# JoelTankard/web-rwkv-gguf

Measured on AMD Instinct MI355X. Metric: tokens/sec RWKV-7 1.5B Q4_K_M decode @1 GPU; achieved HBM GB/s vs roofline, higher is better.
Workload: dtype f16; 1 GPU; RWKV-7 World 1.5B Q4_K_M (Q4_K matrices, Q6_K head, F16 LoRA) batch=1 greedy decode, fused kernels under hipGraph; decode_engine=on, streams_per_gpu=1, pipelines_per_gpu=1, streams=1, parallelism=single

## Files before the change

include/wrk_hip.h:

```cpp
#ifndef WRK_HIP_H
#define WRK_HIP_H

#include <stddef.h>
#include <stdint.h>

#ifdef __cplusplus
extern "C" {
#endif

#define WRK_ABI_VERSION 1

typedef struct wrk_ctx wrk_ctx;
typedef struct wrk_buf wrk_buf;
typedef struct wrk_matrix wrk_matrix;
typedef struct wrk_program wrk_program;
typedef struct wrk_v7_model wrk_v7_model;
typedef struct wrk_v7_state wrk_v7_state;

enum {
    WRK_OK = 0,
    WRK_E_ARG = 1,
    WRK_E_OOM = 2,
    WRK_E_HIP = 3,
    WRK_E_UNSUPPORTED = 4
// ... 56 lines not shown
int32_t wrk_buf_read(wrk_ctx* ctx, const wrk_buf* buf, size_t offset, void* dst, size_t bytes);
int32_t wrk_buf_copy(wrk_ctx* ctx, const wrk_buf* src, size_t src_off, wrk_buf* dst, size_t dst_off, size_t bytes);

int32_t wrk_capture_begin(wrk_ctx* ctx);
int32_t wrk_capture_end(wrk_ctx* ctx, wrk_program** out);
int32_t wrk_program_launch(wrk_ctx* ctx, wrk_program* prog);
int32_t wrk_program_destroy(wrk_program* prog);

int32_t wrk_matrix_create(wrk_ctx* ctx, uint32_t kind, uint32_t k, uint32_t m,
                          const void* data, size_t bytes, uint32_t flags, wrk_matrix** out);
int32_t wrk_matrix_quantize(wrk_ctx* ctx, uint32_t kind, uint32_t k, uint32_t m,
                            const wrk_buf* f16_data, const float* levels, wrk_matrix** out);
int32_t wrk_matrix_export(wrk_matrix* mat, void* dst, size_t capacity, size_t* bytes);
int32_t wrk_matrix_set_scale(wrk_matrix* mat, float scale);
int32_t wrk_matrix_release(wrk_matrix* mat);
size_t wrk_matrix_stream_bytes(const wrk_matrix* mat);


int32_t wrk_op_matmul(wrk_ctx* ctx, const wrk_matrix* mat, const wrk_tensor* input, const wrk_tensor* output,
                      uint32_t act, int32_t turbo, int32_t sparse);
int32_t wrk_op_layer_norm(wrk_ctx* ctx, const wrk_buf* w, const wrk_buf* b, const wrk_tensor* x, float eps);
int32_t wrk_op_group_norm(wrk_ctx* ctx, const wrk_buf* w, const wrk_buf* b, const wrk_tensor* x, float eps);
int32_t wrk_op_l2_norm(wrk_ctx* ctx, const wrk_tensor* x, float eps);
int32_t wrk_op_token_shift(wrk_ctx* ctx, const wrk_buf* cursors, const wrk_tensor* time_mix, const wrk_tensor* state,
                           const wrk_tensor* input, const wrk_tensor* output, int32_t reversed);
int32_t wrk_op_transpose(wrk_ctx* ctx, const wrk_tensor* input, const wrk_tensor* output);
int32_t wrk_op_time_mix_v6(wrk_ctx* ctx, const wrk_buf* cursors, const wrk_tensor* time_decay, const wrk_buf* time_first,
                           const wrk_tensor* state, const wrk_tensor* k, const wrk_tensor* v, const wrk_tensor* r, const wrk_tensor* x);
int32_t wrk_op_channel_mix(wrk_ctx* ctx, const wrk_buf* cursors, const wrk_tensor* state, const wrk_tensor* r, const wrk_tensor* v, const wrk_tensor* x);
int32_t wrk_op_add(wrk_ctx* ctx, const wrk_tensor* input, const wrk_tensor* output, uint32_t act_x, uint32_t act_y, uint32_t act_o);
int32_t wrk_op_mul(wrk_ctx* ctx, const wrk_tensor* input, const wrk_tensor* output, uint32_t act_x, uint32_t act_y, uint32_t act_o);
int32_t wrk_op_lerp(wrk_ctx* ctx, const wrk_tensor* x, const wrk_tensor* y, const wrk_tensor* f, int32_t reversed);
int32_t wrk_op_blit(wrk_ctx* ctx, const wrk_tensor* input, const wrk_tensor* output);
int32_t wrk_op_affine(wrk_ctx* ctx, const wrk_tensor* x, float scale, float bias);
int32_t wrk_op_activate(wrk_ctx* ctx, const wrk_tensor* x, uint32_t act);
int32_t wrk_op_control_k_v7(wrk_ctx* ctx, const wrk_buf* p, const wrk_tensor* a, const wrk_tensor* k);
int32_t wrk_op_time_mix_v7(wrk_ctx* ctx, const wrk_buf* cursors, const wrk_tensor* state, const wrk_tensor* r,
                           const wrk_tensor* w, const wrk_tensor* n, const wrk_tensor* x);
int32_t wrk_op_time_first_v7(wrk_ctx* ctx, const wrk_buf* u, const wrk_tensor* r, const wrk_tensor* n, const wrk_tensor* x);
int32_t wrk_op_channel_mix_v7(wrk_ctx* ctx, const wrk_buf* cursors, const wrk_tensor* state, const wrk_tensor* v, const wrk_tensor* x);
int32_t wrk_op_softmax(wrk_ctx* ctx, const wrk_tensor* x);


typedef struct wrk_v7_layer_desc {
    const wrk_buf *ln1_w, *ln1_b, *ln2_w, *ln2_b;
    const wrk_buf *x_r, *x_w, *x_k, *x_v, *x_a, *x_g;
    const wrk_buf *w0, *a0, *v0;
    const wrk_matrix *w1, *w2, *a1, *a2, *g1, *g2, *v1, *v2;
    const wrk_buf *r_k, *k_k, *k_a;
    const wrk_matrix *w_k, *w_v, *w_r, *w_o;
    const wrk_buf *gn_w, *gn_b;
    const wrk_buf* ffn_x_k;
    const wrk_matrix *ffn_w_k, *ffn_w_v;
} wrk_v7_layer_desc;

typedef struct wrk_v7_model_desc {
    uint32_t num_layer, num_emb, num_hidden, num_vocab, num_head;
    uint32_t lora_w, lora_a, lora_g, lora_v;
    uint32_t rescale;
    const wrk_buf *ln0_w, *ln0_b, *ln_out_w, *ln_out_b;
    const wrk_buf* emb_f16;
    const wrk_matrix* head;
    const wrk_v7_layer_desc* layers;
} wrk_v7_model_desc;

int32_t wrk_v7_model_create(wrk_ctx* ctx, const wrk_v7_model_desc* desc, wrk_v7_model** out);
int32_t wrk_v7_model_destroy(wrk_v7_model* model);
size_t wrk_v7_model_token_bytes(const wrk_v7_model* model, uint32_t num_batch);

int32_t wrk_v7_state_create(wrk_ctx* ctx, const wrk_v7_model* model, uint32_t num_batch, wrk_v7_state** out);
int32_t wrk_v7_state_destroy(wrk_v7_state* state);
int32_t wrk_v7_state_load(wrk_ctx* ctx, wrk_v7_state* state, uint32_t batch, const float* src);
int32_t wrk_v7_state_back(wrk_ctx* ctx, const wrk_v7_state* state, uint32_t batch, float* dst);
int32_t wrk_v7_state_read(wrk_ctx* ctx, const wrk_v7_state* state, uint32_t batch, wrk_buf* buf);
int32_t wrk_v7_state_write(wrk_ctx* ctx, wrk_v7_state* state, uint32_t batch, const wrk_buf* buf);

int32_t wrk_v7_infer(wrk_ctx* ctx, wrk_v7_model* model, wrk_v7_state* state,
                     const uint32_t* tokens, const uint16_t* emb_rows, const uint32_t* cursors, uint32_t num_token,
                     const uint32_t* headers, uint32_t num_header, float* logits, uint32_t* argmax, uint32_t mode);

int32_t wrk_v7_model_set_frame_dtype(wrk_ctx* ctx, wrk_v7_model* model, uint32_t dtype);

int32_t wrk_v7_model_engine_status(wrk_ctx* ctx, wrk_v7_model* model, char* why, size_t capacity);

int32_t wrk_v7_infer_layer(wrk_ctx* ctx, wrk_v7_model* model, wrk_v7_state* state, uint32_t layer, const void* x, const void* v_first,
                           const uint32_t* cursors, uint32_t num_token, uint32_t mode);
int32_t wrk_v7_frame_read(wrk_ctx* ctx, wrk_v7_model* model, const char* name, uint32_t num_token, void* dst, size_t capacity, size_t* bytes);

int32_t wrk_v7_generate_greedy(wrk_ctx* ctx, wrk_v7_model* model, wrk_v7_state* state,
                               const uint32_t* first_tokens, uint32_t num_batch, uint32_t steps,
                               uint32_t* out_tokens, float* last_logits_or_null, float* elapsed_ms_or_null, uint32_t mode);

int32_t wrk_sample_logits(wrk_ctx* ctx, const wrk_buf* logits, uint32_t num_vocab, uint32_t row_stride, uint32_t num_rows,
                          const float* temperature, const float* top_p, const uint32_t* seed, uint32_t step, uint32_t* out_tokens);
int32_t wrk_v7_generate_sample(wrk_ctx* ctx, wrk_v7_model* model, wrk_v7_state* state, const uint32_t* first_tokens, uint32_t num_batch,
                               uint32_t steps, const float* temperature, const float* top_p, const uint32_t* seed,
                               uint32_t* out_tokens, float* last_logits_or_null, float* elapsed_ms_or_null, uint32_t mode);

int32_t wrk_score_logits(wrk_ctx* ctx, const wrk_buf* logits, uint32_t num_vocab, uint32_t row_stride, uint32_t num_rows,
                         const uint32_t* targets, float* logprob, uint32_t* rank);
int32_t wrk_v7_score(wrk_ctx* ctx, wrk_v7_model* model, wrk_v7_state* state,
                     const uint32_t* tokens, const uint16_t* emb_rows, const uint32_t* cursors, uint32_t num_token,
                     const uint32_t* headers, uint32_t num_header, const uint32_t* targets, float* logprob, uint32_t* rank, uint32_t mode);

typedef struct wrk_occurrence wrk_occurrence;
int32_t wrk_occurrence_create(wrk_ctx* ctx, uint32_t num_batch, uint32_t num_vocab, wrk_occurrence** out);
int32_t wrk_occurrence_destroy(wrk_occurrence* occ);
int32_t wrk_occurrence_set_weights(wrk_ctx* ctx, wrk_occurrence* occ, const float* weights);
int32_t wrk_occurrence_ban(wrk_ctx* ctx, wrk_occurrence* occ, uint32_t batch, const uint32_t* tokens, uint32_t n, int32_t banned);
int32_t wrk_occurrence_add(wrk_ctx* ctx, wrk_occurrence* occ, uint32_t batch, const uint32_t* tokens, uint32_t n, float decay);
int32_t wrk_occurrence_back(wrk_ctx* ctx, const wrk_occurrence* occ, uint32_t batch, float* counts, uint32_t* flags);
int32_t wrk_occurrence_load(wrk_ctx* ctx, wrk_occurrence* occ, uint32_t batch, const float* counts, const uint32_t* flags);
int32_t wrk_penalize_logits(wrk_ctx* ctx, wrk_buf* logits, uint32_t num_vocab, uint32_t row_stride, uint32_t num_rows,
                            const wrk_occurrence* occ, uint32_t first_batch, const float* presence, const float* frequency);
int32_t wrk_v7_generate_penalized(wrk_ctx* ctx, wrk_v7_model* model, wrk_v7_state* state, const uint32_t* first_tokens, uint32_t num_batch,
                                  uint32_t steps, const float* temperature, const float* top_p, const uint32_t* seed, const float* presence,
                                  const float* frequency, const float* decay, wrk_occurrence* occ, uint32_t* out_tokens,
                                  float* last_logits_or_null, float* elapsed_ms_or_null, uint32_t mode);

#define WRK_MAX_STOP_TOKENS 16
typedef struct wrk_generate_options {
    const float *temperature, *top_p;
    const uint32_t *seed;
    const float *presence, *frequency, *decay;
    wrk_occurrence *occ;
    const uint32_t *stop_tokens, *stop_offsets;
    uint32_t poll_steps;
} wrk_generate_options;
int32_t wrk_v7_generate_stop(wrk_ctx* ctx, wrk_v7_model* model, wrk_v7_state* state, const uint32_t* first_tokens, uint32_t num_batch,
                             uint32_t steps, const wrk_generate_options* opt, uint32_t* out_tokens, uint32_t* out_lengths,
                             float* last_logits_or_null, uint32_t* steps_run, float* elapsed_ms_or_null, uint32_t mode);

typedef struct wrk_v6_model wrk_v6_model;

typedef struct wrk_v6_layer_desc {
    const wrk_buf *ln1_w, *ln1_b, *ln2_w, *ln2_b;
    const wrk_buf *time_decay;
    const wrk_buf *time_first;
    const wrk_buf *time_mix_x;
    const wrk_buf *time_mix;
    const wrk_matrix *time_decay_w1, *time_decay_w2, *time_mix_w1;
    const wrk_matrix *time_mix_w2[5];
    const wrk_matrix *w_k, *w_v, *w_r, *w_g, *w_o;
    const wrk_buf *gn_w, *gn_b;
    const wrk_buf *ffn_mix_k, *ffn_mix_r;
    const wrk_matrix *ffn_w_k, *ffn_w_v, *ffn_w_r;
} wrk_v6_layer_desc;

typedef struct wrk_v6_model_desc {
    uint32_t num_layer, num_emb, num_hidden, num_vocab, num_head;
    uint32_t time_mix, time_decay;
    uint32_t rescale;
    const wrk_buf *ln0_w, *ln0_b, *ln_out_w, *ln_out_b, *emb_f16;
    const wrk_matrix* head;
    const wrk_v6_layer_desc* layers;
} wrk_v6_model_desc;

int32_t wrk_v6_model_create(wrk_ctx* ctx, const wrk_v6_model_desc* desc, wrk_v6_model** out);
int32_t wrk_v6_model_destroy(wrk_v6_model* model);
size_t wrk_v6_model_token_bytes(const wrk_v6_model* model, uint32_t num_batch);
int32_t wrk_v6_state_create(wrk_ctx* ctx, const wrk_v6_model* model, uint32_t num_batch, wrk_v7_state** out);
int32_t wrk_v6_infer(wrk_ctx* ctx, wrk_v6_model* model, wrk_v7_state* state,
                     const uint32_t* tokens, const uint16_t* emb_rows, const uint32_t* cursors, uint32_t num_token,
                     const uint32_t* headers, uint32_t num_header, float* logits, uint32_t* argmax, uint32_t mode);
int32_t wrk_v6_generate_greedy(wrk_ctx* ctx, wrk_v6_model* model, wrk_v7_state* state,
                               const uint32_t* first_tokens, uint32_t num_batch, uint32_t steps,
// ... 22 lines not shown
```

web-rwkv-gguf_amd/csrc/wrk_runner.h:

```cpp
#pragma once
#include <atomic>
#include <functional>
#include <map>
#include <tuple>
#include <vector>

#include "wrk_internal.h"
#include "wrk_device.h"

struct wrk_v7_state {
    const void* uid = next_uid();
    static const void* next_uid() { static std::atomic<uintptr_t> n{1}; return (const void*)(n.fetch_add(1) << 4); }
    wrk_ctx* ctx = nullptr;
    uint32_t num_layer = 0, num_emb = 0, head_size = 0, num_batch = 0;
    float* data = nullptr;
    size_t layer_elems() const { return (size_t)num_batch * (head_size + 2) * num_emb; }
    float* layer_ptr(uint32_t l) const { return data + layer_elems() * l; }
};

namespace wrk {
struct FrameIo {
    float* head_o;
    uint32_t *cursors, *tokens, *headers, *argmax, *counter;
};

MatJob mat_job(const wrk_matrix* m, DTensor in, DTensor out, uint32_t act);

void advance_tokens(hipStream_t s, const uint32_t* argmax, uint32_t* tokens, uint32_t* history, uint32_t* counter, uint32_t b);
void argmax_finish(hipStream_t s, const float* pv, const uint32_t* pi, uint32_t nwg, uint32_t ntok, uint32_t* argmax, uint32_t* tokens,
                   uint32_t* history, uint32_t* counter);

struct LnMixParams {
    const f16* src;
    const uint32_t* ids;
    const f16 *ln_w, *ln_b;
    float eps;
    uint32_t d, nmix;
    const f16* mix[6];
    f16* out[6];
    f16* ln_out;
    float* state_row;
    size_t state_stride;
    const uint32_t* cursors;
    uint32_t batch1;
    uint32_t no_carry;
};
int ln_mix(hipStream_t s, const LnMixParams& P, uint32_t T);
}

int32_t wrk_buf_write_raw(wrk_ctx* ctx, void* dst, const void* src, size_t bytes);

int32_t wrk_mm(wrk_ctx* ctx, const wrk_matrix* m, DTensor in, DTensor out, uint32_t act);
int32_t wrk_mm_group(wrk_ctx* ctx, wrk::MatJob* jobs, int n);

struct wrk_job_args {
    const uint32_t* tokens; const uint16_t* emb_rows;
    const uint32_t* cursors; uint32_t T;
    const uint32_t* headers; uint32_t NH;
    float* logits; uint32_t* argmax;
    bool score; const uint32_t* targets; float* logprob; uint32_t* rank;
};
struct wrk_job_shape { uint32_t nseq; bool one_token_each, contiguous, identity; };
int32_t wrk_job_check(wrk_ctx* ctx, const wrk_v7_state* st, const uint32_t* cursors, uint32_t T, const uint32_t* tokens_or_null, uint32_t V,
                      const uint32_t* headers, uint32_t NH, wrk_job_shape* shape);
int32_t wrk_score_check(wrk_ctx* ctx, const wrk_job_args& a, uint32_t V, const char* who);

struct wrk_frame_common {
    wrk_ctx* ctx = nullptr;
    void* scratch = nullptr;
    uint32_t scratch_tokens = 0, scratch_headers = 0;
    uint32_t* history = nullptr;
    size_t history_cap = 0;
    wrk::SampleParam* sample_par = nullptr;
    uint32_t sample_par_cap = 0;
    wrk::PenaltyParam* pen_par = nullptr;
    float* pen_o = nullptr;
    uint32_t pen_cap = 0;
    wrk_score_scratch score;
    wrk::StopParam* stop_par = nullptr;
    uint32_t* stop_flags = nullptr;
    float *stop_snap_state = nullptr, *stop_snap_logits = nullptr;
    uint32_t stop_cap = 0;
    size_t stop_slot_cap = 0;
    uint32_t stop_vocab_cap = 0;
    uint32_t* stop_just_ended() const { return stop_flags; }
    uint32_t* stop_live() const { return stop_flags + stop_cap; }
    uint32_t* stop_lengths() const { return stop_flags + stop_cap + 1; }
    uint32_t* live_host = nullptr;
    uint32_t live_host_cap = 0;
    std::vector<hipEvent_t> poll_events;
    uint32_t wkv_nseq = 0;

    struct GraphKey {
        const void* state; uint32_t b, mode, nh = 0;
        bool operator<(const GraphKey& o) const { return std::tie(state, b, mode, nh) < std::tie(o.state, o.b, o.mode, o.nh); }
    };
    std::map<GraphKey, wrk_program*> graphs;

    void drop_graphs();
    int32_t ensure_history(size_t n);
    int32_t ensure_sample_params(uint32_t n);
    int32_t ensure_penalty(uint32_t n, uint32_t num_vocab);
    int32_t ensure_stop(uint32_t n, uint32_t L, uint32_t S, uint32_t D, uint32_t V);
    int32_t ensure_poll(uint32_t lanes);
    void release_common();
};

int32_t wrk_cached_program(wrk_ctx* ctx, std::map<wrk_frame_common::GraphKey, wrk_program*>& graphs, const wrk_frame_common::GraphKey& key,
                           const std::function<int32_t()>& enqueue, wrk_program** prog);

int32_t wrk_job_upload(wrk_frame_common& f, wrk::FrameIo& io, void* input, const wrk_buf* emb, uint32_t D, const wrk_job_args& a, bool gather);
int32_t wrk_job_read_back(wrk_frame_common& f, const wrk::FrameIo& io, uint32_t V, const wrk_job_args& a);

struct wrk_pick_args {
    const float *temperature, *top_p; const uint32_t* seed;
    bool penalized = false;
    const float *presence = nullptr, *frequency = nullptr, *decay = nullptr; wrk_occurrence* occ = nullptr;
};
struct wrk_pick_params {
    std::vector<wrk::SampleParam> par_rows; std::vector<wrk::PenaltyParam> pen_rows;
    const wrk::SampleParam* par = nullptr; const wrk::PenaltyParam* pen = nullptr;
};
int32_t wrk_pick_pack(wrk_ctx* ctx, const wrk_pick_args* pick, uint32_t B, uint32_t V, wrk_pick_params& out);
int32_t wrk_generate_check(wrk_ctx* ctx, const wrk_v7_state* st, bool has_emb, uint32_t num_emb, uint32_t num_layer, uint32_t V,
                           const uint32_t* first_tokens, uint32_t B);
int32_t wrk_decode_prepare(wrk_frame_common& f, wrk::FrameIo& io, uint32_t V, const uint32_t* first_tokens, uint32_t b0, uint32_t B, uint32_t steps,
                           const wrk::SampleParam* par, const wrk::PenaltyParam* pen);
struct wrk_stop_step { const wrk_v7_state* st; uint32_t b0; };
// ... 15 lines not shown
```

web-rwkv-gguf_amd/csrc/wrk_v7.hip:

```cpp
#include "wrk_internal.h"
#include "wrk_v7.h"
#include "wrk_v7_engine.h"

#define LOCK(ctx) std::lock_guard<std::recursive_mutex> _lk((ctx)->mu)

static constexpr float LN_EPS = 1.0e-5f;
static constexpr float GN_EPS = 64.0e-5f;
static constexpr float L2_EPS = 1.0e-12f;

static inline size_t up256(size_t x) { return (x + 255) & ~(size_t)255; }
using wrk::mat_job;

int32_t wrk_v7_model::ensure_scratch(uint32_t T, uint32_t NH) {
    if (T <= scratch_tokens && NH <= scratch_headers && scratch) return WRK_OK;
    if (ctx->capturing_here()) return wrk_fail(ctx, WRK_E_ARG, "scratch must be sized before capture");
    const uint32_t nt = T > scratch_tokens ? T : scratch_tokens;
    const uint32_t nh = NH > scratch_headers ? NH : scratch_headers;
    WRK_HIP(ctx, hipStreamSynchronize(ctx->stream));
    drop_graphs();
    if (scratch) hipFree(scratch);
    scratch = nullptr;
    const size_t D = d.num_emb, F = d.num_hidden, V = d.num_vocab;
    size_t off = 0;
    auto take = [&](size_t bytes) { size_t o = off; off += up256(bytes); return o; };
// ... 400 lines not shown
    wrk_job_shape sh;
    int32_t rc = wrk_job_check(ctx, st, a.cursors, T, a.tokens, V, a.headers, NH, &sh);
    if (rc == WRK_OK) rc = wrk_score_check(ctx, a, V, "wrk_v7_score");
    if (rc == WRK_OK) rc = m->ensure_scratch(T, NH ? NH : 1);
    if (rc == WRK_OK && T == 1 && mode == 1) rc = m->ensure_engine();
    if (rc != WRK_OK) return rc;
    const bool fused = (mode == 1 && sh.one_token_each && sh.nseq == T && m->act_dtype == WRK_F16), want_argmax = NH && a.argmax;
    const uint32_t batch0 = a.cursors[0] & 0xffu;
    rc = wrk_job_upload(*m, m->s, m->s.input, m->emb, m->d.num_emb, a, !fused);
    if (rc != WRK_OK) return rc;
    m->wkv_nseq = sh.nseq;
    auto enqueue_job = [&]() -> int32_t {
        int32_t r;
        if (fused) r = m->enqueue_fused_decode(st, T, NH, sh.identity, a.tokens != nullptr, want_argmax, false, batch0, sh.contiguous);
        else {
            r = m->enqueue_ops(st, T, NH, sh.identity, mode == 1);
            if (r == WRK_OK && want_argmax) wrk::argmax_rows(ctx->op_stream(), m->s.head_o, V, V, NH, m->s.argmax);
        }
        if (r == WRK_OK && a.score && NH &&
            wrk::score_rows(ctx->op_stream(), m->s.head_o, V, V, NH, m->score.targets, m->score.part, m->score.logprob, m->score.rank,
                            ctx->num_cu) != 0)
            r = wrk_fail(ctx, WRK_E_UNSUPPORTED, "score: vocabulary of %u tokens", V);
        return r;
    };
    static const bool no_graph = [] { const char* e = getenv("WRK_NO_GRAPH"); return e && e[0] == '1'; }();
    if (no_graph || ctx->capturing_here()) rc = enqueue_job();
    else {
        const uint32_t flags = 16u | (m->act_dtype == WRK_F32 ? 64u : 0u) | (fused ? 1u : 0u) | (sh.identity ? 2u : 0u) | (a.tokens ? 4u : 0u) | (want_argmax ? 8u : 0u) |
                               ((!fused && mode == 1) ? 32u : 0u) | (fused ? batch0 << 8 : 0u) | ((fused && sh.contiguous) ? 1u << 16 : 0u) |
                               ((fused && T == 1 && m->engine_on()) ? 1u << 17 : 0u) | (split_head_env_on() ? 0u : 1u << 18) |
                               ((!fused && (size_t)sh.nseq * m->d.num_head >= 768) ? 1u << 19 : 0u) | (a.score ? 1u << 20 : 0u);
        const wrk_v7_model::GraphKey key{st->uid, T, flags, NH};
        if (!m->graphs.count(key) && m->graphs.size() > 64) { WRK_HIP(ctx, hipStreamSynchronize(ctx->stream)); m->drop_graphs(); }
        wrk_program* prog = nullptr;
        rc = wrk_cached_program(ctx, m->graphs, key, enqueue_job, &prog);
        if (rc != WRK_OK) return rc;
        WRK_HIP(ctx, hipGraphLaunch(prog->exec, ctx->stream));
    }
    if (rc == WRK_OK) rc = wrk_job_read_back(*m, m->s, V, a);
    if (rc != WRK_OK || ctx->capturing_here()) return rc;
    return wrk_v7_engine_check(m->engine);
}

int32_t wrk_v7_infer(wrk_ctx* ctx, wrk_v7_model* m, wrk_v7_state* st, const uint32_t* tokens, const uint16_t* emb_rows,
                     const uint32_t* cursors, uint32_t T, const uint32_t* headers, uint32_t NH, float* logits, uint32_t* argmax,
                     uint32_t mode) {
    return v7_job(ctx, m, st, {tokens, emb_rows, cursors, T, headers, NH, logits, argmax, false, nullptr, nullptr, nullptr}, mode);
}

int32_t wrk_v7_score(wrk_ctx* ctx, wrk_v7_model* m, wrk_v7_state* st, const uint32_t* tokens, const uint16_t* emb_rows,
                     const uint32_t* cursors, uint32_t T, const uint32_t* headers, uint32_t NH, const uint32_t* targets, float* logprob,
                     uint32_t* rank, uint32_t mode) {
    return v7_job(ctx, m, st, {tokens, emb_rows, cursors, T, headers, NH, nullptr, nullptr, true, targets, logprob, rank}, mode);
}

int32_t wrk_v7_model_set_frame_dtype(wrk_ctx* ctx, wrk_v7_model* m, uint32_t dtype) {
    if (!ctx || !m) return WRK_E_ARG;
    LOCK(ctx);
    WRK_ARG(ctx, dtype == WRK_F16 || dtype == WRK_F32, "frame dtype must be WRK_F16 or WRK_F32");
    WRK_ARG(ctx, !ctx->capturing_here(), "cannot change the frame inside a capture");
    if (dtype == m->act_dtype) return WRK_OK;
    WRK_HIP(ctx, hipSetDevice(ctx->device));
    WRK_HIP(ctx, hipStreamSynchronize(ctx->stream));
    m->drop_graphs();
    if (m->scratch) hipFree(m->scratch);
    m->scratch = nullptr;
    m->scratch_tokens = m->scratch_headers = 0;
    m->act_dtype = dtype;
    for (hipStream_t ls : m->lane_streams) WRK_HIP(ctx, hipStreamSynchronize(ls));
    std::vector<wrk_v7_model*> old_lanes;
    old_lanes.swap(m->lanes);
    for (wrk_v7_model* lane : old_lanes) wrk_v7_model_destroy(lane);
    return WRK_OK;
}

int32_t wrk_v7_model_engine_status(wrk_ctx* ctx, wrk_v7_model* m, char* why, size_t capacity) {
    if (!ctx || !m) return WRK_E_ARG;
    LOCK(ctx);
    WRK_HIP(ctx, hipSetDevice(ctx->device));
    WRK_ARG(ctx, !ctx->capturing_here(), "not inside a capture");
    const int32_t rc = m->ensure_engine();
    if (rc != WRK_OK) return rc;
    if (why && capacity) {
        const std::string& w = m->engine ? std::string() : (m->engine_tried ? m->engine_why : std::string("disabled (WRK_ENGINE=0 or f32 frames)"));
        snprintf(why, capacity, "%s", w.c_str());
    }
    return m->engine ? 1 : 0;
}

int32_t wrk_v7_infer_layer(wrk_ctx* ctx, wrk_v7_model* m, wrk_v7_state* st, uint32_t layer, const void* x, const void* v_first,
                           const uint32_t* cursors, uint32_t T, uint32_t mode) {
    if (!ctx || !m || !st || !x || !cursors) return WRK_E_ARG;
    LOCK(ctx);
    WRK_HIP(ctx, hipSetDevice(ctx->device));
    WRK_ARG(ctx, !ctx->capturing_here(), "wrk_v7_infer_layer cannot be captured");
    WRK_ARG(ctx, layer < m->d.num_layer, "layer %u out of range", layer);
    WRK_ARG(ctx, T >= 1, "no tokens");
    WRK_ARG(ctx, layer == 0 || v_first, "layers above 0 read the layer-0 value (att_v0)");
    WRK_ARG(ctx, st->num_emb == m->d.num_emb && st->num_layer == m->d.num_layer, "state does not belong to this model");
    wrk_job_shape sh;
    int32_t rc = wrk_job_check(ctx, st, cursors, T, nullptr, 0, nullptr, 0, &sh);
    if (rc == WRK_OK) rc = m->ensure_scratch(T, 1);
    if (rc == WRK_OK && T == 1 && mode == 1) rc = m->ensure_engine();
    if (rc != WRK_OK) return rc;
    const size_t esz = m->act_dtype == WRK_F32 ? 4 : 2;
    rc = wrk_buf_write_raw(ctx, m->s.cursors, cursors, (size_t)T * 4);
    if (rc == WRK_OK) rc = wrk_buf_write_raw(ctx, m->s.x, x, (size_t)T * m->d.num_emb * esz);
    if (rc == WRK_OK && v_first) rc = wrk_buf_write_raw(ctx, m->s.att_v0, v_first, (size_t)T * m->d.num_emb * esz);
    if (rc != WRK_OK) return rc;
    m->layer_begin = layer; m->layer_end = layer + 1; m->skip_embed = true;
    m->wkv_nseq = sh.nseq;
    { const char* ei = getenv("WRK_ENGINE_INSPECT"); m->engine_skip_once = !(ei && ei[0] == '1'); }
    if (mode == 1 && sh.one_token_each && sh.nseq == T && m->act_dtype == WRK_F16) rc = m->enqueue_fused_decode(st, T, 0, true, false, false, false, cursors[0] & 0xff, sh.contiguous);
    else rc = m->enqueue_ops(st, T, 0, true, mode == 1);
    m->layer_begin = 0; m->layer_end = 0xffffffffu; m->skip_embed = false; m->engine_skip_once = false;
    if (rc != WRK_OK) return rc;
    WRK_LAUNCH_CHECK(ctx);
    WRK_HIP(ctx, hipStreamSynchronize(ctx->stream));
    return wrk_v7_engine_check(m->engine);
}

int32_t wrk_v7_frame_read(wrk_ctx* ctx, wrk_v7_model* m, const char* name, uint32_t T, void* dst, size_t capacity, size_t* bytes) {
    if (!ctx || !m || !name || !bytes) return WRK_E_ARG;
    LOCK(ctx);
    WRK_ARG(ctx, m->scratch && T >= 1 && T <= m->scratch_tokens, "no frame of %u tokens has been run", T);
    const uint32_t D = m->d.num_emb, F = m->d.num_hidden;
    const V7Scratch& s = m->s;
    struct { const char* n; const void* p; uint32_t c; } tab[] = {
        {"x", s.x, D}, {"att_x", s.att_x, D}, {"att_v0", s.att_v0, D}, {"att_rx", s.rx, D}, {"att_wx", s.wx, D}, {"att_kx", s.kx, D},
        {"att_vx", s.vx, D}, {"att_ax", s.ax, D}, {"att_gx", s.gx, D}, {"att_r", s.r, D}, {"att_w", s.w, D}, {"att_k", s.k, D}, {"att_v", s.v, D},
        {"att_a", s.a, D}, {"att_g", s.g, D}, {"att_o", s.o, D}, {"att_kk", s.kk, D}, {"att_vv", s.vv, D}, {"att_n", s.n, 4 * D},
        {"aux_w", s.aux_w, m->d.lora_w}, {"aux_a", s.aux_a, m->d.lora_a}, {"aux_g", s.aux_g, m->d.lora_g}, {"aux_v", s.aux_v, m->d.lora_v},
        {"ffn_x", s.ffn_x, D}, {"ffn_kx", s.ffn_kx, D}, {"ffn_k", s.ffn_k, F}, {"ffn_v", s.ffn_v, D}, {"att_x_ln", s.ln_tmp, D}};
    const size_t esz = m->act_dtype == WRK_F32 ? 4 : 2;
    for (auto& e : tab)
        if (strcmp(e.n, name) == 0) {
            const size_t n = (size_t)e.c * T * esz;
            *bytes = n;
            if (!dst) return WRK_OK;
            WRK_ARG(ctx, capacity >= n, "frame buffer %s needs %zu bytes, capacity %zu", name, n, capacity);
            WRK_HIP(ctx, hipSetDevice(ctx->device));
            WRK_HIP(ctx, hipMemcpyAsync(dst, e.p, n, hipMemcpyDeviceToHost, ctx->stream));
            WRK_HIP(ctx, hipStreamSynchronize(ctx->stream));
            return WRK_OK;
        }
    return wrk_fail(ctx, WRK_E_ARG, "no frame buffer named %s", name);
}

static int32_t enqueue_decode_step(wrk_ctx* ctx, wrk_v7_model* m, wrk_v7_state* st, uint32_t b0, uint32_t B, uint32_t mode, bool sampled,
                                   bool penalized, bool stop = false) {
    int32_t rc;
    const wrk_stop_step ss{st, b0};
    if (mode == 1 && m->act_dtype == WRK_F16) {
        rc = m->enqueue_fused_decode(st, B, B, true, true, !sampled, !sampled && !stop, b0, true);
        if (!sampled && (!stop || rc != WRK_OK)) return rc;
        if (!sampled) return wrk_enqueue_stop_tail(*m, m->s, m->d.num_vocab, B, false, ss);
    } else {
        wrk::gather_rows_f16(ctx->op_stream(), m->emb->ptr, m->s.tokens, m->s.input, m->d.num_emb, B);
        rc = m->enqueue_ops(st, B, B, true);
    }
    if (rc != WRK_OK) return rc;
    return wrk_enqueue_pick(*m, m->s, m->d.num_vocab, B, sampled, penalized, stop ? &ss : nullptr);
}

static int32_t decode_prepare(wrk_ctx* ctx, wrk_v7_model* m, wrk_v7_state* st, const uint32_t* first_tokens, uint32_t b0, uint32_t B,
                              uint32_t steps, uint32_t mode, bool eager, const wrk::SampleParam* par, const wrk::PenaltyParam* pen,
                              const wrk::StopParam* stop, wrk_program** prog_out) {
    int32_t rc = m->ensure_scratch(B, B);
    if (rc == WRK_OK && B == 1 && mode == 1) rc = m->ensure_engine();
    if (rc == WRK_OK) rc = wrk_decode_prepare(*m, m->s, m->d.num_vocab, first_tokens, b0, B, steps, par, pen);
// ... 134 lines not shown
```

web-rwkv-gguf_amd/csrc/wrk_v7_engine.h:

```cpp
#pragma once
#include <stdint.h>

#include "wrk_internal.h"

namespace wrk {

constexpr int ENG_K1_JOBS = 7;
constexpr uint32_t ENG_NO_HEAD = 0xffffffffu;

struct EngJob {
    uint32_t rows, row_bytes, f16;
    uint32_t act, mix;
    uint32_t wg0, nwg, rows_per_wg;
    uint32_t gbase;
    uint32_t headed;
};

struct EngShape {
    uint32_t D, F, H, nwg;
    uint32_t rw, ra, rg, rv;
    uint32_t rb_d, rb_f;
    uint32_t rb_w2, rb_a2, rb_g2, rb_v2;
    EngJob k1[ENG_K1_JOBS];
    uint32_t k3_rpw, k5_rpw, k6_rpw;
    uint32_t lds_slot1, lds_slot5, lds_slot6, lds_slot3, lds_xraw0, lds_xraw1, lds_xs, lds_ln, lds_misc, lds_total;
    uint32_t g_x, g_k1, g_o, g_x1, g_k, g_total, g_aux;
    float ln_eps, gn_eps, l2_eps;
    uint32_t layer_begin, layer_end, rescale;
    uint32_t batch, state_rows;
    uint32_t x_from_granules;
};

struct EngLayer {
    const uint8_t *w_r, *w_k, *w_v, *w1, *a1, *g1, *v1;
    const uint8_t *w2, *a2, *g2, *v2;
    const uint8_t *w_o, *ffn_k, *ffn_v;
};
enum { ENG_V_LN1W, ENG_V_LN1B, ENG_V_LN2W, ENG_V_LN2B, ENG_V_MIX0, ENG_V_W0 = ENG_V_MIX0 + 6, ENG_V_A0, ENG_V_V0, ENG_V_RK, ENG_V_KK, ENG_V_KA,
       ENG_V_GNW, ENG_V_GNB, ENG_V_FFNXK, ENG_NV };
enum { ENG_S_O = ENG_K1_JOBS, ENG_S_FK, ENG_S_FV, ENG_NS = 16 };

struct EngArgs {
    EngShape S;
    const EngLayer* layers;
    const void* vecs;
    const float* scal;
    unsigned long long* gran;
    const void* x_in;
    const uint32_t* x_row;
    void* x_out;
    void* v_first;
    float* state;
    uint32_t num_batch;
    uint32_t* fail;
    unsigned long long* stamps;
    uint32_t stamp_layer;
};
constexpr int ENG_STAMPS = 32;

}

struct wrk_v7_model;
struct wrk_v7_state;
struct wrk_v7_engine;
int32_t wrk_v7_engine_create(wrk_v7_model* m, wrk_v7_engine** out);
void wrk_v7_engine_destroy(wrk_v7_engine* e);
int32_t wrk_v7_engine_enqueue(wrk_v7_engine* e, hipStream_t q, wrk_v7_state* st, uint32_t batch, uint32_t l0, uint32_t l1, const void* x_in,
                              void* x_out, void* v_first, const uint32_t* token = nullptr);
bool wrk_v7_engine_has_table(const wrk_v7_engine* e);
int32_t wrk_v7_engine_check(wrk_v7_engine* e);
void wrk_v7_engine_report(wrk_v7_engine* e);
```

web-rwkv-gguf_amd/csrc/wrk_v7_engine.hip:

```cpp
#include "wrk_device.h"
#include "wrk_v7.h"
#include "wrk_dmv_body.h"
#include "wrk_v7_engine.h"
#include "wrk_lora_dev.h"

#include <algorithm>
#include <string>

namespace wrk {

#define ENG_LDS __attribute__((address_space(3)))
typedef ENG_LDS unsigned char lds_u8;

#define ENG_BAR() asm volatile("s_waitcnt lgkmcnt(0)\n\ts_barrier" ::: "memory")

constexpr uint32_t ENG_SPIN_MAX = 1u << 21;

__device__ __forceinline__ uint32_t eng_tag(uint32_t layer, uint32_t stage) { return layer * 8u + stage + 1u; }

__device__ __forceinline__ void eng_store_granule(unsigned long long* g, uint32_t tag, uint32_t payload) {
    __hip_atomic_store(g, ((unsigned long long)tag << 32) | payload, __ATOMIC_RELAXED, __HIP_MEMORY_SCOPE_AGENT);
}
__device__ __forceinline__ uint32_t pack_h2(float a, float b) {
    const f16x2 h = {(f16)a, (f16)b};
    return __builtin_bit_cast(uint32_t, h);
}

__device__ __forceinline__ bool eng_gather(const unsigned long long* g, uint32_t n16, uint32_t tag, ENG_LDS uint32_t* dst, uint32_t lane) {
    for (uint32_t base = 0; base < n16; base += 512) {
        const u32x4* p[8];
#pragma unroll
        for (int i = 0; i < 8; ++i) p[i] = (const u32x4*)g + min(base + lane + 64u * i, n16 - 1);
        u32x4 v[8];
        bool good = false;
        for (uint32_t spins = 0; spins < ENG_SPIN_MAX; ++spins) {
            asm volatile(
                "global_load_dwordx4 %0, %8, off sc1\n\tglobal_load_dwordx4 %1, %9, off sc1\n\tglobal_load_dwordx4 %2, %10, off sc1\n\t"
                "global_load_dwordx4 %3, %11, off sc1\n\tglobal_load_dwordx4 %4, %12, off sc1\n\tglobal_load_dwordx4 %5, %13, off sc1\n\t"
                "global_load_dwordx4 %6, %14, off sc1\n\tglobal_load_dwordx4 %7, %15, off sc1\n\ts_waitcnt vmcnt(0)"
                : "=&v"(v[0]), "=&v"(v[1]), "=&v"(v[2]), "=&v"(v[3]), "=&v"(v[4]), "=&v"(v[5]), "=&v"(v[6]), "=&v"(v[7])
                : "v"(p[0]), "v"(p[1]), "v"(p[2]), "v"(p[3]), "v"(p[4]), "v"(p[5]), "v"(p[6]), "v"(p[7])
                : "memory");
            bool ok = true;
#pragma unroll
            for (int i = 0; i < 8; ++i) ok &= (v[i].y == tag) & (v[i].w == tag);
            if (__all(ok)) { good = true; break; }
            __builtin_amdgcn_s_sleep(1);
        }
        if (!good) return false;
#pragma unroll
        for (int i = 0; i < 8; ++i) {
            const uint32_t q = base + lane + 64u * i;
            if (q < n16) { dst[2 * q] = v[i].x; dst[2 * q + 1] = v[i].z; }
        }
    }
    return true;
}

__device__ __forceinline__ void eng_copy_in(const void* src, uint32_t n16, ENG_LDS u32x4* dst, uint32_t lane) {
    for (uint32_t q = lane; q < n16; q += 64) dst[q] = ((const u32x4*)src)[q];
}

template <int KIND>
__device__ __forceinline__ bool eng_sweep_x(const unsigned long long* g, uint32_t c, uint32_t tag, XRegs& x) {
    uint32_t lo, hi;
    chunk_xoff<KIND>(c, lo, hi);
    const u32x4* pl = (const u32x4*)g + (lo >> 2);
    const u32x4* ph = (const u32x4*)g + (hi >> 2);
    u32x4 v[8];
    for (uint32_t spins = 0; spins < ENG_SPIN_MAX; ++spins) {
        asm volatile(
            "global_load_dwordx4 %0, %8, off sc1\n\tglobal_load_dwordx4 %1, %8, off offset:16 sc1\n\tglobal_load_dwordx4 %2, %8, off offset:32 sc1\n\t"
            "global_load_dwordx4 %3, %8, off offset:48 sc1\n\tglobal_load_dwordx4 %4, %9, off sc1\n\tglobal_load_dwordx4 %5, %9, off offset:16 sc1\n\t"
            "global_load_dwordx4 %6, %9, off offset:32 sc1\n\tglobal_load_dwordx4 %7, %9, off offset:48 sc1\n\ts_waitcnt vmcnt(0)"
            : "=&v"(v[0]), "=&v"(v[1]), "=&v"(v[2]), "=&v"(v[3]), "=&v"(v[4]), "=&v"(v[5]), "=&v"(v[6]), "=&v"(v[7])
            : "v"(pl), "v"(ph)
            : "memory");
        bool ok = true;
#pragma unroll
        for (int i = 0; i < 8; ++i) ok &= (v[i].y == tag) & (v[i].w == tag);
        if (__all(ok)) {
#pragma unroll
            for (int h = 0; h < 4; ++h) {
                const u32x4 q = {v[2 * h].x, v[2 * h].z, v[2 * h + 1].x, v[2 * h + 1].z};
                x.v[h] = __builtin_bit_cast(f16x8, q);
            }
            return true;
        }
        __builtin_amdgcn_s_sleep(1);
    }
    return false;
}

__device__ __forceinline__ uint32_t eng_fill(const uint8_t* src, uint32_t bytes, lds_u8* smem, uint32_t lds_off, uint32_t lane) {
    if (bytes == 0) return 0;
    const uint32_t np = (bytes + 1023u) >> 10;
    for (uint32_t p = 0; p < np; ++p) {
        const uint32_t off = min(p * 1024u + lane * 16u, bytes - 16u);
        __builtin_amdgcn_global_load_lds((const __attribute__((address_space(1))) void*)(src + off), (ENG_LDS void*)(smem + lds_off + p * 1024u), 16, 0, 2);
    }
    return np;
// ... 9 lines not shown
    else asm volatile("s_waitcnt vmcnt(0)" ::: "memory");
}

template <int KIND>
__device__ __forceinline__ Raw lds_raw(const lds_u8* row, uint32_t k, uint32_t c) {
    Raw r;
    r.w = *(const ENG_LDS u32x4*)(row + c * 16u);
    r.a = (u32x4){0, 0, 0, 0};
    r.b = (u32x2){0, 0};
    const uint32_t nb = k >> 8, b = c >> 3;
    if (KIND == WRK_MAT_Q4_K) {
        r.a.x = *(const ENG_LDS uint32_t*)(row + (nb * 128u + b * 4u));
        r.a.y = *(const ENG_LDS uint32_t*)(row + (nb * 132u + b * 16u + ((c & 7u) >> 1) * 4u));
    }
    return r;
}

template <int KIND>
__device__ __forceinline__ XRegs lds_x(const ENG_LDS f16* x, uint32_t c) {
    XRegs r;
    const f16x8 z = {0, 0, 0, 0, 0, 0, 0, 0};
    r.v[0] = r.v[1] = r.v[2] = r.v[3] = z;
    r.s[0] = r.s[1] = 0.0f;
    uint32_t lo, hi;
    chunk_xoff<KIND>(c, lo, hi);
    r.v[0] = *(const ENG_LDS f16x8*)(x + lo);
    if (KIND != WRK_MAT_F16) {
        r.v[1] = *(const ENG_LDS f16x8*)(x + lo + 8);
        r.v[2] = *(const ENG_LDS f16x8*)(x + hi);
        r.v[3] = *(const ENG_LDS f16x8*)(x + hi + 8);
    }
    return r;
}

template <int MAXCH>
__device__ __forceinline__ float eng_lora_dot(const f16x8 (&w)[MAXCH], const ENG_LDS f16* aux, uint32_t rank, uint32_t part) {
    float acc = 0.0f;
#pragma unroll
    for (int n = 0; n < MAXCH; ++n) {
        const uint32_t c = part * 8 + 32 * n;
        if (c < rank) {
            const f16x8 x = *(const ENG_LDS f16x8*)(aux + c);
            acc = __builtin_amdgcn_fdot2(__builtin_shufflevector(w[n], w[n], 0, 1), __builtin_shufflevector(x, x, 0, 1), acc, false);
            acc = __builtin_amdgcn_fdot2(__builtin_shufflevector(w[n], w[n], 2, 3), __builtin_shufflevector(x, x, 2, 3), acc, false);
            acc = __builtin_amdgcn_fdot2(__builtin_shufflevector(w[n], w[n], 4, 5), __builtin_shufflevector(x, x, 4, 5), acc, false);
            acc = __builtin_amdgcn_fdot2(__builtin_shufflevector(w[n], w[n], 6, 7), __builtin_shufflevector(x, x, 6, 7), acc, false);
        }
    }
    acc += dpp_f32<0xB1>(acc);
    acc += dpp_f32<0x4E>(acc);
    return acc;
}

struct EngFin {
    uint32_t act;
    float scale;
    const ENG_LDS f16* res;
    float post;
};
__device__ __forceinline__ float eng_finish(const EngFin& f, uint32_t row, float v) {
    float o = act_apply(f.act, v * f.scale);
    if (f.res) o = r16(o) + (float)f.res[row];
    return o;
}

template <int KIND, bool R16, int XI, int RB, class GIDX>
__device__ __forceinline__ void eng_rows(const lds_u8* slot, uint32_t row_bytes, uint32_t K, const ENG_LDS f16* xs, uint32_t row0, uint32_t r_begin,
                                         uint32_t r_end, const EngFin& fin, ENG_LDS uint32_t* pub, unsigned long long* gran, uint32_t tag, GIDX gidx,
                                         uint32_t lane) {
    if (r_begin >= r_end) return;
    const uint32_t kpad = (K + 15u) & ~15u;
    const uint32_t nch = num_chunks<KIND>(K, kpad);
    XRegs x[1][XI];
#pragma unroll
    for (int ci = 0; ci < XI; ++ci) {
        const uint32_t c = lane + 64u * ci;
        x[0][ci] = lds_x<KIND>(xs, min(c, nch - 1));
        if (c >= nch) {
            const f16x8 z = {0, 0, 0, 0, 0, 0, 0, 0};
            x[0][ci].v[0] = x[0][ci].v[1] = x[0][ci].v[2] = x[0][ci].v[3] = z;
        }
        x_sums<KIND>(x[0][ci]);
    }
    static_assert(RB == 2 || RB == 4, "rows per batch");
    for (uint32_t ri = r_begin; ri < r_end; ri += RB) {
        Raw raw[RB][XI];
#pragma unroll
        for (int rb = 0; rb < RB; ++rb) {
            const lds_u8* rowp = slot + (size_t)min(ri + rb, r_end - 1) * row_bytes;
#pragma unroll
            for (int ci = 0; ci < XI; ++ci) raw[rb][ci] = lds_raw<KIND>(rowp, K, min(lane + 64u * ci, nch - 1));
        }
        float v[4] = {0.0f, 0.0f, 0.0f, 0.0f};
#pragma unroll
        for (int rb = 0; rb < RB; ++rb) {
            float acc[1] = {0.0f};
#pragma unroll
            for (int ci = 0; ci < XI; ++ci) dot_raw_tokens<KIND, R16, 1, XI>(raw[rb][ci], min(lane + 64u * ci, nch - 1), x, ci, acc);
            v[rb] = wave_sum(acc[0]);
        }
        if (lane < RB / 2) {
            const uint32_t ra = ri + 2 * lane;
            if (ra < r_end) {
                const float o0 = eng_finish(fin, row0 + ra, lane ? v[2] : v[0]) * fin.post;
                const float o1 = eng_finish(fin, row0 + ra + 1, lane ? v[3] : v[1]) * fin.post;
                if (pub) pub[ra >> 1] = pack_h2(o0, o1);
                else eng_store_granule(gran + gidx(row0 + ra), tag, pack_h2(o0, o1));
            }
        }
    }
}

template <class GIDX>
__device__ __forceinline__ void eng_publish(const ENG_LDS uint32_t* pub, uint32_t nrows, uint32_t row0, unsigned long long* gran, uint32_t tag, GIDX gidx,
                                            uint32_t lane) {
    for (uint32_t i = lane; 2 * i < nrows; i += 64) eng_store_granule(gran + gidx(row0 + 2 * i), tag, pub[i]);
}

template <int VPT>
__device__ __forceinline__ void eng_ln_mix(bool active, const ENG_LDS f16* xraw, ENG_LDS f16* xs, ENG_LDS f16* ln_out, ENG_LDS float* red, uint32_t K, float eps,
                                           const f16x8 (&wv)[VPT], const f16x8 (&bv)[VPT], const f16x8 (&mv)[VPT], const f32x4 (&pv)[VPT][2],
                                           uint32_t tid, uint32_t lane, uint32_t wave) {
    const uint32_t nvec = K >> 3;
    f16x8 xv[VPT];
    float c0 = 0.0f;
    if (active) {
#pragma unroll
        for (int v = 0; v < VPT; ++v) xv[v] = *(const ENG_LDS f16x8*)(xraw + min(tid + 256u * v, nvec - 1) * 8);
        c0 = (float)xraw[0];
        float s1 = 0.0f, s2 = 0.0f;
#pragma unroll
        for (int v = 0; v < VPT; ++v)
            if (tid + 256u * v < nvec)
#pragma unroll
                for (int e = 0; e < 8; ++e) { const float dl = (float)xv[v][e] - c0; s1 += dl; s2 = __builtin_fmaf(dl, dl, s2); }
        s1 = wave_sum(s1);
        s2 = wave_sum(s2);
        if (lane == 0) { red[wave] = s1; red[4 + wave] = s2; }
    }
    ENG_BAR();
    if (active) {
        const float a1 = (red[0] + red[1]) + (red[2] + red[3]);
        const float a2 = (red[4] + red[5]) + (red[6] + red[7]);
        const float md = a1 / (float)K;
        const float mean = c0 + md;
        const float dev = 1.0f / sqrtf(fmaxf(a2 / (float)K - md * md, 0.0f) + eps);
#pragma unroll
        for (int v = 0; v < VPT; ++v) {
            const uint32_t i = tid + 256u * v;
            if (i >= nvec) continue;
            f16x8 yv, o;
#pragma unroll
            for (int e = 0; e < 8; ++e) {
                yv[e] = (f16)__builtin_fmaf(((float)xv[v][e] - mean) * dev, (float)wv[v][e], (float)bv[v][e]);
                o[e] = (f16)wgsl_mix((float)yv[e], pv[v][e >> 2][e & 3], (float)mv[v][e]);
            }
            *(ENG_LDS f16x8*)(xs + i * 8) = o;
            *(ENG_LDS f16x8*)(ln_out + i * 8) = yv;
        }
    }
    ENG_BAR();
}

constexpr int ENG_K2_BARRIERS = 6;
template <int XD, bool R16, int QK, int NCW>
__global__ void __launch_bounds__((NCW + 2) * 64) v7_engine_kernel(const EngArgs A, const uint32_t* __restrict__ wg_head) {
    extern __shared__ __attribute__((aligned(16))) unsigned char eng_smem_generic[];
    lds_u8* smem = (lds_u8*)eng_smem_generic;
    const EngShape& S = A.S;
    const uint32_t tid_all = threadIdx.x;
    const uint32_t wave = (uint32_t)__builtin_amdgcn_readfirstlane((int)(tid_all >> 6));
    const uint32_t wg = blockIdx.x;
    const uint32_t D = S.D, F = S.F;
    const uint32_t head = wg_head[2 * wg], k1r = wg_head[2 * wg + 1];
    const bool is_head = head != ENG_NO_HEAD;
    ENG_LDS uint32_t* abort_flag = (ENG_LDS uint32_t*)(smem + S.lds_misc + 1008);
    ENG_LDS float* red = (ENG_LDS float*)(smem + S.lds_misc);
    ENG_LDS float* part = (ENG_LDS float*)(smem + S.lds_misc + 64);
    ENG_LDS uint32_t* pub = (ENG_LDS uint32_t*)(smem + S.lds_misc + 64);
    ENG_LDS f16* xraw0 = (ENG_LDS f16*)(smem + S.lds_xraw0);
    ENG_LDS f16* xraw1 = (ENG_LDS f16*)(smem + S.lds_xraw1);
    ENG_LDS f16* xs = (ENG_LDS f16*)(smem + S.lds_xs);
    ENG_LDS f16* lnbuf = (ENG_LDS f16*)(smem + S.lds_ln);
    ENG_LDS f16* auxbuf = (ENG_LDS f16*)(smem + S.lds_xs + D * 2u);
    const uint32_t naux = S.rw + S.ra + S.rg + S.rv;
    ENG_LDS float* k2f = (ENG_LDS float*)(smem + S.lds_xs + D * 2u + ((naux + 192u) * 2u + 15u & ~15u));

    uint32_t j1 = ENG_K1_JOBS;
#pragma unroll
    for (int j = 0; j < ENG_K1_JOBS; ++j)
        if (k1r >= S.k1[j].wg0 && k1r < S.k1[j].wg0 + S.k1[j].nwg) j1 = j;
    const uint32_t k1_row0 = j1 < ENG_K1_JOBS ? (k1r - S.k1[j1].wg0) * S.k1[j1].rows_per_wg : 0u;
    const uint32_t k1_rows = j1 < ENG_K1_JOBS ? min(S.k1[j1].rows_per_wg, S.k1[j1].rows - k1_row0) : 0u;
    const uint32_t k1_rb = j1 < ENG_K1_JOBS ? S.k1[j1].row_bytes : 0u;
    const uint32_t k3_row0 = wg * S.k3_rpw, k3_rows = k3_row0 < D ? min(S.k3_rpw, D - k3_row0) : 0u;
    const uint32_t k5_row0 = wg * S.k5_rpw, k5_rows = k5_row0 < F ? min(S.k5_rpw, F - k5_row0) : 0u;
    const uint32_t k6_row0 = wg * S.k6_rpw, k6_rows = k6_row0 < D ? min(S.k6_rpw, D - k6_row0) : 0u;
    const uint32_t srows = S.state_rows;
    auto layer_state = [&](uint32_t l) { return A.state + ((size_t)l * A.num_batch + S.batch) * srows * D; };
    auto k1_src = [&](const EngLayer& L) -> const uint8_t* {
        const uint8_t* base = j1 == 0 ? L.w_r : j1 == 1 ? L.w_k : j1 == 2 ? L.w_v : j1 == 3 ? L.w1 : j1 == 4 ? L.a1 : j1 == 5 ? L.g1 : L.v1;
        return base + (size_t)k1_row0 * k1_rb;
    };
    auto k1_active = [&](uint32_t l) { return j1 < ENG_K1_JOBS && !(j1 == 6 && l == 0) && k1_rows > 0; };
    ENG_LDS unsigned long long* lds_stamps = (ENG_LDS unsigned long long*)(smem + S.lds_misc + 1024);
#define ENG_STAMP(l, k)                                                                                                  \
    do {                                                                                                                 \
        if (A.stamps && (l) == A.stamp_layer && (tid_all & 63u) == 0) lds_stamps[wave * 24 + (k)] = __builtin_amdgcn_s_memrealtime(); \
    } while (0)
#define ENG_STAMP0(l, k) ENG_STAMP(l, k)
#define ENG_FLUSH(l)                                                                                                     \
    do {                                                                                                                 \
        if (A.stamps && (l) == A.stamp_layer && (tid_all & 63u) < 24u)                                                   \
            A.stamps[((size_t)wg * (NCW + 2) + wave) * 24 + (tid_all & 63u)] = lds_stamps[wave * 24 + (tid_all & 63u)];   \
    } while (0)

    if (A.stamps && tid_all < (NCW + 2) * 24) lds_stamps[tid_all] = 0;
    if (tid_all == 0) *abort_flag = 0;
    ENG_BAR();

    if (wave == NCW + 1) {
        const uint32_t lane = tid_all & 63u;
        uint32_t issued = 0, m1 = 0, m3 = 0, m5 = 0, m6 = 0;
        auto fill1 = [&](uint32_t l) { const EngLayer& L = A.layers[l]; issued += eng_fill(k1_src(L), k1_active(l) ? k1_rows * k1_rb : 0u, smem, S.lds_slot1, lane); m1 = issued; };
        auto fill3 = [&](uint32_t l) { const EngLayer& L = A.layers[l]; issued += eng_fill(L.w_o + (size_t)k3_row0 * S.rb_d, k3_rows * S.rb_d, smem, S.lds_slot3, lane); m3 = issued; };
        auto fill5 = [&](uint32_t l) { const EngLayer& L = A.layers[l]; issued += eng_fill(L.ffn_k + (size_t)k5_row0 * S.rb_d, k5_rows * S.rb_d, smem, S.lds_slot5, lane); m5 = issued; };
        auto fill6 = [&](uint32_t l) { const EngLayer& L = A.layers[l]; issued += eng_fill(L.ffn_v + (size_t)k6_row0 * S.rb_f, k6_rows * S.rb_f, smem, S.lds_slot6, lane); m6 = issued; };
        fill1(S.layer_begin); fill3(S.layer_begin); fill5(S.layer_begin); fill6(S.layer_begin);
        bool p6 = false;
        for (uint32_t l = S.layer_begin; l < S.layer_end; ++l) {
            const bool more = l + 1 < S.layer_end;
            eng_wait_vm(issued - m1);
            ENG_BAR();
            if (*abort_flag) break;
            if (p6) { fill6(l); p6 = false; }
            ENG_BAR(); ENG_BAR(); ENG_BAR();
            ENG_STAMP(l, 0);
            if (more) fill1(l + 1);
            if (is_head) {
                ENG_BAR();
                if (*abort_flag) break;
#pragma unroll
                for (int i = 1; i < ENG_K2_BARRIERS; ++i) ENG_BAR();
            }
            eng_wait_vm(issued - m3);
            ENG_BAR();
            if (*abort_flag) break;
            ENG_BAR();
            eng_wait_vm(issued - m5);
            ENG_BAR();
            if (*abort_flag) break;
            if (more) fill3(l + 1);
            ENG_BAR(); ENG_BAR(); ENG_BAR(); ENG_BAR();
            eng_wait_vm(issued - m6);
            ENG_BAR();
            if (*abort_flag) break;
            if (more) fill5(l + 1);
            ENG_BAR(); ENG_BAR();
            p6 = more;
            ENG_FLUSH(l);
        }
        asm volatile("s_waitcnt vmcnt(0)" ::: "memory");
        return;
    }

    if (wave == NCW) {
        const uint32_t lane = tid_all & 63u;
        for (uint32_t l = S.layer_begin; l < S.layer_end; ++l) {
            bool ok = true;
            if (l == S.layer_begin) eng_copy_in(A.x_row ? (const void*)((const f16*)A.x_in + (size_t)A.x_row[0] * D) : A.x_in, D >> 3, (ENG_LDS u32x4*)xraw0, lane);
            else ok = eng_gather(A.gran + S.g_x, D >> 2, eng_tag(l - 1, 4), (ENG_LDS uint32_t*)xraw0, lane);
            if (!ok && lane == 0) { *abort_flag = 1; atomicOr(A.fail, 1u); }
            ENG_STAMP(l, 0);
            ENG_BAR();
            if (*abort_flag) break;
            ENG_BAR(); ENG_BAR(); ENG_BAR();
            if (is_head) {
                ok = eng_gather(A.gran + S.g_k1, (l == 0 ? naux - S.rv : naux) >> 2, eng_tag(l, 0), (ENG_LDS uint32_t*)auxbuf, lane);
                if (ok) ok = eng_gather(A.gran + S.g_k1 + S.g_aux + head * 96u, 48u, eng_tag(l, 0), (ENG_LDS uint32_t*)(auxbuf + naux), lane);
                if (!ok && lane == 0) { *abort_flag = 1; atomicOr(A.fail, 2u); }
                ENG_STAMP(l, 1);
                ENG_BAR();
                if (*abort_flag) break;
#pragma unroll
                for (int i = 1; i < ENG_K2_BARRIERS; ++i) ENG_BAR();
            }
            ok = eng_gather(A.gran + S.g_o, D >> 2, eng_tag(l, 1), (ENG_LDS uint32_t*)xs, lane);
            if (!ok && lane == 0) { *abort_flag = 1; atomicOr(A.fail, 4u); }
            ENG_STAMP(l, 2);
            ENG_BAR();
            if (*abort_flag) break;
            ENG_BAR();
            ok = eng_gather(A.gran + S.g_x1, D >> 2, eng_tag(l, 2), (ENG_LDS uint32_t*)xraw1, lane);
            if (!ok && lane == 0) { *abort_flag = 1; atomicOr(A.fail, 8u); }
            ENG_STAMP(l, 3);
            ENG_BAR();
            if (*abort_flag) break;
            ENG_BAR(); ENG_BAR(); ENG_BAR(); ENG_BAR();
            ENG_BAR();
            if (*abort_flag) break;
            ENG_BAR(); ENG_BAR();
            ENG_FLUSH(l);
        }
        return;
    }

    constexpr int VPT = XD;
    constexpr int S64 = 64;
    constexpr int MAXU = (16 + NCW - 1) / NCW;
    const uint32_t nvec = D >> 3;
    const float eps = S.ln_eps;
    const bool ln_wave = wave < 4;
    auto wave_rows = [&](uint32_t nrows, uint32_t& b, uint32_t& e) {
        const uint32_t q = 2u * (((nrows + 1u) / 2u + NCW - 1u) / NCW);
        b = min(wave * q, nrows);
        e = min(b + q, nrows);
    };
    const uint32_t c0 = is_head ? head * S64 : 0u;
    float vfirst_keep = 0.0f;
    if (is_head && S.layer_begin > 0 && wave == 0) vfirst_keep = (float)((const f16*)A.v_first)[c0 + (tid_all & 63u)];

    unsigned long long clk0 = 0, rt0 = 0;
    if (A.stamps && wg == 0 && tid_all == 0) { clk0 = __builtin_amdgcn_s_memtime(); rt0 = __builtin_amdgcn_s_memrealtime(); }
    for (uint32_t l = S.layer_begin; l < S.layer_end; ++l) {
        uint32_t tid = tid_all;
        asm volatile("" : "+v"(tid));
        const uint32_t lane = tid & 63u;
        float* lst = layer_state(l);
        const bool layer0 = l == 0;
        const f16* lv_base = (const f16*)A.vecs + (size_t)l * ENG_NV * D;
        auto lvec = [&](uint32_t idx) { return lv_base + (size_t)idx * D; };
        const float* scl = A.scal + (size_t)l * ENG_NS;
        const float sc_k1 = scl[j1 < ENG_K1_JOBS ? j1 : 0u], sc_o = scl[ENG_S_O], sc_fk = scl[ENG_S_FK], sc_fv = scl[ENG_S_FV];

        f16x8 wv[VPT], bv[VPT], mv[VPT];
        f32x4 pv[VPT][2];
        if (ln_wave) {
            const f16* mixp = lvec(ENG_V_MIX0 + (j1 < ENG_K1_JOBS ? S.k1[j1].mix : 0u));
#pragma unroll
            for (int v = 0; v < VPT; ++v) {
                const uint32_t i = min(tid + 256u * v, nvec - 1);
                wv[v] = *(const f16x8*)(lvec(ENG_V_LN1W) + i * 8);
                bv[v] = *(const f16x8*)(lvec(ENG_V_LN1B) + i * 8);
                mv[v] = *(const f16x8*)(mixp + i * 8);
                pv[v][0] = *(const f32x4*)(lst + i * 8);
                pv[v][1] = *(const f32x4*)(lst + i * 8 + 4);
            }
        }

        auto request_k5 = [&]() {
            if (ln_wave) {
                float* rowf = lst + (size_t)(srows - 1) * D;
    #pragma unroll
                for (int v = 0; v < VPT; ++v) {
                    const uint32_t i = min(tid + 256u * v, nvec - 1);
                    wv[v] = *(const f16x8*)(lvec(ENG_V_LN2W) + i * 8);
                    bv[v] = *(const f16x8*)(lvec(ENG_V_LN2B) + i * 8);
                    mv[v] = *(const f16x8*)(lvec(ENG_V_FFNXK) + i * 8);
                    pv[v][0] = *(const f32x4*)(rowf + i * 8);
                    pv[v][1] = *(const f32x4*)(rowf + i * 8 + 4);
                }
            }
        };
        if (!is_head) {
            ENG_BAR();
            if (*abort_flag) break;
            ENG_STAMP0(l, 1);
            eng_ln_mix<VPT>(ln_wave, xraw0, xs, lnbuf, red, D, eps, wv, bv, mv, pv, tid, lane, wave);
            ENG_STAMP0(l, 2);
            if (k1_active(l)) {
                const EngJob& J = S.k1[j1];
                uint32_t rb, re;
                wave_rows(k1_rows, rb, re);
                const EngFin fin{J.act, sc_k1, nullptr, 1.0f};
                const lds_u8* slot = smem + S.lds_slot1;
                ENG_LDS uint32_t* nopub = nullptr;
                if (J.f16) {
                    const uint32_t gb = S.g_k1 + J.gbase;
                    eng_rows<WRK_MAT_F16, false, 4 * XD, 2>(slot, k1_rb, D, xs, k1_row0, rb, re, fin, nopub, A.gran, eng_tag(l, 0),
                                                            [&](uint32_t r) { return gb + (r >> 1); }, lane);
                } else {
                    const uint32_t gb = S.g_k1 + S.g_aux + J.gbase * 32u;
                    eng_rows<QK, R16, XD, 4>(slot, k1_rb, D, xs, k1_row0, rb, re, fin, nopub, A.gran, eng_tag(l, 0),
                                             [&](uint32_t r) { return gb + (r >> 6) * 96u + ((r & 63u) >> 1); }, lane);
                }
            }
            ENG_STAMP0(l, 3);
            ENG_BAR();
        } else {
            const EngLayer& Lp = A.layers[l];
            const uint8_t* p_m[4] = {Lp.w2, Lp.a2, Lp.g2, layer0 ? Lp.w2 : Lp.v2};
            const uint32_t rbm[4] = {S.rb_w2, S.rb_a2, S.rb_g2, layer0 ? S.rb_w2 : S.rb_v2};
            const uint32_t rkm[4] = {S.rw, S.ra, S.rg, layer0 ? S.rw : S.rv};
            f16x8 lu[MAXU][8];
#pragma unroll
            for (int i = 0; i < MAXU; ++i) {
                const uint32_t u = min(wave + (uint32_t)i * NCW, 15u), mi = u >> 2, bi = u & 3u;
                const f16* rowp = (const f16*)(p_m[mi] + (size_t)(c0 + 16u * bi + (lane >> 2)) * rbm[mi]);
#pragma unroll
                for (int n = 0; n < 8; ++n) lu[i][n] = *(const f16x8*)(rowp + min((lane & 3u) * 8 + 32 * n, rkm[mi] - 8));
            }
            float Sreg[16];
            const uint32_t ci64 = tid & 63u, g4 = tid >> 6;
            float* st = lst + (size_t)D + c0 + ci64;
            if (ln_wave) {
#pragma unroll
                for (int jj = 0; jj < 16; ++jj) Sreg[jj] = st[(size_t)(g4 * 16 + jj) * D];
            }
            f16 h_w0 = 0, h_a0 = 0, h_kk = 0, h_ka = 0, h_v0 = 0, h_gnw = 0, h_gnb = 0, h_rk = 0;
            if (wave == 0) {
                const uint32_t cc = c0 + lane;
                h_w0 = lvec(ENG_V_W0)[cc]; h_a0 = lvec(ENG_V_A0)[cc]; h_kk = lvec(ENG_V_KK)[cc]; h_ka = lvec(ENG_V_KA)[cc]; h_v0 = lvec(ENG_V_V0)[cc];
                h_gnw = lvec(ENG_V_GNW)[cc]; h_gnb = lvec(ENG_V_GNB)[cc]; h_rk = lvec(ENG_V_RK)[cc];
            }
            ENG_BAR();
            if (*abort_flag) break;
            ENG_STAMP0(l, 1);
            eng_ln_mix<VPT>(ln_wave, xraw0, xs, lnbuf, red, D, eps, wv, bv, mv, pv, tid, lane, wave);
            ENG_STAMP0(l, 3);
            ENG_BAR();

            ENG_LDS float* sh_r = k2f; ENG_LDS float* sh_w = k2f + 64; ENG_LDS float* sh_k = k2f + 128; ENG_LDS float* sh_v = k2f + 192;
            ENG_LDS float* sh_a = k2f + 256; ENG_LDS float* sh_b = k2f + 320; ENG_LDS float* sh_g = k2f + 384; ENG_LDS float* sh_kk = k2f + 448;
            ENG_LDS float* sh_red = k2f + 512;
            ENG_LDS float* sh_red2 = k2f + 768;
            ENG_LDS float* sh_d = k2f + 1024;
            ENG_BAR();
            if (*abort_flag) break;
            ENG_STAMP0(l, 4);
            {
                const ENG_LDS f16* auxm[4] = {auxbuf, auxbuf + S.rw, auxbuf + S.rw + S.ra, layer0 ? auxbuf : auxbuf + S.rw + S.ra + S.rg};
#pragma unroll
                for (int i = 0; i < MAXU; ++i) {
                    const uint32_t u = wave + (uint32_t)i * NCW;
                    if (u < 16u) {
                        const uint32_t mi = u >> 2, bi = u & 3u;
                        const float dd = eng_lora_dot<8>(lu[i], auxm[mi], rkm[mi], lane & 3u);
                        if ((lane & 3u) == 0) sh_d[mi * 64 + 16 * bi + (lane >> 2)] = dd;
                    }
                }
            }
            ENG_STAMP0(l, 16);
            ENG_BAR();
            const ENG_LDS f16* hr = auxbuf + naux, *hk = hr + 64, *hv = hr + 128;
            if (wave == 0) {
                const float w0 = (float)h_w0, a0 = (float)h_a0, kkw = (float)h_kk, kaw = (float)h_ka;
                const float kraw = (float)hk[lane], rraw = (float)hr[lane];
                float v = (float)hv[lane];
                const float v0w = layer0 ? 0.0f : (float)h_v0, vfirst = layer0 ? 0.0f : vfirst_keep;
                const float dw = sh_d[lane], da = sh_d[64 + lane], dg = sh_d[128 + lane], dv = layer0 ? 0.0f : sh_d[192 + lane];
                const float w = r16(w0 + r16(dw));
                const float a = r16(act_sigmoid(a0 + r16(da)));
                const float g = r16(dg);
                if (layer0) { vfirst_keep = v; ((f16*)A.v_first)[c0 + lane] = (f16)v; }
                else {
                    const float vv = r16(act_sigmoid(v0w + r16(dv)));
                    v = r16(wgsl_mix(v, vfirst, vv));
                }
                sh_w[lane] = __expf(-0.606531f * act_sigmoid(w));
                sh_g[lane] = g;
                sh_v[lane] = v;
                sh_r[lane] = rraw;
                const float kkv = r16(kkw * kraw);
                sh_k[lane] = r16(kraw * (1.0f + (a - 1.0f) * kaw));
                const float nrm = 1.0f / sqrtf(wave_sum(kkv * kkv) + S.l2_eps);
                const float kkn = r16(kkv * nrm);
                sh_a[lane] = -kkn;
                sh_b[lane] = kkn * a;
                sh_kk[lane] = kkv;
            }
            if (wave == 1) lst[c0 + lane] = (float)lnbuf[c0 + lane];
            ENG_STAMP0(l, 17);
            ENG_BAR();
            if (ln_wave) {
                float sa = 0.0f;
                f32x4 av[4];
#pragma unroll
                for (int q = 0; q < 4; ++q) av[q] = *(const ENG_LDS f32x4*)(sh_a + g4 * 16 + 4 * q);
#pragma unroll
                for (int jj = 0; jj < 16; ++jj) sa = __builtin_fmaf(Sreg[jj], av[jj >> 2][jj & 3], sa);
                sh_red[g4 * 64 + ci64] = sa;
            }
            ENG_BAR();
            if (ln_wave) {
                const float sa = (sh_red[ci64] + sh_red[64 + ci64]) + (sh_red[128 + ci64] + sh_red[192 + ci64]);
                const float vv = sh_v[ci64];
                float y = 0.0f;
#pragma unroll
                for (int q = 0; q < 4; ++q) {
                    const f32x4 wq = *(const ENG_LDS f32x4*)(sh_w + g4 * 16 + 4 * q), kq4 = *(const ENG_LDS f32x4*)(sh_k + g4 * 16 + 4 * q);
                    const f32x4 bq = *(const ENG_LDS f32x4*)(sh_b + g4 * 16 + 4 * q), rq4 = *(const ENG_LDS f32x4*)(sh_r + g4 * 16 + 4 * q);
#pragma unroll
                    for (int e = 0; e < 4; ++e) {
                        const int jj = 4 * q + e, j = g4 * 16 + jj;
                        const float sn = Sreg[jj] * wq[e] + kq4[e] * vv + sa * bq[e];
                        st[(size_t)j * D] = sn;
                        y = __builtin_fmaf(rq4[e], sn, y);
                    }
                }
                sh_red2[g4 * 64 + ci64] = y;
            }
            ENG_STAMP0(l, 18);
            ENG_BAR();
            if (wave == 0) {
                float y = r16((sh_red2[lane] + sh_red2[64 + lane]) + (sh_red2[128 + lane] + sh_red2[192 + lane]));
                const float mean = wave_sum(y) * (1.0f / S64);
                const float dl = y - mean;
                const float var = wave_sum(dl * dl) * (1.0f / S64) + S.gn_eps;
                float o = r16(__builtin_fmaf(dl * (1.0f / sqrtf(var)), (float)h_gnw, (float)h_gnb));
                const float xx = wave_sum((float)h_rk * sh_k[lane] * sh_r[lane]);
                o = r16(o + xx * sh_v[lane]);
                o = sh_g[lane] * o;
                const float o_next = __shfl_down(o, 1, WAVE);
                if ((lane & 1u) == 0) eng_store_granule(A.gran + S.g_o + ((c0 + lane) >> 1), eng_tag(l, 1), pack_h2(o, o_next));
            }
            ENG_STAMP0(l, 5);
            ENG_BAR();
        }

        request_k5();
        ENG_BAR();
        if (*abort_flag) break;
        ENG_STAMP0(l, 6);
        {
            uint32_t rb, re;
            wave_rows(k3_rows, rb, re);
            const EngFin fin{WRK_ACT_NONE, sc_o, xraw0, 1.0f};
            const uint32_t gb = S.g_x1;
            ENG_LDS uint32_t* nopub = nullptr;
            eng_rows<QK, R16, XD, 2>(smem + S.lds_slot3, S.rb_d, D, xs, k3_row0, rb, re, fin, nopub, A.gran, eng_tag(l, 2),
                                     [&](uint32_t r) { return gb + (r >> 1); }, lane);
        }
        ENG_STAMP0(l, 7);
        ENG_BAR();

        ENG_BAR();
        if (*abort_flag) break;
        ENG_STAMP0(l, 8);
        eng_ln_mix<VPT>(ln_wave, xraw1, xs, lnbuf, red, D, eps, wv, bv, mv, pv, tid, lane, wave);
        ENG_STAMP0(l, 14);
        {
            uint32_t rb, re;
            wave_rows(k5_rows, rb, re);
            const EngFin fin{WRK_ACT_SQUARED_RELU, sc_fk, nullptr, 1.0f};
            const uint32_t gb = S.g_k;
            eng_rows<QK, R16, XD, 4>(smem + S.lds_slot5, S.rb_d, D, xs, k5_row0, rb, re, fin, pub, A.gran, eng_tag(l, 3), [&](uint32_t r) { return gb + (r >> 1); }, lane);
            ENG_BAR();
            if (wave == 0) eng_publish(pub, k5_rows, k5_row0, A.gran, eng_tag(l, 3), [&](uint32_t r) { return gb + (r >> 1); }, lane);
        }
        ENG_STAMP0(l, 9);
        ENG_BAR();

        {
            constexpr uint32_t NG = NCW / 4;
            const uint32_t kq = wave & 3u, grp = wave >> 2;
            const bool k6_wave = grp < NG;
            const uint32_t rq = (k6_rows + NG - 1) / NG;
            const uint32_t g_b = min(grp * rq, k6_rows), g_e = min(g_b + rq, k6_rows);
            const uint32_t kpad = (F + 15u) & ~15u;
            const uint32_t nch = num_chunks<QK>(F, kpad);
            const uint32_t cbase = lane + 64u * kq;
            XRegs x[1][XD];
            bool swept = true;
#pragma unroll
            for (int ci = 0; ci < XD; ++ci) {
                const uint32_t c = cbase + 256u * ci;
                x[0][ci].s[0] = x[0][ci].s[1] = 0.0f;
                const f16x8 z = {0, 0, 0, 0, 0, 0, 0, 0};
                x[0][ci].v[0] = x[0][ci].v[1] = x[0][ci].v[2] = x[0][ci].v[3] = z;
                if (k6_wave && g_b < g_e && swept) swept = eng_sweep_x<QK>(A.gran + S.g_k, min(c, nch - 1), eng_tag(l, 3), x[0][ci]);
                if (c >= nch) x[0][ci].v[0] = x[0][ci].v[1] = x[0][ci].v[2] = x[0][ci].v[3] = z;
                x_sums<QK>(x[0][ci]);
            }
            if (!swept && lane == 0) { *abort_flag = 1; atomicOr(A.fail, 16u); }
            ENG_STAMP0(l, 10);
            ENG_BAR();
            if (*abort_flag) break;
            ENG_STAMP0(l, 11);
            const lds_u8* slot = smem + S.lds_slot6;
            if (k6_wave)
                for (uint32_t ri = g_b; ri < g_e; ri += 4) {
                    Raw raw[4][XD];
#pragma unroll
                    for (int rb = 0; rb < 4; ++rb) {
                        const lds_u8* rowp = slot + (size_t)min(ri + rb, g_e - 1) * S.rb_f;
#pragma unroll
                        for (int ci = 0; ci < XD; ++ci) raw[rb][ci] = lds_raw<QK>(rowp, F, min(cbase + 256u * ci, nch - 1));
                    }
#pragma unroll
                    for (int rb = 0; rb < 4; ++rb) {
                        float acc[1] = {0.0f};
#pragma unroll
                        for (int ci = 0; ci < XD; ++ci) dot_raw_tokens<QK, R16, 1, XD>(raw[rb][ci], min(cbase + 256u * ci, nch - 1), x, ci, acc);
                        const float pvs = wave_sum(acc[0]);
                        if (lane == 0 && ri + rb < g_e) part[(ri + rb) * 4 + kq] = pvs;
                    }
                }
        }
        ENG_STAMP0(l, 12);
        ENG_BAR();
        if (wave == 0) {
            const bool valid = lane < k6_rows;
            const uint32_t r = k6_row0 + min(lane, k6_rows ? k6_rows - 1 : 0u);
            float o = 0.0f;
            if (k6_rows) {
                const uint32_t p = min(lane, k6_rows - 1);
                o = ((part[p * 4] + part[p * 4 + 1]) + (part[p * 4 + 2] + part[p * 4 + 3])) * sc_fv;
                o = r16(o) + (float)xraw1[r];
                if ((l + 1) % S.rescale == 0) o = r16(o) * 0.5f;
            }
            const float o_next = __shfl_down(o, 1, WAVE);
            if (valid) {
                lst[(size_t)(srows - 1) * D + r] = (float)lnbuf[r];
                if ((lane & 1u) == 0) eng_store_granule(A.gran + S.g_x + (r >> 1), eng_tag(l, 4), pack_h2(o, o_next));
                if (l + 1 == S.layer_end) ((f16*)A.x_out)[r] = (f16)o;
            }
        }
        ENG_STAMP0(l, 13);
        ENG_BAR();
        ENG_FLUSH(l);
    }
    if (A.stamps && wg == 0 && tid_all == 0) {
        unsigned long long* tail = A.stamps + (size_t)S.nwg * 16 * 24;
        tail[0] = __builtin_amdgcn_s_memtime() - clk0;
        tail[1] = __builtin_amdgcn_s_memrealtime() - rt0;
    }
#undef ENG_STAMP
#undef ENG_STAMP0
#undef ENG_FLUSH
}

}

struct wrk_v7_engine {
    wrk_v7_model* m = nullptr;
    wrk::EngShape S{};
    wrk::EngLayer* layers = nullptr;
    void* vecs = nullptr;
    float* scal = nullptr;
    uint32_t* wg_head = nullptr;
    unsigned long long* gran = nullptr;
    uint32_t* fail = nullptr;
    unsigned long long* stamps = nullptr;
    void* emb_ln = nullptr;
    bool r16 = false;
    int xd = 1, ncw = 8;
    uint32_t quant = 0;
};

static uint32_t up(uint32_t v, uint32_t a) { return (v + a - 1) / a * a; }

typedef void (*eng_fn)(const wrk::EngArgs, const uint32_t*);
static eng_fn eng_kernel(int xd, bool r16, int ncw) {
    using namespace wrk;
#define ENG_PICK(XD_, R_) (ncw == 14 ? (eng_fn)v7_engine_kernel<XD_, R_, WRK_MAT_Q4_K, 14> : (eng_fn)v7_engine_kernel<XD_, R_, WRK_MAT_Q4_K, 8>)
    if (xd == 1) return r16 ? ENG_PICK(1, true) : ENG_PICK(1, false);
    return r16 ? ENG_PICK(2, true) : ENG_PICK(2, false);
#undef ENG_PICK
}
static const void* eng_kernel_fn(int xd, bool r16, int ncw) { return (const void*)eng_kernel(xd, r16, ncw); }

int32_t wrk_v7_engine_create(wrk_v7_model* m, wrk_v7_engine** out) {
    using namespace wrk;
    wrk_ctx* ctx = m->ctx;
    *out = nullptr;
    const auto& d = m->d;
    const uint32_t D = d.num_emb, F = d.num_hidden, H = d.num_head, NWG = (uint32_t)ctx->num_cu;
    auto no = [&](const char* why) { return wrk_fail(ctx, WRK_E_UNSUPPORTED, "decode engine: %s", why); };
    if (m->act_dtype != WRK_F16) return no("f32 frames");
    if (H == 0 || D != H * 64 || D % 256 || D > 4096 || F % 1024 || F != 4 * D) return no("shape");
    if (d.lora_w % 8 || d.lora_a % 8 || d.lora_g % 8 || d.lora_v % 8 || d.lora_w < 8 || d.lora_a < 8 || d.lora_g < 8 || d.lora_v < 8 ||
        d.lora_w > 128 || d.lora_a > 128 || d.lora_v > 128 || d.lora_g > 256 || ((d.lora_w + d.lora_a + d.lora_g + d.lora_v) % 16))
        return no("LoRA ranks");
    if (NWG < 2 * H || NWG < 64) return no("too few compute units");
    uint32_t quant = 0xffffffffu, flags = 0xffffffffu;
    for (size_t li = 0; li < m->layers.size(); ++li) {
        const auto& L = m->layers[li];
        const wrk_matrix* big[] = {L.w_r, L.w_k, L.w_v, L.w_o, L.ffn_w_k, L.ffn_w_v};
        for (const wrk_matrix* q : big) {
            if (quant == 0xffffffffu) { quant = q->kind; flags = q->flags; }
            if (q->kind != quant || q->flags != flags) return no("mixed matrix kinds");
        }
        const wrk_matrix* lo[] = {L.w1, L.a1, L.g1, li ? L.v1 : L.a1, L.w2, L.a2, L.g2, li ? L.v2 : L.a2};
        for (const wrk_matrix* q : lo)
            if (!q || q->kind != WRK_MAT_F16) return no("LoRA matrices must be F16");
        if (L.w_r->k != D || L.w_r->m != D || L.ffn_w_k->m != F || L.ffn_w_v->k != F || L.w1->m != d.lora_w || L.a1->m != d.lora_a ||
            L.g1->m != d.lora_g || (li && L.v1->m != d.lora_v))
            return no("matrix shapes");
    }
    if (quant != WRK_MAT_Q4_K) return no("only Q4_K matrices so far");
    if (m->layers.empty()) return no("no layers");

    wrk_v7_engine* e = new wrk_v7_engine();
    e->m = m;
    e->quant = quant;
    e->r16 = (flags & WRK_MATRIX_ROUND_F16) != 0;
    e->xd = D <= 2048 ? 1 : 2;
    EngShape& S = e->S;
    S.D = D; S.F = F; S.H = H; S.nwg = NWG;
    S.rw = d.lora_w; S.ra = d.lora_a; S.rg = d.lora_g; S.rv = d.lora_v;
    const auto& L0 = m->layers[0];
    const auto& L1 = m->layers[m->layers.size() > 1 ? 1 : 0];
    S.rb_d = (uint32_t)L0.w_r->row_bytes; S.rb_f = (uint32_t)L0.ffn_w_v->row_bytes;
    S.rb_w2 = (uint32_t)L0.w2->row_bytes; S.rb_a2 = (uint32_t)L0.a2->row_bytes; S.rb_g2 = (uint32_t)L0.g2->row_bytes;
    S.rb_v2 = (uint32_t)(m->layers.size() > 1 ? L1.v2->row_bytes : L0.a2->row_bytes);
    for (const auto& L : m->layers) {
        if (L.w_r->row_bytes != S.rb_d || L.w_k->row_bytes != S.rb_d || L.w_v->row_bytes != S.rb_d || L.w_o->row_bytes != S.rb_d ||
            L.ffn_w_k->row_bytes != S.rb_d || L.ffn_w_v->row_bytes != S.rb_f || L.w2->row_bytes != S.rb_w2 || L.a2->row_bytes != S.rb_a2 ||
            L.g2->row_bytes != S.rb_g2) { delete e; return no("row strides differ between layers"); }
    }
    const uint32_t rb_l = (uint32_t)L0.w1->row_bytes;
    struct { uint32_t rows, rb, f16, act, mix, headed, gbase; } jd[ENG_K1_JOBS] = {
        {D, S.rb_d, 0, WRK_ACT_NONE, 0, 1, 0}, {D, S.rb_d, 0, WRK_ACT_NONE, 2, 1, 1}, {D, S.rb_d, 0, WRK_ACT_NONE, 3, 1, 2},
        {S.rw, rb_l, 1, WRK_ACT_TANH, 1, 0, 0}, {S.ra, rb_l, 1, WRK_ACT_NONE, 4, 0, S.rw / 2}, {S.rg, rb_l, 1, WRK_ACT_SIGMOID, 5, 0, (S.rw + S.ra) / 2},
        {S.rv, rb_l, 1, WRK_ACT_NONE, 3, 0, (S.rw + S.ra + S.rg) / 2}};
    double total = 0;
    for (auto& j : jd) total += (double)j.rows * j.rb;
    uint32_t slot1 = 0;
    bool placed = false;
    const uint32_t NK1 = NWG - H;
    for (double target = total / NK1; target < total; target *= 1.03) {
        uint32_t used = 0, worst = 0;
        uint32_t rpw[ENG_K1_JOBS], nw[ENG_K1_JOBS];
        for (int j = 0; j < ENG_K1_JOBS; ++j) {
            uint32_t r = (uint32_t)(target / jd[j].rb);
            r = std::max(2u, r / 2 * 2);
            rpw[j] = r;
            nw[j] = (jd[j].rows + r - 1) / r;
            used += nw[j];
            worst = std::max(worst, std::min(r, jd[j].rows) * jd[j].rb);
        }
        if (used > NK1) continue;
        uint32_t w0 = 0;
        for (int j = 0; j < ENG_K1_JOBS; ++j) {
            S.k1[j] = EngJob{jd[j].rows, jd[j].rb, jd[j].f16, jd[j].act, jd[j].mix, w0, nw[j], rpw[j], jd[j].gbase, jd[j].headed};
            w0 += nw[j];
        }
        slot1 = worst;
        placed = true;
        break;
    }
    if (!placed) { delete e; return no("K1 partition"); }
    S.k3_rpw = std::max(8u, up((D + NWG - 1) / NWG, 8));
    S.k5_rpw = std::max(8u, up((F + NWG - 1) / NWG, 8));
    S.k6_rpw = std::max(2u, up((D + NWG - 1) / NWG, 2));
    if (S.k6_rpw > 32) { delete e; return no("ffn value rows per workgroup"); }
    uint32_t off = 0;
    auto take = [&](uint32_t bytes) { const uint32_t o = off; off += up(bytes, 1024); return o; };
    S.lds_slot1 = take(slot1);
    S.lds_slot5 = take(S.k5_rpw * S.rb_d);
    S.lds_slot6 = take(S.k6_rpw * S.rb_f);
    S.lds_slot3 = take(S.k3_rpw * S.rb_d);
    S.lds_xraw0 = take(D * 2);
    S.lds_xraw1 = take(D * 2);
    const uint32_t naux = S.rw + S.ra + S.rg + S.rv;
    S.lds_xs = take(D * 2 + up((naux + 192) * 2, 16) + 1280 * 4);
    S.lds_ln = take(D * 2);
    S.lds_misc = take(4096);
    S.lds_total = off;
    int lds_max = 0;
    hipDeviceGetAttribute(&lds_max, hipDeviceAttributeMaxSharedMemoryPerBlock, ctx->device);
    if (lds_max < 160 * 1024) lds_max = 160 * 1024;
    if (S.lds_total > (uint32_t)lds_max) { delete e; return no("weights of a layer do not fit the LDS"); }
    S.g_aux = naux / 2;
    uint32_t g = 0;
    auto gtake = [&](uint32_t n) { const uint32_t o = g; g += up(n, 128); return o; };
    S.g_x = gtake(D / 2);
    S.g_k1 = gtake(S.g_aux + H * 96);
    S.g_o = gtake(D / 2);
    S.g_x1 = gtake(D / 2);
    S.g_k = gtake(F / 2);
    S.g_total = g;
    S.ln_eps = 1.0e-5f; S.gn_eps = 64.0e-5f; S.l2_eps = 1.0e-12f;
    S.rescale = d.rescale ? d.rescale : 0xffffffffu;
    S.state_rows = 64 + 2;

    std::vector<float> hs(m->layers.size() * ENG_NS, 1.0f);
    auto fail_alloc = [&](hipError_t er) { wrk_v7_engine_destroy(e); return wrk_fail(ctx, WRK_E_OOM, "decode engine: %s", hipGetErrorString(er)); };
    hipError_t er;
    std::vector<EngLayer> hl(m->layers.size());
    for (size_t li = 0; li < m->layers.size(); ++li) {
        const auto& L = m->layers[li];
        EngLayer& o = hl[li];
        o.w_r = L.w_r->data; o.w_k = L.w_k->data; o.w_v = L.w_v->data; o.w1 = L.w1->data; o.a1 = L.a1->data; o.g1 = L.g1->data;
        o.v1 = li ? L.v1->data : L.a1->data;
        o.w2 = L.w2->data; o.a2 = L.a2->data; o.g2 = L.g2->data; o.v2 = li ? L.v2->data : L.a2->data;
        o.w_o = L.w_o->data; o.ffn_k = L.ffn_w_k->data; o.ffn_v = L.ffn_w_v->data;
        const wrk_matrix* k1m[ENG_K1_JOBS] = {L.w_r, L.w_k, L.w_v, L.w1, L.a1, L.g1, li ? L.v1 : L.a1};
        float* sc = hs.data() + li * ENG_NS;
        for (int j = 0; j < ENG_K1_JOBS; ++j) sc[j] = k1m[j]->out_scale;
        sc[ENG_S_O] = L.w_o->out_scale; sc[ENG_S_FK] = L.ffn_w_k->out_scale; sc[ENG_S_FV] = L.ffn_w_v->out_scale;
    }
    if ((er = hipMalloc((void**)&e->vecs, hl.size() * ENG_NV * D * 2)) != hipSuccess) return fail_alloc(er);
    for (size_t li = 0; li < m->layers.size(); ++li) {
        const auto& L = m->layers[li];
        const wrk_buf* src[ENG_NV] = {L.ln1_w, L.ln1_b, L.ln2_w, L.ln2_b, L.x_r, L.x_w, L.x_k, L.x_v, L.x_a, L.x_g, L.w0, L.a0, li ? L.v0 : L.w0,
                                      L.r_k, L.k_k, L.k_a, L.gn_w, L.gn_b, L.ffn_x_k};
        for (int i = 0; i < ENG_NV; ++i) {
            if (!src[i] || src[i]->bytes < (size_t)D * 2) { wrk_v7_engine_destroy(e); return no("a layer vector is missing"); }
            if ((er = hipMemcpy((char*)e->vecs + (li * ENG_NV + i) * (size_t)D * 2, src[i]->ptr, (size_t)D * 2, hipMemcpyDeviceToDevice)) != hipSuccess) return fail_alloc(er);
        }
    }
    if ((er = hipMalloc((void**)&e->scal, hs.size() * 4)) != hipSuccess) return fail_alloc(er);
    if ((er = hipMemcpy(e->scal, hs.data(), hs.size() * 4, hipMemcpyHostToDevice)) != hipSuccess) return fail_alloc(er);
    if ((er = hipMalloc((void**)&e->layers, hl.size() * sizeof(EngLayer))) != hipSuccess) return fail_alloc(er);
    if ((er = hipMemcpy(e->layers, hl.data(), hl.size() * sizeof(EngLayer), hipMemcpyHostToDevice)) != hipSuccess) return fail_alloc(er);
    std::vector<uint32_t> hh(2 * NWG, ENG_NO_HEAD);
    for (uint32_t h = 0; h < H; ++h) hh[2 * ((size_t)h * NWG / H)] = h;
    for (uint32_t w = 0, r = 0; w < NWG; ++w)
        if (hh[2 * w] == ENG_NO_HEAD) hh[2 * w + 1] = r++;
    if ((er = hipMalloc((void**)&e->wg_head, hh.size() * 4)) != hipSuccess) return fail_alloc(er);
    if ((er = hipMemcpy(e->wg_head, hh.data(), hh.size() * 4, hipMemcpyHostToDevice)) != hipSuccess) return fail_alloc(er);
    if ((er = hipMalloc((void**)&e->gran, (size_t)S.g_total * 8)) != hipSuccess) return fail_alloc(er);
    if ((er = hipMalloc((void**)&e->fail, 256)) != hipSuccess) return fail_alloc(er);
    if ((er = hipMemset(e->fail, 0, 256)) != hipSuccess) return fail_alloc(er);
    const char* tm = getenv("WRK_TIMING");
    if (tm && tm[0] == '1') {
        const size_t n = (size_t)NWG * 16 * 24 * 8 + 64;
        if ((er = hipMalloc((void**)&e->stamps, n)) != hipSuccess) return fail_alloc(er);
        hipMemset(e->stamps, 0, n);
    }
    { const char* ev = getenv("WRK_ENGINE_WAVES"); e->ncw = (ev && atoi(ev) == 14) ? 14 : 8; }
    const void* fn = eng_kernel_fn(e->xd, e->r16, e->ncw);
    if ((er = hipFuncSetAttribute(fn, hipFuncAttributeMaxDynamicSharedMemorySize, (int)S.lds_total)) != hipSuccess) {
        wrk_v7_engine_destroy(e);
        return wrk_fail(ctx, WRK_E_UNSUPPORTED, "decode engine: %u bytes of LDS refused (%s)", S.lds_total, hipGetErrorString(er));
    }
    {
        hipFuncAttributes fa{};
        const int waves = e->ncw + 2, per_simd = (waves + 3) / 4;
        if (hipFuncGetAttributes(&fa, fn) == hipSuccess && fa.numRegs > 0) {
            const int alloc = (fa.numRegs + 7) / 8 * 8;
            if (per_simd * alloc > 512 || fa.maxThreadsPerBlock < waves * 64 || (size_t)fa.sharedSizeBytes + S.lds_total > 160 * 1024) {
                const int regs = fa.numRegs;
                wrk_v7_engine_destroy(e);
                return wrk_fail(ctx, WRK_E_UNSUPPORTED, "decode engine: a workgroup of %d waves x %d registers + %u bytes of LDS does not fit a CU", waves, regs,
                                S.lds_total);
            }
        }
        (void)hipGetLastError();
    }
    {
        const char* te = getenv("WRK_ENGINE_TABLE");
        if (!(te && te[0] == '0') && m->emb && m->ln0_w && m->ln0_b) {
            const size_t bytes = (size_t)d.num_vocab * D * 2;
            if (hipMalloc(&e->emb_ln, bytes) == hipSuccess) {
                LnMixParams P{};
                P.src = (const f16*)m->emb->ptr; P.ln_w = (const f16*)m->ln0_w->ptr; P.ln_b = (const f16*)m->ln0_b->ptr; P.eps = 1.0e-5f;
                P.d = D; P.nmix = 0; P.ln_out = (f16*)e->emb_ln;
                if (ln_mix(ctx->stream, P, d.num_vocab) != 0 || hipStreamSynchronize(ctx->stream) != hipSuccess) { hipFree(e->emb_ln); e->emb_ln = nullptr; }
            } else e->emb_ln = nullptr;
            (void)hipGetLastError();
        }
    }
    *out = e;
    return WRK_OK;
}

bool wrk_v7_engine_has_table(const wrk_v7_engine* e) { return e && e->emb_ln; }

void wrk_v7_engine_destroy(wrk_v7_engine* e) {
    if (!e) return;
    if (e->emb_ln) hipFree(e->emb_ln);
    if (e->layers) hipFree(e->layers);
    if (e->vecs) hipFree(e->vecs);
    if (e->scal) hipFree(e->scal);
    if (e->wg_head) hipFree(e->wg_head);
    if (e->gran) hipFree(e->gran);
    if (e->fail) hipFree(e->fail);
    if (e->stamps) hipFree(e->stamps);
    delete e;
}

int32_t wrk_v7_engine_enqueue(wrk_v7_engine* e, hipStream_t q, wrk_v7_state* st, uint32_t batch, uint32_t l0, uint32_t l1, const void* x_in, void* x_out,
                              void* v_first, const uint32_t* token) {
    using namespace wrk;
    wrk_ctx* ctx = e->m->ctx;
    EngArgs A{};
    A.S = e->S;
    A.S.layer_begin = l0; A.S.layer_end = l1; A.S.batch = batch;
    A.layers = e->layers; A.vecs = e->vecs; A.scal = e->scal; A.gran = e->gran; A.x_in = x_in; A.x_out = x_out; A.v_first = v_first;
    if (token && e->emb_ln && l0 == 0) { A.x_in = e->emb_ln; A.x_row = token; }
    A.state = st->data; A.num_batch = st->num_batch; A.fail = e->fail; A.stamps = e->stamps; A.stamp_layer = std::min(5u, l1 - 1);
    WRK_HIP(ctx, hipMemsetAsync(e->gran, 0, (size_t)e->S.g_total * 8, q));
    const dim3 grid(e->S.nwg), block((e->ncw + 2) * 64);
    hipLaunchKernelGGL(eng_kernel(e->xd, e->r16, e->ncw), grid, block, e->S.lds_total, q, A, (const uint32_t*)e->wg_head);
    WRK_LAUNCH_CHECK(ctx);
    return WRK_OK;
}

int32_t wrk_v7_engine_check(wrk_v7_engine* e) {
    if (!e) return WRK_OK;
    wrk_ctx* ctx = e->m->ctx;
    uint32_t f = 0;
    WRK_HIP(ctx, hipMemcpy(&f, e->fail, 4, hipMemcpyDeviceToHost));
    if (f) {
        hipMemset(e->fail, 0, 4);
        return wrk_fail(ctx, WRK_E_HIP, "decode engine: a hand-off wait gave up (stage mask 0x%x): workgroups not co-resident or a producer died", f);
    }
    return WRK_OK;
}

void wrk_v7_engine_report(wrk_v7_engine* e) {
    using namespace wrk;
    if (!e || !e->stamps) return;
    const uint32_t NWG = e->S.nwg, NW = (uint32_t)e->ncw + 2;
    std::vector<unsigned long long> h((size_t)NWG * NW * 24);
    if (hipMemcpy(h.data(), e->stamps, h.size() * 8, hipMemcpyDeviceToHost) != hipSuccess) return;
    unsigned long long t0 = ~0ull;
    for (auto v : h) if (v && v < t0) t0 = v;
    auto col = [&](int wave, uint32_t k, const char* label) {
        std::vector<double> v;
        for (uint32_t w = 0; w < NWG; ++w) {
            unsigned long long x = 0;
            if (wave >= 0) x = h[((size_t)w * NW + wave) * 24 + k];
            else for (int cw = 0; cw < e->ncw; ++cw) x = std::max(x, h[((size_t)w * NW + cw) * 24 + k]);
            if (x) v.push_back((double)(x - t0) * 0.01);
        }
        if (v.empty()) return;
        std::sort(v.begin(), v.end());
        fprintf(stderr, "  %-62s %4zu WGs  first %7.2f  median %7.2f  last %7.2f us\n", label, v.size(), v.front(), v[v.size() / 2], v.back());
    };
    {
        unsigned long long tail[2] = {0, 0};
        if (hipMemcpy(tail, e->stamps + (size_t)NWG * 16 * 24, 16, hipMemcpyDeviceToHost) == hipSuccess && tail[1])
            fprintf(stderr, "[WRK_TIMING] decode engine: shader clock over the last launch %.0f MHz (%llu cycles in %.1f us)\n",
                    (double)tail[0] / ((double)tail[1] * 0.01), tail[0], (double)tail[1] * 0.01);
    }
    const int G = e->ncw, Ld = e->ncw + 1;
    fprintf(stderr, "[WRK_TIMING] decode engine (%d compute waves), one layer of the last token; us since the layer's first stamp\n", e->ncw);
    col(G, 0, "gather: layer input complete");
    col(0, 1, "K1 start (input + weights in LDS), wave 0");
    col(0, 2, "K1 LN + shift done, wave 0");
    col(0, 3, "K1 rows published, wave 0");
    col(-1, 3, "K1 rows published, slowest wave");
    col(G, 1, "gather (heads): K1 outputs complete");
    col(0, 4, "K2 start");
    col(-1, 16, "K2 LoRA dots done, slowest wave");
    col(0, 17, "K2 per-channel stage done");
    col(-1, 18, "K2 state updated, slowest wave");
    col(0, 5, "K2 published");
    col(G, 2, "gather: head outputs complete");
    col(0, 6, "K3 start");
    col(-1, 7, "K3 published, slowest wave");
    col(G, 3, "gather: x1 complete");
    col(0, 8, "K5 start");
    col(0, 14, "K5 LN + shift done, wave 0");
    col(0, 9, "K5 published, wave 0");
    col(-1, 9, "K5 published, slowest wave");
    col(0, 10, "K6 own quarter of the ffn vector swept, wave 0");
    col(-1, 10, "K6 swept, slowest wave");
    col(0, 11, "K6 start");
    col(-1, 12, "K6 partial sums done, slowest wave");
    col(0, 13, "K6 published");
    col(Ld, 0, "loader: K1 slot free, next layer's fill issued");
}
```

web-rwkv-gguf_amd/csrc/wrk_v7_fused.hip:

```cpp
#include "wrk_device.h"
#include "wrk_v7.h"
#include "wrk_v7_engine.h"
#include "wrk_lora_dev.h"

namespace wrk {

__global__ void advance_tokens_kernel(const uint32_t* __restrict__ argmax, uint32_t* __restrict__ tokens,
                                      uint32_t* __restrict__ history, uint32_t* __restrict__ counter, uint32_t b) {
    const uint32_t step = *counter;
    const uint32_t i = threadIdx.x;
    if (i < b) {
        const uint32_t t = argmax[i];
        tokens[i] = t;
        history[(size_t)step * b + i] = t;
    }
    __syncthreads();
    if (i == 0) *counter = step + 1;
}

void advance_tokens(hipStream_t s, const uint32_t* argmax, uint32_t* tokens, uint32_t* history, uint32_t* counter, uint32_t b) {
    advance_tokens_kernel<<<1, 256, 0, s>>>(argmax, tokens, history, counter, b);
}

template <int VPT, int NMIX>
__global__ void __launch_bounds__(256) ln_mix_kernel(const LnMixParams P) {
    __shared__ float red[4];
    const uint32_t t = blockIdx.x, D = P.d, nvec = D >> 3, tid = threadIdx.x;
    const size_t rowi = P.ids ? P.ids[t] : t;
    const uint32_t batch = P.batch1 ? P.batch1 - 1 + t : (P.cursors ? (P.cursors[t] & 0xffu) : t);
    const f16* row = P.src + rowi * D;
    const float* st = P.state_row ? P.state_row + (size_t)batch * P.state_stride : (const float*)P.ln_w;
    f16x8 xv[VPT], wv[VPT], bv[VPT], mv[NMIX > 0 ? NMIX : 1][VPT];
    f32x4 pv[VPT][2];
#pragma unroll
    for (int v = 0; v < VPT; ++v) {
        const uint32_t i = min(tid + 256u * v, nvec - 1);
        xv[v] = *(const f16x8*)(row + i * 8);
        wv[v] = *(const f16x8*)(P.ln_w + i * 8);
        bv[v] = *(const f16x8*)(P.ln_b + i * 8);
        if (NMIX > 0) {
            pv[v][0] = *(const f32x4*)(st + i * 8);
            pv[v][1] = *(const f32x4*)(st + i * 8 + 4);
#pragma unroll
            for (int m = 0; m < NMIX; ++m) mv[m][v] = *(const f16x8*)(P.mix[m] + i * 8);
        }
    }
    float s = 0.0f;
#pragma unroll
    for (int v = 0; v < VPT; ++v)
        if (tid + 256 * v < nvec)
#pragma unroll
            for (int e = 0; e < 8; ++e) s += (float)xv[v][e];
    const float mean = block_sum<4>(s, red) / (float)D;
    float q = 0.0f;
#pragma unroll
    for (int v = 0; v < VPT; ++v)
        if (tid + 256 * v < nvec)
#pragma unroll
            for (int e = 0; e < 8; ++e) { const float dl = (float)xv[v][e] - mean; q += dl * dl; }
    const float var = block_sum<4>(q, red) / (float)D + P.eps;
    const float dev = 1.0f / sqrtf(var);
#pragma unroll
    for (int v = 0; v < VPT; ++v) {
        const uint32_t i = tid + 256 * v;
        if (i >= nvec) continue;
        float y[8];
        f16x8 yv;
#pragma unroll
        for (int e = 0; e < 8; ++e) {
            const float value = ((float)xv[v][e] - mean) * dev;
            yv[e] = (f16)__builtin_fmaf(value, (float)wv[v][e], (float)bv[v][e]);
            y[e] = (float)yv[e];
        }
        if (P.ln_out) *(f16x8*)(P.ln_out + (size_t)t * D + i * 8) = yv;
        if (NMIX > 0) {
#pragma unroll
            for (int m = 0; m < NMIX; ++m) {
                f16x8 o;
#pragma unroll
                for (int e = 0; e < 8; ++e) o[e] = (f16)wgsl_mix(y[e], pv[v][e >> 2][e & 3], (float)mv[m][v][e]);
                *(f16x8*)(P.out[m] + (size_t)t * D + i * 8) = o;
            }
            if (!P.no_carry) {
                f32x4 n0 = {y[0], y[1], y[2], y[3]}, n1 = {y[4], y[5], y[6], y[7]};
                float* sw = P.state_row + (size_t)batch * P.state_stride;
                *(f32x4*)(sw + i * 8) = n0;
                *(f32x4*)(sw + i * 8 + 4) = n1;
            }
        }
    }
}

int ln_mix(hipStream_t s, const LnMixParams& P, uint32_t T) {
    const uint32_t nvec = P.d >> 3;
    const int vpt = nvec <= 256 ? 1 : (nvec <= 512 ? 2 : (nvec <= 1024 ? 4 : 0));
    if (vpt == 0 || (P.d & 7u)) return -1;
#define LN_LAUNCH(V, M) ln_mix_kernel<V, M><<<T, 256, 0, s>>>(P)
#define LN_SWITCH(M) do { if (vpt == 1) LN_LAUNCH(1, M); else if (vpt == 2) LN_LAUNCH(2, M); else LN_LAUNCH(4, M); } while (0)
    if (P.nmix == 0) LN_SWITCH(0);
    else if (P.nmix == 1) LN_SWITCH(1);
    else if (P.nmix == 2) LN_SWITCH(2);
    else if (P.nmix == 6) LN_SWITCH(6);
    else return -1;
#undef LN_SWITCH
#undef LN_LAUNCH
    return 0;
}

struct HeadParams {
    uint32_t d, layer0;
    uint32_t rw, ra, rg, rv;
    const f16 *w2, *a2, *g2, *v2;
    uint32_t w2_rb, a2_rb, g2_rb, v2_rb;
    const f16 *w0, *a0, *v0;
    const f16 *k_k, *k_a, *r_k, *gn_w, *gn_b;
    const f16 *aux_w, *aux_a, *aux_g, *aux_v;
    const f16 *r, *k, *v;
    f16* v_first;
    f16* out;
    float* state;
    const uint32_t* cursors;
    const f16* shift_src;
    float gn_eps, l2_eps;
    uint32_t batch1;
    unsigned long long* dbg;
};

template <int GCH>
__global__ void __launch_bounds__(256) head_kernel(const HeadParams P) {
    constexpr int S = 64;
    __shared__ float sh_r[S], sh_w[S], sh_k[S], sh_v[S], sh_a[S], sh_b[S], sh_g[S], sh_kk[S];
    __shared__ float sh_red[4][S];
    const uint32_t head = blockIdx.x, t = blockIdx.y, tid = threadIdx.x;
    const uint32_t D = P.d;
    const uint32_t c0 = head * S;
    const uint32_t i = tid & 63, g4 = tid >> 6;
    WRK_STAMP(P.dbg, 0);

    const uint32_t row = tid >> 2, part = tid & 3u, ch = c0 + row;
    LoraRegs<4> lw, la, lv;
    LoraRegs<GCH> lg;
    lora_load<4>(lw, (const f16*)((const uint8_t*)P.w2 + (size_t)ch * P.w2_rb), P.aux_w + (size_t)t * P.rw, P.rw, part);
    lora_load<4>(la, (const f16*)((const uint8_t*)P.a2 + (size_t)ch * P.a2_rb), P.aux_a + (size_t)t * P.ra, P.ra, part);
    lora_load<GCH>(lg, (const f16*)((const uint8_t*)P.g2 + (size_t)ch * P.g2_rb), P.aux_g + (size_t)t * P.rg, P.rg, part);
    if (!P.layer0) lora_load<4>(lv, (const f16*)((const uint8_t*)P.v2 + (size_t)ch * P.v2_rb), P.aux_v + (size_t)t * P.rv, P.rv, part);
    const float w0 = (float)P.w0[ch], a0 = (float)P.a0[ch], kkw = (float)P.k_k[ch], kaw = (float)P.k_a[ch];
    const float kraw = (float)P.k[(size_t)t * D + ch], rraw = (float)P.r[(size_t)t * D + ch];
    float v = (float)P.v[(size_t)t * D + ch];
    const f16 v0h = (P.layer0 ? P.w0 : P.v0)[ch], vfh = P.v_first[(size_t)t * D + ch];
    const float v0w = P.layer0 ? 0.0f : (float)v0h, vfirst = P.layer0 ? 0.0f : (float)vfh;
    const float gnw = (float)P.gn_w[c0 + i], gnb = (float)P.gn_b[c0 + i], rkw = (float)P.r_k[c0 + i];
    const float shift = (float)(P.shift_src ? P.shift_src + (size_t)t * D : P.w0)[c0 + i];

    const uint32_t batch = P.batch1 ? P.batch1 - 1 + t : (P.cursors[t] & 0xffu);
    float* st = P.state + ((size_t)batch * (S + 2) + 1) * D + c0 + i;
    float Sreg[16];
#pragma unroll
    for (int jj = 0; jj < 16; ++jj) Sreg[jj] = st[(size_t)(g4 * 16 + jj) * D];

    {
        const float dw = lora_dot<4>(lw, P.rw, part);
        const float da = lora_dot<4>(la, P.ra, part);
        const float dg = lora_dot<GCH>(lg, P.rg, part);
        float dv = 0.0f;
        if (!P.layer0) dv = lora_dot<4>(lv, P.rv, part);
        if (part == 0) {
            const float w = r16(w0 + r16(dw));
            const float a = r16(act_sigmoid(a0 + r16(da)));
            const float g = r16(dg);
            if (P.layer0) P.v_first[(size_t)t * D + ch] = (f16)v;
            else {
                const float vv = r16(act_sigmoid(v0w + r16(dv)));
                v = r16(wgsl_mix(v, vfirst, vv));
// ... 243 lines not shown
    return g_timing.dev + (g_timing.labels.size() - 1) * 16;
}
void wrk::timing_report(wrk_ctx* ctx) {
    if (!g_timing.enabled || !g_timing.dev || g_timing.labels.empty()) return;
    std::vector<unsigned long long> h(64 * 16);
    hipMemcpy(h.data(), g_timing.dev, h.size() * 8, hipMemcpyDeviceToHost);
    unsigned long long t0 = ~0ull;
    for (size_t i = 0; i < g_timing.labels.size() * 16; ++i) if (h[i] && h[i] < t0) t0 = h[i];
    fprintf(stderr, "[WRK_TIMING] layer %u of the last decode step; ns since the first stamp (100 MHz clock); first WG | last WG\n", TIMED_LAYER);
    for (size_t i = 0; i < g_timing.labels.size(); ++i) {
        fprintf(stderr, "  %-40s", g_timing.labels[i].c_str());
        for (int w = 0; w < 2; ++w) {
            for (int k = 0; k < 5; ++k) {
                const unsigned long long v = h[i * 16 + w * 8 + k];
                if (v) fprintf(stderr, " %6llu", (v - t0) * 10); else fprintf(stderr, "      -");
            }
            if (w == 0) fprintf(stderr, "  |");
        }
        fprintf(stderr, "\n");
    }
}

void wrk_v7_model::free_fused() {
    if (amax_val) hipFree(amax_val);
    if (amax_idx) hipFree(amax_idx);
    amax_val = nullptr; amax_idx = nullptr; amax_cap = 0;
}

int32_t wrk_v7_model::enqueue_fused_decode(wrk_v7_state* st, uint32_t T, uint32_t NH, bool identity_headers, bool from_tokens,
                                            bool want_argmax, bool advance, uint32_t cursor0_batch, bool contiguous) {
    using namespace wrk;
    hipStream_t q = ctx->op_stream();
    const uint32_t D = d.num_emb, F = d.num_hidden, H = d.num_head, S = D / H, V = d.num_vocab;
    bool ok = (D % 8 == 0) && D <= 8192 && d.lora_w % 8 == 0 && d.lora_a % 8 == 0 && d.lora_g % 8 == 0 && d.lora_v % 8 == 0 &&
              d.lora_w <= 128 && d.lora_a <= 128 && d.lora_v <= 128 && d.lora_g <= 512;
    for (auto& L : layers) {
        const wrk_matrix* ms[] = {L.w2, L.a2, L.g2, L.v2};
        for (const wrk_matrix* m : ms)
            if (m && m->kind != WRK_MAT_F16) ok = false;
    }
    if (!ok) {
        if (from_tokens) gather_rows_f16(q, emb->ptr, s.tokens, s.input, D, T);
        int32_t rc = enqueue_ops(st, T, NH, identity_headers);
        if (rc != WRK_OK) return rc;
        if (want_argmax && NH) {
            argmax_rows(q, s.head_o, V, V, NH, s.argmax);
            if (advance) advance_tokens(q, s.argmax, s.tokens, history, s.counter, NH);
        }
        return WRK_OK;
    }
    auto vec = [&](void* p, uint32_t c = 0) { return make_dense(p, WRK_F16, c ? c : D, T); };
    bool single = false;
    auto run_jobs = [&](MatJob* jobs, int n) -> int {
        if (!single && T >= gemm_min_tokens()) {
            jobs[0].ks_part = s.ks_part; jobs[0].ks_cnt = s.ks_cnt; jobs[0].ks_part_cap = s.ks_part_cap; jobs[0].ks_cnt_cap = s.ks_cnt_cap;
            jobs[0].xsum = ctx->gemm_scratch; jobs[0].xsum_cap = ctx->gemm_scratch_cap;
            if (matmul_mfma_multi(q, jobs, n, ctx->num_cu) == 0) return 0;
            for (int i = 0; i < n; ++i) {
                int rc = matmul_mfma(q, jobs[i], ctx->num_cu);
                if (rc == -2) rc = matvec(q, &jobs[i], 1, ctx->num_cu);
                if (rc != 0) return rc;
            }
            return 0;
        }
        return matvec_grouped(q, jobs, n, ctx->num_cu);
    };
#define LN(P, n)                                                                             \
    do {                                                                                     \
        if (ln_mix(q, P, n) != 0) return wrk_fail(ctx, WRK_E_UNSUPPORTED, "ln_mix shape");   \
    } while (0)

    if (T >= 2 && s.ks_cnt && s.ks_cnt_cap) WRK_HIP(ctx, hipMemsetAsync(s.ks_cnt, 0, (size_t)s.ks_cnt_cap * 4, q));
    const bool eng_embeds = T == 1 && from_tokens && !skip_embed && layer_begin == 0 && engine_on() && !engine_skip_once && wrk_v7_engine_has_table(engine) &&
                            d.num_layer > 0;
    if (!skip_embed && !eng_embeds) {
        LnMixParams P{};
        if (from_tokens) { P.src = (const f16*)emb->ptr; P.ids = s.tokens; }
        else P.src = (const f16*)s.input;
        P.ln_w = (const f16*)ln0_w->ptr; P.ln_b = (const f16*)ln0_b->ptr; P.eps = 1.0e-5f;
        P.d = D; P.nmix = 0; P.ln_out = (f16*)s.x;
        LN(P, T);
    }
    uint32_t first_launch_layer = layer_begin;
    if (T == 1 && engine_on() && !engine_skip_once) {
        const uint32_t l1 = std::min<uint32_t>(d.num_layer, layer_end);
        if (layer_begin < l1) {
            const int32_t rc = wrk_v7_engine_enqueue(engine, q, st, cursor0_batch, layer_begin, l1, s.x, s.x, s.att_v0, eng_embeds ? s.tokens : nullptr);
            if (rc != WRK_OK) return rc;
        }
        first_launch_layer = l1;
    }
    for (uint32_t li = first_launch_layer; li < d.num_layer && li < layer_end; ++li) {
        const wrk_v7_layer_desc& L = layers[li];
        float* lst = st->layer_ptr(li);
        static const bool fuse_ln = [] { const char* e = getenv("WRK_FUSE_LN"); return !(e && e[0] == '0'); }();
        static const uint32_t few_max = [] { const char* e = getenv("WRK_DMV_TOKENS"); const int v = e ? atoi(e) : 4; return (uint32_t)(v < 1 ? 1 : (v > 4 ? 4 : v)); }();
        single = fuse_ln && (T == 1 || (T <= few_max && contiguous)) && D <= 4096;
        if (single) {
            MatJob k1[7] = {mat_job(L.w_r, vec(s.x), vec(s.r), 0), mat_job(L.w_k, vec(s.x), vec(s.k), 0), mat_job(L.w_v, vec(s.x), vec(s.v), 0),
                            mat_job(L.w1, vec(s.x), vec(s.aux_w, d.lora_w), 0), mat_job(L.a1, vec(s.x), vec(s.aux_a, d.lora_a), 0),
                            mat_job(L.g1, vec(s.x), vec(s.aux_g, d.lora_g), 0), mat_job(li ? L.v1 : L.a1, vec(s.x), vec(s.aux_v, d.lora_v), 0)};
            for (MatJob& j : k1) j.pro = 1;
            MatJob k5 = mat_job(L.ffn_w_k, vec(s.x), vec(s.ffn_k, F), 0);
            k5.pro = 1;
            MatJob k6 = mat_job(L.ffn_w_v, vec(s.ffn_k, F), vec(s.x), 0);
            k6.has_res = 1; k6.res = vec(s.x);
            k6.carry_dst = (float*)s.x;
            single = matvec_grouped(q, k1, li ? 7 : 6, ctx->num_cu, true) == 0 && matvec(q, &k5, 1, ctx->num_cu, true) == 0 &&
                     matvec(q, &k6, 1, ctx->num_cu, true) == 0;
        }
        const bool want_split = split_head_env_on() && !(T == 1 && engine != nullptr && engine_env_on_public() && !engine_skip_once);
        const uint32_t state_stride = (S + 2) * D;
        bool split_head = want_split && single && d.lora_w >= 8 && d.lora_a >= 8 && d.lora_g >= 8 && d.lora_v >= 8 && d.lora_g <= 512;
        if (split_head) {
            MatJob k3 = mat_job(L.w_o, vec(s.att_x), vec(s.x), 0);
            k3.has_res = 1; k3.res = vec(s.x);
            k3.pro = 2; k3.ln_w = L.gn_w->ptr; k3.ln_b = L.gn_b->ptr; k3.mixw = s.g; k3.prev = (const float*)s.n;
            split_head = matvec(q, &k3, 1, ctx->num_cu, true) == 0;
        }
        uint32_t batch0 = 0;
        if (single) batch0 = cursor0_batch;
        float* row0 = lst + (size_t)batch0 * (S + 2) * D;
        if (!single) {
            LnMixParams P{};
            P.src = (const f16*)s.x; P.ln_w = (const f16*)L.ln1_w->ptr; P.ln_b = (const f16*)L.ln1_b->ptr; P.eps = 1.0e-5f;
            P.d = D; P.nmix = 6;
            const wrk_buf* mx[6] = {L.x_r, L.x_w, L.x_k, L.x_v, L.x_a, L.x_g};
            void* outs[6] = {s.rx, s.wx, s.kx, s.vx, s.ax, s.gx};
            for (int i = 0; i < 6; ++i) { P.mix[i] = (const f16*)mx[i]->ptr; P.out[i] = (f16*)outs[i]; }
            P.state_row = lst; P.state_stride = (size_t)(S + 2) * D; P.cursors = s.cursors; P.batch1 = contiguous ? cursor0_batch + 1 : 0;
            LN(P, T);
        }
        {
            MatJob jobs[7] = {mat_job(L.w_r, vec(s.rx), vec(s.r), WRK_ACT_NONE), mat_job(L.w_k, vec(s.kx), vec(s.k), WRK_ACT_NONE),
                              mat_job(L.w_v, vec(s.vx), vec(s.v), WRK_ACT_NONE),
                              mat_job(L.w1, vec(s.wx), vec(s.aux_w, d.lora_w), WRK_ACT_TANH),
                              mat_job(L.a1, vec(s.ax), vec(s.aux_a, d.lora_a), WRK_ACT_NONE),
                              mat_job(L.g1, vec(s.gx), vec(s.aux_g, d.lora_g), WRK_ACT_SIGMOID),
                              mat_job(li ? L.v1 : L.a1, vec(s.vx), vec(s.aux_v, d.lora_v), WRK_ACT_NONE)};
            if (single) {
                const wrk_buf* mx[7] = {L.x_r, L.x_k, L.x_v, L.x_w, L.x_a, L.x_g, L.x_v};
                for (int i = 0; i < 7; ++i) {
                    jobs[i].in = vec(s.x);
                    jobs[i].pro = 1; jobs[i].pro_eps = 1.0e-5f; jobs[i].ln_w = L.ln1_w->ptr; jobs[i].ln_b = L.ln1_b->ptr;
                    jobs[i].mixw = mx[i]->ptr; jobs[i].prev = row0; jobs[i].tok_prev_stride = state_stride;
                }
                jobs[0].ln_out = s.ln_tmp;
            }
            if (li == TIMED_LAYER) jobs[0].dbg = jobs[(li ? 7 : 6) - 1].dbg = wrk::timing_slot(ctx, "K1 r,k,v + LoRA-1 (LN1 prologue)");
            const int rc = run_jobs(jobs, li ? 7 : 6);
            if (rc != 0) return wrk_fail(ctx, WRK_E_ARG, "fused K1 rejected (%d)", rc);
        }
        {
            HeadParams P{};
            P.d = D; P.layer0 = li == 0;
            P.rw = d.lora_w; P.ra = d.lora_a; P.rg = d.lora_g; P.rv = d.lora_v;
            P.w2 = (const f16*)L.w2->data; P.a2 = (const f16*)L.a2->data; P.g2 = (const f16*)L.g2->data;
            P.w2_rb = (uint32_t)L.w2->row_bytes; P.a2_rb = (uint32_t)L.a2->row_bytes; P.g2_rb = (uint32_t)L.g2->row_bytes;
            if (li) { P.v2 = (const f16*)L.v2->data; P.v2_rb = (uint32_t)L.v2->row_bytes; P.v0 = (const f16*)L.v0->ptr; }
            P.w0 = (const f16*)L.w0->ptr; P.a0 = (const f16*)L.a0->ptr;
            P.k_k = (const f16*)L.k_k->ptr; P.k_a = (const f16*)L.k_a->ptr; P.r_k = (const f16*)L.r_k->ptr;
            P.gn_w = (const f16*)L.gn_w->ptr; P.gn_b = (const f16*)L.gn_b->ptr;
            P.aux_w = (const f16*)s.aux_w; P.aux_a = (const f16*)s.aux_a; P.aux_g = (const f16*)s.aux_g; P.aux_v = (const f16*)s.aux_v;
            P.r = (const f16*)s.r; P.k = (const f16*)s.k; P.v = (const f16*)s.v;
            P.v_first = (f16*)s.att_v0; P.out = (f16*)s.att_x;
            P.state = lst; P.cursors = s.cursors; P.gn_eps = 64.0e-5f; P.l2_eps = 1.0e-12f;
            P.shift_src = single ? (const f16*)s.ln_tmp : nullptr;
            P.batch1 = (single || contiguous) ? cursor0_batch + 1 : 0;
            P.dbg = li == TIMED_LAYER ? wrk::timing_slot(ctx, "K2 head: LoRA-2 + WKV7 + group norm") : nullptr;
            if (split_head) {
                if (d.lora_g <= 256) head_split_kernel<2><<<dim3(H * 4, T), 256, 0, q>>>(P, (float*)s.n, (f16*)s.g, H);
                else head_split_kernel<4><<<dim3(H * 4, T), 256, 0, q>>>(P, (float*)s.n, (f16*)s.g, H);
            }
            else if (d.lora_g <= 256) head_kernel<8><<<dim3(H, T), 256, 0, q>>>(P);
            else head_kernel<16><<<dim3(H, T), 256, 0, q>>>(P);
        }
        {
            MatJob j = mat_job(L.w_o, vec(s.att_x), vec(s.x), WRK_ACT_NONE);
            j.has_res = 1; j.res = vec(s.x);
            if (split_head) {
                j.pro = 2; j.pro_eps = 64.0e-5f; j.ln_w = L.gn_w->ptr; j.ln_b = L.gn_b->ptr; j.mixw = s.g; j.prev = (const float*)s.n;
                j.tok_mix_stride = D; j.tok_prev_stride = D;
            }
            if (li == TIMED_LAYER) j.dbg = wrk::timing_slot(ctx, "K3 w_o + residual");
            if (run_jobs(&j, 1) != 0) return wrk_fail(ctx, WRK_E_ARG, "fused K3 rejected");
        }
        float* rowf = lst + ((size_t)batch0 * (S + 2) + (S + 1)) * D;
        if (!single) {
            LnMixParams P{};
            P.src = (const f16*)s.x; P.ln_w = (const f16*)L.ln2_w->ptr; P.ln_b = (const f16*)L.ln2_b->ptr; P.eps = 1.0e-5f;
            P.d = D; P.nmix = 1; P.mix[0] = (const f16*)L.ffn_x_k->ptr; P.out[0] = (f16*)s.ffn_kx;
            P.state_row = lst + (size_t)(S + 1) * D; P.state_stride = (size_t)(S + 2) * D; P.cursors = s.cursors; P.batch1 = contiguous ? cursor0_batch + 1 : 0;
            LN(P, T);
        }
        {
            MatJob j = mat_job(L.ffn_w_k, vec(s.ffn_kx), vec(s.ffn_k, F), WRK_ACT_SQUARED_RELU);
            if (single) {
                j.in = vec(s.x);
                j.pro = 1; j.pro_eps = 1.0e-5f; j.ln_w = L.ln2_w->ptr; j.ln_b = L.ln2_b->ptr; j.mixw = L.ffn_x_k->ptr; j.prev = rowf;
                j.tok_prev_stride = state_stride;
                j.ln_out = s.ffn_x;
            }
            if (li == TIMED_LAYER) j.dbg = wrk::timing_slot(ctx, "K5 ffn key (LN2 prologue)");
            if (run_jobs(&j, 1) != 0) return wrk_fail(ctx, WRK_E_ARG, "fused K5 rejected");
        }
        {
            MatJob j = mat_job(L.ffn_w_v, vec(s.ffn_k, F), vec(s.x), WRK_ACT_NONE);
            j.has_res = 1; j.res = vec(s.x);
            if (single) { j.carry_src = s.ffn_x; j.carry_dst = rowf; j.tok_carry_src_stride = D; j.tok_carry_dst_stride = state_stride; }
            if (li == TIMED_LAYER) j.dbg = wrk::timing_slot(ctx, "K6 ffn value + residual");
            if (run_jobs(&j, 1) != 0) return wrk_fail(ctx, WRK_E_ARG, "fused K6 rejected");
        }
        if ((li + 1) % d.rescale == 0) wrk::affine(q, vec(s.x), 0.5f, 0.0f);
    }
    if (NH > 0) {
        LnMixParams P{};
        P.src = (const f16*)s.x; P.ids = identity_headers ? nullptr : s.headers;
        P.ln_w = (const f16*)ln_out_w->ptr; P.ln_b = (const f16*)ln_out_b->ptr; P.eps = 1.0e-5f;
        P.d = D; P.nmix = 0; P.ln_out = (f16*)s.head_x;
        LN(P, NH);
        MatJob j = mat_job(head, make_dense(s.head_x, WRK_F16, D, NH), make_dense(s.head_o, WRK_F32, V, NH), WRK_ACT_NONE);
        uint32_t nwg = 0;
        bool head_mv = NH < gemm_min_tokens();
        if (!head_mv && NH <= 4) {
            MatJob probe = j;
            if (want_argmax) { probe.amax_val = amax_val; probe.amax_idx = amax_idx; }
            head_mv = (size_t)matvec_num_wg(&j, 1, ctx->num_cu, nullptr) * NH <= amax_cap && matvec(q, &probe, 1, ctx->num_cu, true, false, true) == 0;
        }
        if (!head_mv && matmul_mfma(q, j, ctx->num_cu) == 0) {
            if (want_argmax) {
                wrk::argmax_rows(q, (const float*)s.head_o, V, V, NH, s.argmax);
                if (advance) wrk::advance_tokens(q, s.argmax, s.tokens, history, s.counter, NH);
            }
        } else {
            if (want_argmax) {
                nwg = matvec_num_wg(&j, 1, ctx->num_cu, nullptr);
                if ((size_t)nwg * NH > amax_cap) return wrk_fail(ctx, WRK_E_ARG, "arg-max scratch too small");
                j.amax_val = amax_val; j.amax_idx = amax_idx;
            }
            if (matvec(q, &j, 1, ctx->num_cu) != 0) return wrk_fail(ctx, WRK_E_ARG, "fused head rejected");
            if (want_argmax)
                argmax_finish(q, amax_val, amax_idx, nwg, NH, s.argmax, advance ? s.tokens : nullptr, history, advance ? s.counter : nullptr);
        }
    }
#undef LN
    WRK_LAUNCH_CHECK(ctx);
    return WRK_OK;
}
```

web-rwkv-gguf_amd/wrk/__init__.py:

```python
from __future__ import annotations

import ctypes as C
import os
from typing import Dict, List, Optional, Sequence

import numpy as np

_HERE = os.path.dirname(os.path.abspath(__file__))
_LIBDIR = os.environ.get("WRK_LIB_DIR") or os.path.join(os.path.dirname(_HERE), "lib")
LIB_HIP = os.path.join(_LIBDIR, "libwrk_hip.so")
LIB_RT = os.path.join(_LIBDIR, "libwrk_runtime.so")


class WrkError(RuntimeError):
    def __init__(self, code: int, msg: str):
        super().__init__(f"[{STATUS.get(code, code)}] {msg}")
        self.code = code


OK, E_ARG, E_OOM, E_HIP, E_UNSUPPORTED = 0, 1, 2, 3, 4
STATUS = {0: "WRK_OK", 1: "WRK_E_ARG", 2: "WRK_E_OOM", 3: "WRK_E_HIP", 4: "WRK_E_UNSUPPORTED"}
F16, F32, U8, U32 = 0, 1, 2, 3
ACT = {"none": 0, "squared_relu": 1, "tanh": 2, "stable_exp": 3, "opposite_exp": 4, "softplus": 5, "sigmoid": 6, "silu": 7}
MAT = {"F32": 0, "F16": 1, "Q8_0": 8, "Q4_K": 12, "Q5_K": 13, "Q6_K": 14, "INT8": 100, "NF4": 101}
# ... 18 lines not shown
class TensorDesc(C.Structure):
    _fields_ = [("buf", C.c_void_p), ("dtype", C.c_uint32), ("view", View)]


class ModelInfo(C.Structure):
    _fields_ = [(n, C.c_uint32) for n in ("version", "num_layer", "num_emb", "num_hidden", "num_vocab", "num_head",
                                           "lora_w", "lora_a", "lora_g", "lora_v")]

    def as_dict(self):
        return {n: getattr(self, n) for n, _ in self._fields_}


class BuildOptions(C.Structure):
    _fields_ = [("rescale", C.c_uint32), ("weights", C.c_uint32), ("quant", C.POINTER(C.c_uint8)), ("num_quant", C.c_uint32)]


_P = C.c_void_p
_u32p = C.POINTER(C.c_uint32)
_i32p = C.POINTER(C.c_int32)
_f32p = C.POINTER(C.c_float)


class GenerateOptions(C.Structure):
    _fields_ = [("temperature", _f32p), ("top_p", _f32p), ("seed", _u32p), ("presence", _f32p), ("frequency", _f32p), ("decay", _f32p),
                ("occ", _P), ("stop_tokens", _u32p), ("stop_offsets", _u32p), ("poll_steps", C.c_uint32)]


MAX_STOP_TOKENS = 16
_TP = C.POINTER(TensorDesc)

HIP_SYMBOLS = {
    "wrk_abi_version": (C.c_int32, []),
    "wrk_ctx_create": (C.c_int32, [C.c_int32, C.POINTER(_P)]),
    "wrk_ctx_destroy": (C.c_int32, [_P]),
    "wrk_last_error": (C.c_char_p, [_P]),
    "wrk_ctx_sync": (C.c_int32, [_P]),
    "wrk_ctx_stream": (_P, [_P]),
    "wrk_buf_create": (C.c_int32, [_P, C.c_size_t, _P, C.POINTER(_P)]),
    "wrk_buf_retain": (C.c_int32, [_P]),
    "wrk_buf_release": (C.c_int32, [_P]),
    "wrk_buf_size": (C.c_size_t, [_P]),
    "wrk_buf_device_ptr": (_P, [_P]),
    "wrk_buf_write": (C.c_int32, [_P, _P, C.c_size_t, _P, C.c_size_t]),
    "wrk_buf_read": (C.c_int32, [_P, _P, C.c_size_t, _P, C.c_size_t]),
    "wrk_buf_copy": (C.c_int32, [_P, _P, C.c_size_t, _P, C.c_size_t, C.c_size_t]),
    "wrk_capture_begin": (C.c_int32, [_P]),
    "wrk_capture_end": (C.c_int32, [_P, C.POINTER(_P)]),
    "wrk_program_launch": (C.c_int32, [_P, _P]),
    "wrk_program_destroy": (C.c_int32, [_P]),
    "wrk_matrix_create": (C.c_int32, [_P, C.c_uint32, C.c_uint32, C.c_uint32, _P, C.c_size_t, C.c_uint32, C.POINTER(_P)]),
    "wrk_matrix_quantize": (C.c_int32, [_P, C.c_uint32, C.c_uint32, C.c_uint32, _P, C.POINTER(C.c_float), C.POINTER(_P)]),
    "wrk_matrix_export": (C.c_int32, [_P, _P, C.c_size_t, C.POINTER(C.c_size_t)]),
    "wrk_matrix_set_scale": (C.c_int32, [_P, C.c_float]),
    "wrk_matrix_release": (C.c_int32, [_P]),
    "wrk_matrix_stream_bytes": (C.c_size_t, [_P]),
    "wrk_op_matmul": (C.c_int32, [_P, _P, _TP, _TP, C.c_uint32, C.c_int32, C.c_int32]),
    "wrk_op_layer_norm": (C.c_int32, [_P, _P, _P, _TP, C.c_float]),
    "wrk_op_group_norm": (C.c_int32, [_P, _P, _P, _TP, C.c_float]),
    "wrk_op_l2_norm": (C.c_int32, [_P, _TP, C.c_float]),
    "wrk_op_token_shift": (C.c_int32, [_P, _P, _TP, _TP, _TP, _TP, C.c_int32]),
    "wrk_op_add": (C.c_int32, [_P, _TP, _TP, C.c_uint32, C.c_uint32, C.c_uint32]),
    "wrk_op_mul": (C.c_int32, [_P, _TP, _TP, C.c_uint32, C.c_uint32, C.c_uint32]),
    "wrk_op_lerp": (C.c_int32, [_P, _TP, _TP, _TP, C.c_int32]),
    "wrk_op_blit": (C.c_int32, [_P, _TP, _TP]),
    "wrk_op_affine": (C.c_int32, [_P, _TP, C.c_float, C.c_float]),
    "wrk_op_activate": (C.c_int32, [_P, _TP, C.c_uint32]),
    "wrk_op_control_k_v7": (C.c_int32, [_P, _P, _TP, _TP]),
    "wrk_op_time_mix_v7": (C.c_int32, [_P, _P, _TP, _TP, _TP, _TP, _TP]),
    "wrk_op_time_first_v7": (C.c_int32, [_P, _P, _TP, _TP, _TP]),
    "wrk_op_channel_mix_v7": (C.c_int32, [_P, _P, _TP, _TP, _TP]),
    "wrk_op_softmax": (C.c_int32, [_P, _TP]),
    "wrk_v7_model_create": (C.c_int32, [_P, _P, C.POINTER(_P)]),
    "wrk_v7_model_destroy": (C.c_int32, [_P]),
    "wrk_v7_model_token_bytes": (C.c_size_t, [_P, C.c_uint32]),
    "wrk_v7_state_create": (C.c_int32, [_P, _P, C.c_uint32, C.POINTER(_P)]),
    "wrk_v7_state_destroy": (C.c_int32, [_P]),
    "wrk_v7_state_load": (C.c_int32, [_P, _P, C.c_uint32, _f32p]),
    "wrk_v7_state_read": (C.c_int32, [_P, _P, C.c_uint32, _P]),
    "wrk_v7_state_write": (C.c_int32, [_P, _P, C.c_uint32, _P]),
    "wrk_v7_state_back": (C.c_int32, [_P, _P, C.c_uint32, _f32p]),
    "wrk_v7_infer": (C.c_int32, [_P, _P, _P, _u32p, C.POINTER(C.c_uint16), _u32p, C.c_uint32, _u32p, C.c_uint32, _f32p, _u32p, C.c_uint32]),
    "wrk_v7_model_set_frame_dtype": (C.c_int32, [_P, _P, C.c_uint32]),
    "wrk_v7_model_engine_status": (C.c_int32, [_P, _P, C.c_char_p, C.c_size_t]),
    "wrk_v7_infer_layer": (C.c_int32, [_P, _P, _P, C.c_uint32, _P, _P, _u32p, C.c_uint32, C.c_uint32]),
    "wrk_v7_frame_read": (C.c_int32, [_P, _P, C.c_char_p, C.c_uint32, _P, C.c_size_t, C.POINTER(C.c_size_t)]),
    "wrk_v7_generate_greedy": (C.c_int32, [_P, _P, _P, _u32p, C.c_uint32, C.c_uint32, _u32p, _f32p, _f32p, C.c_uint32]),
    "wrk_op_transpose": (C.c_int32, [_P, _TP, _TP]),
    "wrk_op_time_mix_v6": (C.c_int32, [_P, _P, _TP, _P, _TP, _TP, _TP, _TP, _TP]),
    "wrk_op_channel_mix": (C.c_int32, [_P, _P, _TP, _TP, _TP, _TP]),
    "wrk_v6_model_create": (C.c_int32, [_P, _P, C.POINTER(_P)]),
    "wrk_v6_model_destroy": (C.c_int32, [_P]),
    "wrk_v6_model_token_bytes": (C.c_size_t, [_P, C.c_uint32]),
    "wrk_v6_state_create": (C.c_int32, [_P, _P, C.c_uint32, C.POINTER(_P)]),
    "wrk_v6_infer": (C.c_int32, [_P, _P, _P, _u32p, C.POINTER(C.c_uint16), _u32p, C.c_uint32, _u32p, C.c_uint32, _f32p, _u32p, C.c_uint32]),
    "wrk_v6_generate_greedy": (C.c_int32, [_P, _P, _P, _u32p, C.c_uint32, C.c_uint32, _u32p, _f32p, _f32p, C.c_uint32]),
    "wrk_sample_logits": (C.c_int32, [_P, _P, C.c_uint32, C.c_uint32, C.c_uint32, _f32p, _f32p, _u32p, C.c_uint32, _u32p]),
    "wrk_v7_generate_sample": (C.c_int32, [_P, _P, _P, _u32p, C.c_uint32, C.c_uint32, _f32p, _f32p, _u32p, _u32p, _f32p, _f32p,
                                           C.c_uint32]),
    "wrk_v6_generate_sample": (C.c_int32, [_P, _P, _P, _u32p, C.c_uint32, C.c_uint32, _f32p, _f32p, _u32p, _u32p, _f32p, _f32p,
                                           C.c_uint32]),
    "wrk_score_logits": (C.c_int32, [_P, _P, C.c_uint32, C.c_uint32, C.c_uint32, _u32p, _f32p, _u32p]),
    "wrk_v7_score": (C.c_int32, [_P, _P, _P, _u32p, C.POINTER(C.c_uint16), _u32p, C.c_uint32, _u32p, C.c_uint32, _u32p, _f32p, _u32p,
                                 C.c_uint32]),
    "wrk_v6_score": (C.c_int32, [_P, _P, _P, _u32p, C.POINTER(C.c_uint16), _u32p, C.c_uint32, _u32p, C.c_uint32, _u32p, _f32p, _u32p,
                                 C.c_uint32]),
    "wrk_occurrence_create": (C.c_int32, [_P, C.c_uint32, C.c_uint32, C.POINTER(_P)]),
    "wrk_occurrence_destroy": (C.c_int32, [_P]),
    "wrk_occurrence_set_weights": (C.c_int32, [_P, _P, _f32p]),
    "wrk_occurrence_ban": (C.c_int32, [_P, _P, C.c_uint32, _u32p, C.c_uint32, C.c_int32]),
    "wrk_occurrence_add": (C.c_int32, [_P, _P, C.c_uint32, _u32p, C.c_uint32, C.c_float]),
    "wrk_occurrence_back": (C.c_int32, [_P, _P, C.c_uint32, _f32p, _u32p]),
    "wrk_occurrence_load": (C.c_int32, [_P, _P, C.c_uint32, _f32p, _u32p]),
    "wrk_penalize_logits": (C.c_int32, [_P, _P, C.c_uint32, C.c_uint32, C.c_uint32, _P, C.c_uint32, _f32p, _f32p]),
    "wrk_v7_generate_penalized": (C.c_int32, [_P, _P, _P, _u32p, C.c_uint32, C.c_uint32, _f32p, _f32p, _u32p, _f32p, _f32p, _f32p, _P,
                                              _u32p, _f32p, _f32p, C.c_uint32]),
    "wrk_v6_generate_penalized": (C.c_int32, [_P, _P, _P, _u32p, C.c_uint32, C.c_uint32, _f32p, _f32p, _u32p, _f32p, _f32p, _f32p, _P,
                                              _u32p, _f32p, _f32p, C.c_uint32]),
    "wrk_v7_generate_stop": (C.c_int32, [_P, _P, _P, _u32p, C.c_uint32, C.c_uint32, C.POINTER(GenerateOptions), _u32p, _u32p, _f32p, _u32p,
                                         _f32p, C.c_uint32]),
    "wrk_v6_generate_stop": (C.c_int32, [_P, _P, _P, _u32p, C.c_uint32, C.c_uint32, C.POINTER(GenerateOptions), _u32p, _u32p, _f32p, _u32p,
                                         _f32p, C.c_uint32]),
}
RT_SYMBOLS = {
    "wrk_host_last_error": (C.c_char_p, []),
    "wrk_gguf_open": (C.c_int32, [C.c_char_p, C.POINTER(_P)]),
    "wrk_gguf_from_memory": (C.c_int32, [_P, C.c_size_t, C.POINTER(_P)]),
    "wrk_gguf_close": (C.c_int32, [_P]),
    "wrk_gguf_version": (C.c_uint32, [_P]),
    "wrk_gguf_tensor_data_offset": (C.c_uint64, [_P]),
    "wrk_gguf_contains": (C.c_int32, [_P, C.c_char_p]),
    "wrk_gguf_shape": (C.c_int32, [_P, C.c_char_p, C.c_uint32 * 4, _u32p]),
    "wrk_gguf_tensor_f16": (C.c_int32, [_P, C.c_char_p, C.POINTER(C.c_uint16), C.c_size_t, C.POINTER(C.c_size_t)]),
    "wrk_gguf_raw": (C.c_int32, [_P, C.c_char_p, _u32p, C.POINTER(_P), C.POINTER(C.c_size_t)]),
    "wrk_gguf_meta_u64": (C.c_int32, [_P, C.c_char_p, C.POINTER(C.c_uint64)]),
    "wrk_gguf_read_state": (C.c_int32, [_P, _f32p, C.c_size_t, C.POINTER(C.c_size_t)]),
    "wrk_gguf_info": (C.c_int32, [_P, C.POINTER(ModelInfo)]),
    "wrk_quantile_student": (C.c_int32, [C.c_double, _f32p]),
    "wrk_rnn_input_create": (C.c_int32, [C.c_uint32, C.c_uint32, C.POINTER(_P)]),
    "wrk_rnn_input_destroy": (C.c_int32, [_P]),
    "wrk_rnn_input_token_chunk_size": (C.c_uint32, [_P]),
    "wrk_rnn_input_append": (C.c_int32, [_P, C.c_uint32, _u32p, C.c_uint32]),
    "wrk_rnn_input_set_option": (C.c_int32, [_P, C.c_uint32, C.c_int32]),
    "wrk_rnn_input_remaining": (C.c_uint32, [_P, C.c_uint32]),
    "wrk_rnn_input_step": (C.c_int32, [_P]),
    "wrk_rnn_iter_create": (C.c_int32, [_P, C.POINTER(_P)]),
    "wrk_rnn_iter_destroy": (C.c_int32, [_P]),
    "wrk_rnn_iter_next": (C.c_int32, [_P, _u32p, _i32p]),
    "wrk_rnn_redirect": (C.c_int32, [_u32p, _i32p, C.c_uint32, _u32p, _u32p, _u32p, _u32p]),
    "wrk_runtime_create": (C.c_int32, [_P, _P, C.POINTER(BuildOptions), C.c_uint32, C.POINTER(_P)]),
    "wrk_runtime_destroy": (C.c_int32, [_P]),
    "wrk_runtime_info": (C.c_int32, [_P, C.POINTER(ModelInfo)]),
    "wrk_runtime_model": (_P, [_P]),
    "wrk_runtime_state": (_P, [_P]),
    "wrk_runtime_model_v6": (_P, [_P]),
    "wrk_runtime_infer": (C.c_int32, [_P, _P, _f32p, C.c_size_t, _u32p, C.c_uint32]),
    "wrk_rnn_score_plan": (C.c_int32, [_P, _u32p, _u32p, _u32p, _u32p, _u32p]),
    "wrk_runtime_score": (C.c_int32, [_P, _P, _f32p, _u32p, C.c_size_t, _u32p, C.c_uint32]),
}
for _lib, _tab in ((hip, HIP_SYMBOLS), (rt, RT_SYMBOLS)):
    for _name, (_res, _args) in _tab.items():
        _f = getattr(_lib, _name)
        _f.restype = _res
        _f.argtypes = _args


def _u32(a) -> np.ndarray:
# ... 549 lines not shown
            q = np.zeros(max(quant) + 1, np.uint8)
            for l, v in quant.items():
                q[l] = v
            opt.quant, opt.num_quant = q.ctypes.data_as(C.POINTER(C.c_uint8)), q.size
        h = _P()
        _host_check(rt.wrk_runtime_create(ctx.h, reader.h, C.byref(opt), num_batch, C.byref(h)))
        self.ctx, self.h, self.num_batch = ctx, h, num_batch
        self.info = ModelInfo()
        rt.wrk_runtime_info(h, C.byref(self.info))
        self.model = rt.wrk_runtime_model(h)
        self.model6 = rt.wrk_runtime_model_v6(h)
        self.state = rt.wrk_runtime_state(h)

    def token_bytes(self, num_batch: int = 1) -> int:
        if self.model6:
            return hip.wrk_v6_model_token_bytes(self.model6, num_batch)
        return hip.wrk_v7_model_token_bytes(self.model, num_batch)

    def infer(self, inp: RnnInput, mode: int = 1) -> List[np.ndarray]:
        V = self.info.num_vocab
        cap = inp.token_chunk_size + inp.num_batch
        logits = np.empty((cap, V), dtype=np.float32)
        rows = np.zeros(inp.num_batch, np.uint32)
        _host_check(rt.wrk_runtime_infer(self.h, inp.h, _ptr(logits, _f32p), cap, _ptr(rows, _u32p), mode))
        out, p = [], 0
        for b in range(inp.num_batch):
            out.append(logits[p:p + rows[b]].copy())
            p += int(rows[b])
        return out

    def score(self, inp: RnnInput, mode: int = 1):
        cap = inp.token_chunk_size + inp.num_batch
        lp = np.empty(cap, np.float32)
        rk = np.empty(cap, np.uint32)
        rows = np.zeros(inp.num_batch, np.uint32)
        _host_check(rt.wrk_runtime_score(self.h, inp.h, _ptr(lp, _f32p), _ptr(rk, _u32p), cap, _ptr(rows, _u32p), mode))
        out, p = [], 0
        for b in range(inp.num_batch):
            out.append((lp[p:p + rows[b]].copy(), rk[p:p + rows[b]].copy()))
            p += int(rows[b])
        return out

    def score_sequences(self, seqs, token_chunk_size: int = 128, mode: int = 1):
        inp = RnnInput(seqs, token_chunk_size)
        lps = [[] for _ in seqs]
        rks = [[] for _ in seqs]
        while any(inp.remaining(b) for b in range(inp.num_batch)):
            for b, (lp, rk) in enumerate(self.score(inp, mode)):
                lps[b].append(lp)
                rks[b].append(rk)
        return [(np.concatenate(l) if l else np.zeros(0, np.float32), np.concatenate(r) if r else np.zeros(0, np.uint32))
                for l, r in zip(lps, rks)]

    def score_raw(self, tokens, cursors, headers, targets, mode: int = 1):
        t, c, h, tg = _u32(tokens), _u32(cursors), _u32(headers), _u32(targets)
        lp = np.zeros(max(h.size, 1), np.float32)
        rk = np.zeros(max(h.size, 1), np.uint32)
        fn, mdl = (hip.wrk_v6_score, self.model6) if self.model6 else (hip.wrk_v7_score, self.model)
        self.ctx.check(fn(self.ctx.h, mdl, self.state, _ptr(t, _u32p), None, _ptr(c, _u32p), t.size, _ptr(h, _u32p), h.size,
                          _ptr(tg, _u32p) if tg.size else None, _ptr(lp, _f32p), _ptr(rk, _u32p), mode))
        return lp[: h.size], rk[: h.size]

    def infer_raw(self, tokens, cursors, headers, mode: int = 1, want_argmax: bool = False):
        t, c, h = _u32(tokens), _u32(cursors), _u32(headers)
        V = self.info.num_vocab
        logits = np.empty((max(h.size, 1), V), np.float32)
        am = np.zeros(max(h.size, 1), np.uint32)
        fn, mdl = (hip.wrk_v6_infer, self.model6) if self.model6 else (hip.wrk_v7_infer, self.model)
        self.ctx.check(fn(self.ctx.h, mdl, self.state, _ptr(t, _u32p), None, _ptr(c, _u32p), t.size,
                          _ptr(h, _u32p), h.size, _ptr(logits, _f32p), _ptr(am, _u32p) if want_argmax else None, mode))
        return (logits[: h.size], am[: h.size]) if want_argmax else logits[: h.size]

    def set_frame_dtype(self, dtype: int):
        self.ctx.check(hip.wrk_v7_model_set_frame_dtype(self.ctx.h, self.model, dtype))
        self.frame_dtype = dtype

    def engine_status(self):
        buf = C.create_string_buffer(512)
        rc = hip.wrk_v7_model_engine_status(self.ctx.h, self.model, buf, 512)
        if rc < 0:
            self.ctx.check(rc)
        return rc == 1, buf.value.decode()

    def infer_layer(self, layer: int, x: np.ndarray, v_first: Optional[np.ndarray], cursors, mode: int = 0):
        dt = np.float32 if getattr(self, "frame_dtype", F16) == F32 else np.float16
        xa = np.ascontiguousarray(x, dtype=dt)
        va = np.ascontiguousarray(v_first, dtype=dt) if v_first is not None else None
        c = _u32(cursors)
        self.ctx.check(hip.wrk_v7_infer_layer(self.ctx.h, self.model, self.state, layer, xa.ctypes.data_as(_P),
                                              va.ctypes.data_as(_P) if va is not None else None, _ptr(c, _u32p), c.size, mode))

    def frame(self, name: str, num_token: int) -> np.ndarray:
        dt = np.float32 if getattr(self, "frame_dtype", F16) == F32 else np.float16
        n = C.c_size_t()
        self.ctx.check(hip.wrk_v7_frame_read(self.ctx.h, self.model, name.encode(), num_token, None, 0, C.byref(n)))
        out = np.empty(n.value // np.dtype(dt).itemsize, dt)
        self.ctx.check(hip.wrk_v7_frame_read(self.ctx.h, self.model, name.encode(), num_token, out.ctypes.data_as(_P), out.nbytes, C.byref(n)))
        return out.reshape(num_token, -1)

    def generate_greedy(self, first_tokens, steps: int, mode: int = 1, want_logits: bool = False, groups: int = 1):
        mode = (mode & 0xff) | ((groups & 0xff) << 8 if groups > 1 and not self.model6 else 0)
        ft = _u32(first_tokens)
        B = ft.size
        out = np.zeros((steps, B), np.uint32)
        ms = C.c_float()
        logits = np.empty((B, self.info.num_vocab), np.float32) if want_logits else None
        fn, mdl = (hip.wrk_v6_generate_greedy, self.model6) if self.model6 else (hip.wrk_v7_generate_greedy, self.model)
        self.ctx.check(fn(self.ctx.h, mdl, self.state, _ptr(ft, _u32p), B, steps, _ptr(out, _u32p),
                          _ptr(logits, _f32p) if want_logits else None, C.byref(ms), mode))
        return (out, ms.value, logits) if want_logits else (out, ms.value)

    def generate_sample(self, first_tokens, steps: int, temperature=1.0, top_p=0.5, seed=None, mode: int = 1, want_logits: bool = False,
                        groups: int = 1):
        mode = (mode & 0xff) | ((groups & 0xff) << 8 if groups > 1 and not self.model6 else 0)
        ft = _u32(first_tokens)
        B = ft.size
        t, p = _per_row(temperature, B, np.float32), _per_row(top_p, B, np.float32)
        sd = np.arange(B, dtype=np.uint32) if seed is None else _per_row(seed, B, np.uint32)
        out = np.zeros((steps, B), np.uint32)
        ms = C.c_float()
        logits = np.empty((B, self.info.num_vocab), np.float32) if want_logits else None
        fn, mdl = (hip.wrk_v6_generate_sample, self.model6) if self.model6 else (hip.wrk_v7_generate_sample, self.model)
        self.ctx.check(fn(self.ctx.h, mdl, self.state, _ptr(ft, _u32p), B, steps, _ptr(t, _f32p), _ptr(p, _f32p), _ptr(sd, _u32p),
                          _ptr(out, _u32p), _ptr(logits, _f32p) if want_logits else None, C.byref(ms), mode))
        return (out, ms.value, logits) if want_logits else (out, ms.value)

    def generate_penalized(self, first_tokens, steps: int, occurrence: "Occurrence", temperature=1.0, top_p=0.5, seed=None, presence=0.0,
                           frequency=0.0, decay=1.0, mode: int = 1, want_logits: bool = False, groups: int = 1):
        mode = (mode & 0xff) | ((groups & 0xff) << 8 if groups > 1 and not self.model6 else 0)
        ft = _u32(first_tokens)
        B = ft.size
        t, p = _per_row(temperature, B, np.float32), _per_row(top_p, B, np.float32)
        sd = np.arange(B, dtype=np.uint32) if seed is None else _per_row(seed, B, np.uint32)
        ap, af, g = _per_row(presence, B, np.float32), _per_row(frequency, B, np.float32), _per_row(decay, B, np.float32)
        out = np.zeros((steps, B), np.uint32)
        ms = C.c_float()
        logits = np.empty((B, self.info.num_vocab), np.float32) if want_logits else None
        fn, mdl = (hip.wrk_v6_generate_penalized, self.model6) if self.model6 else (hip.wrk_v7_generate_penalized, self.model)
        self.ctx.check(fn(self.ctx.h, mdl, self.state, _ptr(ft, _u32p), B, steps, _ptr(t, _f32p), _ptr(p, _f32p), _ptr(sd, _u32p),
                          _ptr(ap, _f32p), _ptr(af, _f32p), _ptr(g, _f32p), occurrence.h, _ptr(out, _u32p),
                          _ptr(logits, _f32p) if want_logits else None, C.byref(ms), mode))
        return (out, ms.value, logits) if want_logits else (out, ms.value)

    def generate_stop(self, first_tokens, steps: int, stop, temperature=None, top_p=None, seed=None, occurrence: "Occurrence" = None,
                      presence=0.0, frequency=0.0, decay=1.0, mode: int = 1, want_logits: bool = False, groups: int = 1,
                      poll_steps: int = 0):
        mode = (mode & 0xff) | ((groups & 0xff) << 8 if groups > 1 and not self.model6 else 0)
        ft = _u32(first_tokens)
        B = ft.size
        sets = list(stop)
        if not (sets and all(isinstance(x, (list, tuple, np.ndarray)) for x in sets)):
            sets = [sets] * B
        if len(sets) != B:
            raise ValueError(f"{len(sets)} stop sets for {B} sequences")
        off = np.zeros(B + 1, np.uint32)
        off[1:] = np.cumsum([len(x) for x in sets])
        ids = _u32(np.concatenate([np.asarray(x, np.int64).reshape(-1) for x in sets]) if B else [])
        if ids.size == 0:
            ids = np.zeros(1, np.uint32)
        opt = GenerateOptions()
        keep = []
        sampled = temperature is not None or top_p is not None or seed is not None or occurrence is not None
        if sampled:
            t = _per_row(1.0 if temperature is None else temperature, B, np.float32)
            p = _per_row(0.5 if top_p is None else top_p, B, np.float32)
            sd = np.arange(B, dtype=np.uint32) if seed is None else _per_row(seed, B, np.uint32)
# ... 44 lines not shown
```

Baseline: 1666 tokens/s.

## Replace per-token granule memset with epoch tags and add engine scheduling levers

```diff
diff --git a/include/wrk_hip.h b/include/wrk_hip.h
--- a/include/wrk_hip.h
+++ b/include/wrk_hip.h
@@ -162,6 +162,7 @@
 int32_t wrk_v7_model_set_frame_dtype(wrk_ctx* ctx, wrk_v7_model* model, uint32_t dtype);
 
 int32_t wrk_v7_model_engine_status(wrk_ctx* ctx, wrk_v7_model* model, char* why, size_t capacity);
+int32_t wrk_v7_model_engine_debug(wrk_ctx* ctx, wrk_v7_model* model, uint32_t set_epoch, uint32_t prefill_stale);
 
 int32_t wrk_v7_infer_layer(wrk_ctx* ctx, wrk_v7_model* model, wrk_v7_state* state, uint32_t layer, const void* x, const void* v_first,
                            const uint32_t* cursors, uint32_t num_token, uint32_t mode);
diff --git a/web-rwkv-gguf_amd/csrc/wrk_runner.h b/web-rwkv-gguf_amd/csrc/wrk_runner.h
--- a/web-rwkv-gguf_amd/csrc/wrk_runner.h
+++ b/web-rwkv-gguf_amd/csrc/wrk_runner.h
@@ -44,6 +44,9 @@
     const uint32_t* cursors;
     uint32_t batch1;
     uint32_t no_carry;
+    uint32_t* eng_epoch;
+    unsigned long long* eng_gran;
+    uint32_t eng_ngran;
 };
 int ln_mix(hipStream_t s, const LnMixParams& P, uint32_t T);
 }
diff --git a/web-rwkv-gguf_amd/csrc/wrk_v7.hip b/web-rwkv-gguf_amd/csrc/wrk_v7.hip
--- a/web-rwkv-gguf_amd/csrc/wrk_v7.hip
+++ b/web-rwkv-gguf_amd/csrc/wrk_v7.hip
@@ -506,10 +506,21 @@
     const int32_t rc = m->ensure_engine();
     if (rc != WRK_OK) return rc;
     if (why && capacity) {
-        const std::string& w = m->engine ? std::string() : (m->engine_tried ? m->engine_why : std::string("disabled (WRK_ENGINE=0 or f32 frames)"));
+        const std::string& w = m->engine ? wrk_v7_engine_levers(m->engine) : (m->engine_tried ? m->engine_why : std::string("disabled (WRK_ENGINE=0 or f32 frames)"));
         snprintf(why, capacity, "%s", w.c_str());
     }
     return m->engine ? 1 : 0;
+}
+
+int32_t wrk_v7_model_engine_debug(wrk_ctx* ctx, wrk_v7_model* m, uint32_t set_epoch, uint32_t prefill_stale) {
+    if (!ctx || !m) return WRK_E_ARG;
+    LOCK(ctx);
+    WRK_HIP(ctx, hipSetDevice(ctx->device));
+    WRK_ARG(ctx, !ctx->capturing_here(), "not inside a capture");
+    const int32_t rc = m->ensure_engine();
+    if (rc != WRK_OK) return rc;
+    WRK_ARG(ctx, m->engine != nullptr, "this model has no decode engine");
+    return wrk_v7_engine_debug(m->engine, set_epoch, prefill_stale);
 }
 
 int32_t wrk_v7_infer_layer(wrk_ctx* ctx, wrk_v7_model* m, wrk_v7_state* st, uint32_t layer, const void* x, const void* v_first,
diff --git a/web-rwkv-gguf_amd/csrc/wrk_v7_engine.h b/web-rwkv-gguf_amd/csrc/wrk_v7_engine.h
--- a/web-rwkv-gguf_amd/csrc/wrk_v7_engine.h
+++ b/web-rwkv-gguf_amd/csrc/wrk_v7_engine.h
@@ -1,5 +1,7 @@
 #pragma once
 #include <stdint.h>
+
+#include <string>
 
 #include "wrk_internal.h"
 
@@ -7,6 +9,8 @@
 
 constexpr int ENG_K1_JOBS = 7;
 constexpr uint32_t ENG_NO_HEAD = 0xffffffffu;
+constexpr uint32_t ENG_TAG_BITS = 11;
+constexpr uint32_t ENG_EPOCH_MAX = (1u << (32 - ENG_TAG_BITS)) - 1u;
 
 struct EngJob {
     uint32_t rows, row_bytes, f16;
@@ -29,6 +33,8 @@
     uint32_t layer_begin, layer_end, rescale;
     uint32_t batch, state_rows;
     uint32_t x_from_granules;
+    uint32_t deal, k1_rb6;
+    uint32_t k6_share, k6x[4];
 };
 
 struct EngLayer {
@@ -46,6 +52,7 @@
     const void* vecs;
     const float* scal;
     unsigned long long* gran;
+    const uint32_t* epoch;
     const void* x_in;
     const uint32_t* x_row;
     void* x_out;
@@ -58,6 +65,22 @@
 };
 constexpr int ENG_STAMPS = 32;
 
+struct EngEpoch {
+    uint32_t* epoch;
+    unsigned long long* gran;
+    uint32_t ngran;
+};
+#if defined(__HIPCC__)
+__device__ __forceinline__ void eng_epoch_advance(const EngEpoch& E) {
+    const uint32_t e = E.epoch[0];
+    const bool wrap = e >= ENG_EPOCH_MAX;
+    if (wrap)
+        for (uint32_t i = threadIdx.x; i < E.ngran; i += blockDim.x) E.gran[i] = 0ull;
+    __syncthreads();
+    if (threadIdx.x == 0) E.epoch[0] = wrap ? 1u : e + 1u;
+}
+#endif
+
 }
 
 struct wrk_v7_model;
@@ -66,7 +89,9 @@
 int32_t wrk_v7_engine_create(wrk_v7_model* m, wrk_v7_engine** out);
 void wrk_v7_engine_destroy(wrk_v7_engine* e);
 int32_t wrk_v7_engine_enqueue(wrk_v7_engine* e, hipStream_t q, wrk_v7_state* st, uint32_t batch, uint32_t l0, uint32_t l1, const void* x_in,
-                              void* x_out, void* v_first, const uint32_t* token = nullptr);
+                              void* x_out, void* v_first, const uint32_t* token = nullptr, wrk::EngEpoch* advance = nullptr);
+int32_t wrk_v7_engine_debug(wrk_v7_engine* e, uint32_t set_epoch, uint32_t prefill_stale);
 bool wrk_v7_engine_has_table(const wrk_v7_engine* e);
+std::string wrk_v7_engine_levers(const wrk_v7_engine* e);
 int32_t wrk_v7_engine_check(wrk_v7_engine* e);
 void wrk_v7_engine_report(wrk_v7_engine* e);
diff --git a/web-rwkv-gguf_amd/csrc/wrk_v7_engine.hip b/web-rwkv-gguf_amd/csrc/wrk_v7_engine.hip
--- a/web-rwkv-gguf_amd/csrc/wrk_v7_engine.hip
+++ b/web-rwkv-gguf_amd/csrc/wrk_v7_engine.hip
@@ -16,7 +16,13 @@
 
 constexpr uint32_t ENG_SPIN_MAX = 1u << 21;
 
-__device__ __forceinline__ uint32_t eng_tag(uint32_t layer, uint32_t stage) { return layer * 8u + stage + 1u; }
+__device__ __forceinline__ uint32_t eng_tag(uint32_t ep, uint32_t layer, uint32_t stage) { return ep | (layer * 8u + stage + 1u); }
+
+template <int N>
+__device__ __forceinline__ void eng_bars() {
+#pragma unroll
+    for (int i = 0; i < N; ++i) asm volatile("s_waitcnt lgkmcnt(0)\n\ts_barrier" ::: "memory");
+}
 
 __device__ __forceinline__ void eng_store_granule(unsigned long long* g, uint32_t tag, uint32_t payload) {
     __hip_atomic_store(g, ((unsigned long long)tag << 32) | payload, __ATOMIC_RELAXED, __HIP_MEMORY_SCOPE_AGENT);
@@ -192,7 +198,7 @@
         }
         x_sums<KIND>(x[0][ci]);
     }
-    static_assert(RB == 2 || RB == 4, "rows per batch");
+    static_assert(RB == 2 || RB == 4 || RB == 6, "rows per batch");
     for (uint32_t ri = r_begin; ri < r_end; ri += RB) {
         Raw raw[RB][XI];
 #pragma unroll
@@ -201,7 +207,7 @@
 #pragma unroll
             for (int ci = 0; ci < XI; ++ci) raw[rb][ci] = lds_raw<KIND>(rowp, K, min(lane + 64u * ci, nch - 1));
         }
-        float v[4] = {0.0f, 0.0f, 0.0f, 0.0f};
+        float v[RB];
 #pragma unroll
         for (int rb = 0; rb < RB; ++rb) {
             float acc[1] = {0.0f};
@@ -212,8 +218,12 @@
         if (lane < RB / 2) {
             const uint32_t ra = ri + 2 * lane;
             if (ra < r_end) {
-                const float o0 = eng_finish(fin, row0 + ra, lane ? v[2] : v[0]) * fin.post;
-                const float o1 = eng_finish(fin, row0 + ra + 1, lane ? v[3] : v[1]) * fin.post;
+                float va = v[0], vb = v[1];
+#pragma unroll
+                for (int p = 1; p < RB / 2; ++p)
+                    if (lane == (uint32_t)p) { va = v[2 * p]; vb = v[2 * p + 1]; }
+                const float o0 = eng_finish(fin, row0 + ra, va) * fin.post;
+                const float o1 = eng_finish(fin, row0 + ra + 1, vb) * fin.post;
                 if (pub) pub[ra >> 1] = pack_h2(o0, o1);
                 else eng_store_granule(gran + gidx(row0 + ra), tag, pack_h2(o0, o1));
             }
@@ -272,7 +282,18 @@
     ENG_BAR();
 }
 
+constexpr int ENG_K1_BARRIERS = 4;
 constexpr int ENG_K2_BARRIERS = 6;
+constexpr int ENG_K3_BARRIERS = 2;
+constexpr int ENG_K5_BARRIERS = 5;
+constexpr int ENG_K6_BARRIERS = 3;
+constexpr int ENG_LN_BARRIERS = 2;
+#define ENG_CBAR(i, N)                                                        \
+    do {                                                                      \
+        static_assert((i) >= 1 && (i) <= (N), "barrier outside its stage");   \
+        ENG_BAR();                                                            \
+    } while (0)
+static_assert(1 + ENG_LN_BARRIERS + 1 == ENG_K1_BARRIERS && 1 + ENG_LN_BARRIERS + 2 == ENG_K5_BARRIERS, "LN barriers inside K1 / K5");
 template <int XD, bool R16, int QK, int NCW>
 __global__ void __launch_bounds__((NCW + 2) * 64) v7_engine_kernel(const EngArgs A, const uint32_t* __restrict__ wg_head) {
     extern __shared__ __attribute__((aligned(16))) unsigned char eng_smem_generic[];
@@ -282,6 +303,7 @@
     const uint32_t wave = (uint32_t)__builtin_amdgcn_readfirstlane((int)(tid_all >> 6));
     const uint32_t wg = blockIdx.x;
     const uint32_t D = S.D, F = S.F;
+    const uint32_t ep = A.epoch[0] << ENG_TAG_BITS;
     const uint32_t head = wg_head[2 * wg], k1r = wg_head[2 * wg + 1];
     const bool is_head = head != ENG_NO_HEAD;
     ENG_LDS uint32_t* abort_flag = (ENG_LDS uint32_t*)(smem + S.lds_misc + 1008);
@@ -344,29 +366,28 @@
             ENG_BAR();
             if (*abort_flag) break;
             if (p6) { fill6(l); p6 = false; }
-            ENG_BAR(); ENG_BAR(); ENG_BAR();
+            eng_bars<ENG_K1_BARRIERS - 1>();
             ENG_STAMP(l, 0);
             if (more) fill1(l + 1);
             if (is_head) {
                 ENG_BAR();
                 if (*abort_flag) break;
-#pragma unroll
-                for (int i = 1; i < ENG_K2_BARRIERS; ++i) ENG_BAR();
+                eng_bars<ENG_K2_BARRIERS - 1>();
             }
             eng_wait_vm(issued - m3);
             ENG_BAR();
             if (*abort_flag) break;
-            ENG_BAR();
+            eng_bars<ENG_K3_BARRIERS - 1>();
             eng_wait_vm(issued - m5);
             ENG_BAR();
             if (*abort_flag) break;
             if (more) fill3(l + 1);
-            ENG_BAR(); ENG_BAR(); ENG_BAR(); ENG_BAR();
+            eng_bars<ENG_K5_BARRIERS - 1>();
             eng_wait_vm(issued - m6);
             ENG_BAR();
             if (*abort_flag) break;
             if (more) fill5(l + 1);
-            ENG_BAR(); ENG_BAR();
+            eng_bars<ENG_K6_BARRIERS - 1>();
             p6 = more;
             ENG_FLUSH(l);
         }
@@ -379,37 +400,36 @@
         for (uint32_t l = S.layer_begin; l < S.layer_end; ++l) {
             bool ok = true;
             if (l == S.layer_begin) eng_copy_in(A.x_row ? (const void*)((const f16*)A.x_in + (size_t)A.x_row[0] * D) : A.x_in, D >> 3, (ENG_LDS u32x4*)xraw0, lane);
-            else ok = eng_gather(A.gran + S.g_x, D >> 2, eng_tag(l - 1, 4), (ENG_LDS uint32_t*)xraw0, lane);
+            else ok = eng_gather(A.gran + S.g_x, D >> 2, eng_tag(ep, l - 1, 4), (ENG_LDS uint32_t*)xraw0, lane);
             if (!ok && lane == 0) { *abort_flag = 1; atomicOr(A.fail, 1u); }
             ENG_STAMP(l, 0);
             ENG_BAR();
             if (*abort_flag) break;
-            ENG_BAR(); ENG_BAR(); ENG_BAR();
+            eng_bars<ENG_K1_BARRIERS - 1>();
             if (is_head) {
-                ok = eng_gather(A.gran + S.g_k1, (l == 0 ? naux - S.rv : naux) >> 2, eng_tag(l, 0), (ENG_LDS uint32_t*)auxbuf, lane);
-                if (ok) ok = eng_gather(A.gran + S.g_k1 + S.g_aux + head * 96u, 48u, eng_tag(l, 0), (ENG_LDS uint32_t*)(auxbuf + naux), lane);
+                ok = eng_gather(A.gran + S.g_k1, (l == 0 ? naux - S.rv : naux) >> 2, eng_tag(ep, l, 0), (ENG_LDS uint32_t*)auxbuf, lane);
+                if (ok) ok = eng_gather(A.gran + S.g_k1 + S.g_aux + head * 96u, 48u, eng_tag(ep, l, 0), (ENG_LDS uint32_t*)(auxbuf + naux), lane);
                 if (!ok && lane == 0) { *abort_flag = 1; atomicOr(A.fail, 2u); }
                 ENG_STAMP(l, 1);
                 ENG_BAR();
                 if (*abort_flag) break;
-#pragma unroll
-                for (int i = 1; i < ENG_K2_BARRIERS; ++i) ENG_BAR();
-            }
-            ok = eng_gather(A.gran + S.g_o, D >> 2, eng_tag(l, 1), (ENG_LDS uint32_t*)xs, lane);
+                eng_bars<ENG_K2_BARRIERS - 1>();
+            }
+            ok = eng_gather(A.gran + S.g_o, D >> 2, eng_tag(ep, l, 1), (ENG_LDS uint32_t*)xs, lane);
             if (!ok && lane == 0) { *abort_flag = 1; atomicOr(A.fail, 4u); }
             ENG_STAMP(l, 2);
             ENG_BAR();
             if (*abort_flag) break;
-            ENG_BAR();
-            ok = eng_gather(A.gran + S.g_x1, D >> 2, eng_tag(l, 2), (ENG_LDS uint32_t*)xraw1, lane);
+            eng_bars<ENG_K3_BARRIERS - 1>();
+            ok = eng_gather(A.gran + S.g_x1, D >> 2, eng_tag(ep, l, 2), (ENG_LDS uint32_t*)xraw1, lane);
             if (!ok && lane == 0) { *abort_flag = 1; atomicOr(A.fail, 8u); }
             ENG_STAMP(l, 3);
             ENG_BAR();
             if (*abort_flag) break;
-            ENG_BAR(); ENG_BAR(); ENG_BAR(); ENG_BAR();
+            eng_bars<ENG_K5_BARRIERS - 1>();
             ENG_BAR();
             if (*abort_flag) break;
-            ENG_BAR(); ENG_BAR();
+            eng_bars<ENG_K6_BARRIERS - 1>();
             ENG_FLUSH(l);
         }
         return;
@@ -422,9 +442,17 @@
     const float eps = S.ln_eps;
     const bool ln_wave = wave < 4;
     auto wave_rows = [&](uint32_t nrows, uint32_t& b, uint32_t& e) {
-        const uint32_t q = 2u * (((nrows + 1u) / 2u + NCW - 1u) / NCW);
-        b = min(wave * q, nrows);
-        e = min(b + q, nrows);
+        const uint32_t pairs = (nrows + 1u) / 2u;
+        if (S.deal) {
+            const uint32_t base = pairs / NCW, rem = pairs % NCW;
+            const uint32_t pb = wave * base + min(wave, rem);
+            b = min(2u * pb, nrows);
+            e = min(2u * (pb + base + (wave < rem ? 1u : 0u)), nrows);
+        } else {
+            const uint32_t q = 2u * ((pairs + NCW - 1u) / NCW);
+            b = min(wave * q, nrows);
+            e = min(b + q, nrows);
+        }
     };
     const uint32_t c0 = is_head ? head * S64 : 0u;
     float vfirst_keep = 0.0f;
@@ -473,7 +501,7 @@
             }
         };
         if (!is_head) {
-            ENG_BAR();
+            ENG_CBAR(1, ENG_K1_BARRIERS);
             if (*abort_flag) break;
             ENG_STAMP0(l, 1);
             eng_ln_mix<VPT>(ln_wave, xraw0, xs, lnbuf, red, D, eps, wv, bv, mv, pv, tid, lane, wave);
@@ -487,16 +515,21 @@
                 ENG_LDS uint32_t* nopub = nullptr;
                 if (J.f16) {
                     const uint32_t gb = S.g_k1 + J.gbase;
-                    eng_rows<WRK_MAT_F16, false, 4 * XD, 2>(slot, k1_rb, D, xs, k1_row0, rb, re, fin, nopub, A.gran, eng_tag(l, 0),
+                    eng_rows<WRK_MAT_F16, false, 4 * XD, 2>(slot, k1_rb, D, xs, k1_row0, rb, re, fin, nopub, A.gran, eng_tag(ep, l, 0),
                                                             [&](uint32_t r) { return gb + (r >> 1); }, lane);
                 } else {
                     const uint32_t gb = S.g_k1 + S.g_aux + J.gbase * 32u;
-                    eng_rows<QK, R16, XD, 4>(slot, k1_rb, D, xs, k1_row0, rb, re, fin, nopub, A.gran, eng_tag(l, 0),
-                                             [&](uint32_t r) { return gb + (r >> 6) * 96u + ((r & 63u) >> 1); }, lane);
+                    auto gi = [&](uint32_t r) { return gb + (r >> 6) * 96u + ((r & 63u) >> 1); };
+                    bool six = false;
+                    if constexpr (XD == 1) {
+                        six = S.k1_rb6 != 0;
+                        if (six) eng_rows<QK, R16, XD, 6>(slot, k1_rb, D, xs, k1_row0, rb, re, fin, nopub, A.gran, eng_tag(ep, l, 0), gi, lane);
+                    }
+                    if (!six) eng_rows<QK, R16, XD, 4>(slot, k1_rb, D, xs, k1_row0, rb, re, fin, nopub, A.gran, eng_tag(ep, l, 0), gi, lane);
                 }
             }
             ENG_STAMP0(l, 3);
-            ENG_BAR();
+            ENG_CBAR(4, ENG_K1_BARRIERS);
         } else {
             const EngLayer& Lp = A.layers[l];
             const uint8_t* p_m[4] = {Lp.w2, Lp.a2, Lp.g2, layer0 ? Lp.w2 : Lp.v2};
@@ -523,19 +556,19 @@
                 h_w0 = lvec(ENG_V_W0)[cc]; h_a0 = lvec(ENG_V_A0)[cc]; h_kk = lvec(ENG_V_KK)[cc]; h_ka = lvec(ENG_V_KA)[cc]; h_v0 = lvec(ENG_V_V0)[cc];
                 h_gnw = lvec(ENG_V_GNW)[cc]; h_gnb = lvec(ENG_V_GNB)[cc]; h_rk = lvec(ENG_V_RK)[cc];
             }
-            ENG_BAR();
+            ENG_CBAR(1, ENG_K1_BARRIERS);
             if (*abort_flag) break;
             ENG_STAMP0(l, 1);
             eng_ln_mix<VPT>(ln_wave, xraw0, xs, lnbuf, red, D, eps, wv, bv, mv, pv, tid, lane, wave);
             ENG_STAMP0(l, 3);
-            ENG_BAR();
+            ENG_CBAR(4, ENG_K1_BARRIERS);
 
             ENG_LDS float* sh_r = k2f; ENG_LDS float* sh_w = k2f + 64; ENG_LDS float* sh_k = k2f + 128; ENG_LDS float* sh_v = k2f + 192;
             ENG_LDS float* sh_a = k2f + 256; ENG_LDS float* sh_b = k2f + 320; ENG_LDS float* sh_g = k2f + 384; ENG_LDS float* sh_kk = k2f + 448;
             ENG_LDS float* sh_red = k2f + 512;
             ENG_LDS float* sh_red2 = k2f + 768;
             ENG_LDS float* sh_d = k2f + 1024;
-            ENG_BAR();
+            ENG_CBAR(1, ENG_K2_BARRIERS);
             if (*abort_flag) break;
             ENG_STAMP0(l, 4);
             {
@@ -551,7 +584,7 @@
                 }
             }
             ENG_STAMP0(l, 16);
-            ENG_BAR();
+            ENG_CBAR(2, ENG_K2_BARRIERS);
             const ENG_LDS f16* hr = auxbuf + naux, *hk = hr + 64, *hv = hr + 128;
             if (wave == 0) {
                 const float w0 = (float)h_w0, a0 = (float)h_a0, kkw = (float)h_kk, kaw = (float)h_ka;
@@ -581,7 +614,7 @@
             }
             if (wave == 1) lst[c0 + lane] = (float)lnbuf[c0 + lane];
             ENG_STAMP0(l, 17);
-            ENG_BAR();
+            ENG_CBAR(3, ENG_K2_BARRIERS);
             if (ln_wave) {
                 float sa = 0.0f;
                 f32x4 av[4];
@@ -591,7 +624,7 @@
                 for (int jj = 0; jj < 16; ++jj) sa = __builtin_fmaf(Sreg[jj], av[jj >> 2][jj & 3], sa);
                 sh_red[g4 * 64 + ci64] = sa;
             }
-            ENG_BAR();
+            ENG_CBAR(4, ENG_K2_BARRIERS);
             if (ln_wave) {
                 const float sa = (sh_red[ci64] + sh_red[64 + ci64]) + (sh_red[128 + ci64] + sh_red[192 + ci64]);
                 const float vv = sh_v[ci64];
@@ -611,7 +644,7 @@
                 sh_red2[g4 * 64 + ci64] = y;
             }
             ENG_STAMP0(l, 18);
-            ENG_BAR();
+            ENG_CBAR(5, ENG_K2_BARRIERS);
             if (wave == 0) {
                 float y = r16((sh_red2[lane] + sh_red2[64 + lane]) + (sh_red2[128 + lane] + sh_red2[192 + lane]));
                 const float mean = wave_sum(y) * (1.0f / S64);
@@ -622,14 +655,14 @@
                 o = r16(o + xx * sh_v[lane]);
                 o = sh_g[lane] * o;
                 const float o_next = __shfl_down(o, 1, WAVE);
-                if ((lane & 1u) == 0) eng_store_granule(A.gran + S.g_o + ((c0 + lane) >> 1), eng_tag(l, 1), pack_h2(o, o_next));
+                if ((lane & 1u) == 0) eng_store_granule(A.gran + S.g_o + ((c0 + lane) >> 1), eng_tag(ep, l, 1), pack_h2(o, o_next));
             }
             ENG_STAMP0(l, 5);
-            ENG_BAR();
+            ENG_CBAR(6, ENG_K2_BARRIERS);
         }
 
         request_k5();
-        ENG_BAR();
+        ENG_CBAR(1, ENG_K3_BARRIERS);
         if (*abort_flag) break;
         ENG_STAMP0(l, 6);
         {
@@ -638,13 +671,13 @@
             const EngFin fin{WRK_ACT_NONE, sc_o, xraw0, 1.0f};
             const uint32_t gb = S.g_x1;
             ENG_LDS uint32_t* nopub = nullptr;
-            eng_rows<QK, R16, XD, 2>(smem + S.lds_slot3, S.rb_d, D, xs, k3_row0, rb, re, fin, nopub, A.gran, eng_tag(l, 2),
+            eng_rows<QK, R16, XD, 2>(smem + S.lds_slot3, S.rb_d, D, xs, k3_row0, rb, re, fin, nopub, A.gran, eng_tag(ep, l, 2),
                                      [&](uint32_t r) { return gb + (r >> 1); }, lane);
         }
         ENG_STAMP0(l, 7);
-        ENG_BAR();
-
-        ENG_BAR();
+        ENG_CBAR(2, ENG_K3_BARRIERS);
+
+        ENG_CBAR(1, ENG_K5_BARRIERS);
         if (*abort_flag) break;
         ENG_STAMP0(l, 8);
         eng_ln_mix<VPT>(ln_wave, xraw1, xs, lnbuf, red, D, eps, wv, bv, mv, pv, tid, lane, wave);
@@ -654,17 +687,19 @@
             wave_rows(k5_rows, rb, re);
             const EngFin fin{WRK_ACT_SQUARED_RELU, sc_fk, nullptr, 1.0f};
             const uint32_t gb = S.g_k;
-            eng_rows<QK, R16, XD, 4>(smem + S.lds_slot5, S.rb_d, D, xs, k5_row0, rb, re, fin, pub, A.gran, eng_tag(l, 3), [&](uint32_t r) { return gb + (r >> 1); }, lane);
-            ENG_BAR();
-            if (wave == 0) eng_publish(pub, k5_rows, k5_row0, A.gran, eng_tag(l, 3), [&](uint32_t r) { return gb + (r >> 1); }, lane);
+            eng_rows<QK, R16, XD, 4>(smem + S.lds_slot5, S.rb_d, D, xs, k5_row0, rb, re, fin, pub, A.gran, eng_tag(ep, l, 3), [&](uint32_t r) { return gb + (r >> 1); }, lane);
+            ENG_CBAR(4, ENG_K5_BARRIERS);
+            if (wave == 0) eng_publish(pub, k5_rows, k5_row0, A.gran, eng_tag(ep, l, 3), [&](uint32_t r) { return gb + (r >> 1); }, lane);
         }
         ENG_STAMP0(l, 9);
-        ENG_BAR();
+        ENG_CBAR(5, ENG_K5_BARRIERS);
 
         {
             constexpr uint32_t NG = NCW / 4;
             const uint32_t kq = wave & 3u, grp = wave >> 2;
             const bool k6_wave = grp < NG;
+            const bool share = S.k6_share != 0 && NG == 2;
+            ENG_LDS u32x4* k6x = (ENG_LDS u32x4*)(smem + S.k6x[kq]);
             const uint32_t rq = (k6_rows + NG - 1) / NG;
             const uint32_t g_b = min(grp * rq, k6_rows), g_e = min(g_b + rq, k6_rows);
             const uint32_t kpad = (F + 15u) & ~15u;
@@ -678,15 +713,28 @@
                 x[0][ci].s[0] = x[0][ci].s[1] = 0.0f;
                 const f16x8 z = {0, 0, 0, 0, 0, 0, 0, 0};
                 x[0][ci].v[0] = x[0][ci].v[1] = x[0][ci].v[2] = x[0][ci].v[3] = z;
-                if (k6_wave && g_b < g_e && swept) swept = eng_sweep_x<QK>(A.gran + S.g_k, min(c, nch - 1), eng_tag(l, 3), x[0][ci]);
+                const bool sweeps = share ? (grp == 0 && k6_rows > 0) : (k6_wave && g_b < g_e);
+                if (sweeps && swept) swept = eng_sweep_x<QK>(A.gran + S.g_k, min(c, nch - 1), eng_tag(ep, l, 3), x[0][ci]);
                 if (c >= nch) x[0][ci].v[0] = x[0][ci].v[1] = x[0][ci].v[2] = x[0][ci].v[3] = z;
+                if (share && grp == 0 && k6_rows > rq) {
+#pragma unroll
+                    for (int h = 0; h < 4; ++h) k6x[(ci * 4 + h) * 64 + lane] = __builtin_bit_cast(u32x4, x[0][ci].v[h]);
+                }
                 x_sums<QK>(x[0][ci]);
             }
             if (!swept && lane == 0) { *abort_flag = 1; atomicOr(A.fail, 16u); }
             ENG_STAMP0(l, 10);
-            ENG_BAR();
+            ENG_CBAR(1, ENG_K6_BARRIERS);
             if (*abort_flag) break;
             ENG_STAMP0(l, 11);
+            if (share && grp == 1 && g_b < g_e) {
+#pragma unroll
+                for (int ci = 0; ci < XD; ++ci) {
+#pragma unroll
+                    for (int h = 0; h < 4; ++h) x[0][ci].v[h] = __builtin_bit_cast(f16x8, k6x[(ci * 4 + h) * 64 + lane]);
+                    x_sums<QK>(x[0][ci]);
+                }
+            }
             const lds_u8* slot = smem + S.lds_slot6;
             if (k6_wave)
                 for (uint32_t ri = g_b; ri < g_e; ri += 4) {
@@ -708,7 +756,7 @@
                 }
         }
         ENG_STAMP0(l, 12);
-        ENG_BAR();
+        ENG_CBAR(2, ENG_K6_BARRIERS);
         if (wave == 0) {
             const bool valid = lane < k6_rows;
             const uint32_t r = k6_row0 + min(lane, k6_rows ? k6_rows - 1 : 0u);
@@ -722,12 +770,12 @@
             const float o_next = __shfl_down(o, 1, WAVE);
             if (valid) {
                 lst[(size_t)(srows - 1) * D + r] = (float)lnbuf[r];
-                if ((lane & 1u) == 0) eng_store_granule(A.gran + S.g_x + (r >> 1), eng_tag(l, 4), pack_h2(o, o_next));
+                if ((lane & 1u) == 0) eng_store_granule(A.gran + S.g_x + (r >> 1), eng_tag(ep, l, 4), pack_h2(o, o_next));
                 if (l + 1 == S.layer_end) ((f16*)A.x_out)[r] = (f16)o;
             }
         }
         ENG_STAMP0(l, 13);
-        ENG_BAR();
+        ENG_CBAR(3, ENG_K6_BARRIERS);
         ENG_FLUSH(l);
     }
     if (A.stamps && wg == 0 && tid_all == 0) {
@@ -750,6 +798,8 @@
     float* scal = nullptr;
     uint32_t* wg_head = nullptr;
     unsigned long long* gran = nullptr;
+    uint32_t* epoch = nullptr;
+    bool epoch_on = true;
     uint32_t* fail = nullptr;
     unsigned long long* stamps = nullptr;
     void* emb_ln = nullptr;
@@ -783,6 +833,7 @@
         d.lora_w > 128 || d.lora_a > 128 || d.lora_v > 128 || d.lora_g > 256 || ((d.lora_w + d.lora_a + d.lora_g + d.lora_v) % 16))
         return no("LoRA ranks");
     if (NWG < 2 * H || NWG < 64) return no("too few compute units");
+    if (F > 2048 && F <= 4096) return no("ffn value rows of 2049 .. 4096 elements: the launches sum them in another order");
     uint32_t quant = 0xffffffffu, flags = 0xffffffffu;
     for (size_t li = 0; li < m->layers.size(); ++li) {
         const auto& L = m->layers[li];
@@ -800,6 +851,7 @@
     }
     if (quant != WRK_MAT_Q4_K) return no("only Q4_K matrices so far");
     if (m->layers.empty()) return no("no layers");
+    if (m->layers.size() * 8 + 8 > (1u << ENG_TAG_BITS)) return no("too many layers for the tag");
 
     wrk_v7_engine* e = new wrk_v7_engine();
     e->m = m;
@@ -829,12 +881,15 @@
     uint32_t slot1 = 0;
     bool placed = false;
     const uint32_t NK1 = NWG - H;
+    uint32_t force_rows = 0;
+    { const char* fr = getenv("WRK_ENGINE_K1_ROWS"); if (fr && atoi(fr) >= 2) force_rows = (uint32_t)atoi(fr) / 2 * 2; }
     for (double target = total / NK1; target < total; target *= 1.03) {
         uint32_t used = 0, worst = 0;
         uint32_t rpw[ENG_K1_JOBS], nw[ENG_K1_JOBS];
         for (int j = 0; j < ENG_K1_JOBS; ++j) {
             uint32_t r = (uint32_t)(target / jd[j].rb);
             r = std::max(2u, r / 2 * 2);
+            if (force_rows && j < 3) r = force_rows;
             rpw[j] = r;
             nw[j] = (jd[j].rows + r - 1) / r;
             used += nw[j];
@@ -855,6 +910,15 @@
     S.k5_rpw = std::max(8u, up((F + NWG - 1) / NWG, 8));
     S.k6_rpw = std::max(2u, up((D + NWG - 1) / NWG, 2));
     if (S.k6_rpw > 32) { delete e; return no("ffn value rows per workgroup"); }
+    auto env_on = [](const char* name) { const char* v = getenv(name); return !(v && v[0] == '0'); };
+    S.deal = env_on("WRK_ENGINE_DEAL") ? 1u : 0u;
+    S.k6_share = env_on("WRK_ENGINE_SWEEP") ? 1u : 0u;
+    e->epoch_on = env_on("WRK_ENGINE_EPOCH");
+    {
+        uint32_t most = 0;
+        for (int j = 0; j < 3; ++j) most = std::max(most, ((std::min(S.k1[j].rows_per_wg, S.k1[j].rows) + 1) / 2 + 7) / 8);
+        S.k1_rb6 = S.deal && most == 3 && e->xd == 1 ? 1u : 0u;
+    }
     uint32_t off = 0;
     auto take = [&](uint32_t bytes) { const uint32_t o = off; off += up(bytes, 1024); return o; };
     S.lds_slot1 = take(slot1);
@@ -867,6 +931,15 @@
     S.lds_xs = take(D * 2 + up((naux + 192) * 2, 16) + 1280 * 4);
     S.lds_ln = take(D * 2);
     S.lds_misc = take(4096);
+    {
+        const uint32_t qb = 4096u * (uint32_t)e->xd;
+        const uint32_t in_xs = std::min(4u, (S.lds_ln - S.lds_xs) / qb);
+        uint32_t n = 0;
+        for (; n < in_xs; ++n) S.k6x[n] = S.lds_xs + n * qb;
+        if (n < 4 && S.lds_xraw1 - S.lds_xraw0 >= qb) S.k6x[n++] = S.lds_xraw0;
+        if (n < 4 && off + (4 - n) * qb > 160u * 1024u) S.k6_share = 0;
+        if (n < 4 && S.k6_share) { const uint32_t o = take((4 - n) * qb); for (uint32_t i = 0; n < 4; ++n, ++i) S.k6x[n] = o + i * qb; }
+    }
     S.lds_total = off;
     int lds_max = 0;
     hipDeviceGetAttribute(&lds_max, hipDeviceAttributeMaxSharedMemoryPerBlock, ctx->device);
@@ -922,6 +995,9 @@
     if ((er = hipMalloc((void**)&e->wg_head, hh.size() * 4)) != hipSuccess) return fail_alloc(er);
     if ((er = hipMemcpy(e->wg_head, hh.data(), hh.size() * 4, hipMemcpyHostToDevice)) != hipSuccess) return fail_alloc(er);
     if ((er = hipMalloc((void**)&e->gran, (size_t)S.g_total * 8)) != hipSuccess) return fail_alloc(er);
+    if ((er = hipMemset(e->gran, 0, (size_t)S.g_total * 8)) != hipSuccess) return fail_alloc(er);
+    if ((er = hipMalloc((void**)&e->epoch, 256)) != hipSuccess) return fail_alloc(er);
+    { const uint32_t one = 1; if ((er = hipMemcpy(e->epoch, &one, 4, hipMemcpyHostToDevice)) != hipSuccess) return fail_alloc(er); }
     if ((er = hipMalloc((void**)&e->fail, 256)) != hipSuccess) return fail_alloc(er);
     if ((er = hipMemset(e->fail, 0, 256)) != hipSuccess) return fail_alloc(er);
     const char* tm = getenv("WRK_TIMING");
@@ -969,6 +1045,13 @@
 
 bool wrk_v7_engine_has_table(const wrk_v7_engine* e) { return e && e->emb_ln; }
 
+std::string wrk_v7_engine_levers(const wrk_v7_engine* e) {
+    if (!e) return std::string();
+    char b[96];
+    snprintf(b, sizeof b, "levers: deal=%u rb6=%u sweep=%u epoch=%u", e->S.deal, e->S.k1_rb6, e->S.k6_share, e->epoch_on ? 1u : 0u);
+    return b;
+}
+
 void wrk_v7_engine_destroy(wrk_v7_engine* e) {
     if (!e) return;
     if (e->emb_ln) hipFree(e->emb_ln);
@@ -977,13 +1060,18 @@
     if (e->scal) hipFree(e->scal);
     if (e->wg_head) hipFree(e->wg_head);
     if (e->gran) hipFree(e->gran);
+    if (e->epoch) hipFree(e->epoch);
     if (e->fail) hipFree(e->fail);
     if (e->stamps) hipFree(e->stamps);
     delete e;
 }
 
+namespace wrk {
+__global__ void __launch_bounds__(256) eng_epoch_kernel(const EngEpoch E) { eng_epoch_advance(E); }
+}
+
 int32_t wrk_v7_engine_enqueue(wrk_v7_engine* e, hipStream_t q, wrk_v7_state* st, uint32_t batch, uint32_t l0, uint32_t l1, const void* x_in, void* x_out,
-                              void* v_first, const uint32_t* token) {
+                              void* v_first, const uint32_t* token, wrk::EngEpoch* advance) {
     using namespace wrk;
     wrk_ctx* ctx = e->m->ctx;
     EngArgs A{};
@@ -992,10 +1080,42 @@
     A.layers = e->layers; A.vecs = e->vecs; A.scal = e->scal; A.gran = e->gran; A.x_in = x_in; A.x_out = x_out; A.v_first = v_first;
     if (token && e->emb_ln && l0 == 0) { A.x_in = e->emb_ln; A.x_row = token; }
     A.state = st->data; A.num_batch = st->num_batch; A.fail = e->fail; A.stamps = e->stamps; A.stamp_layer = std::min(5u, l1 - 1);
-    WRK_HIP(ctx, hipMemsetAsync(e->gran, 0, (size_t)e->S.g_total * 8, q));
+    A.epoch = e->epoch;
+    if (advance) *advance = EngEpoch{nullptr, nullptr, 0};
+    if (!e->epoch_on) WRK_HIP(ctx, hipMemsetAsync(e->gran, 0, (size_t)e->S.g_total * 8, q));
     const dim3 grid(e->S.nwg), block((e->ncw + 2) * 64);
     hipLaunchKernelGGL(eng_kernel(e->xd, e->r16, e->ncw), grid, block, e->S.lds_total, q, A, (const uint32_t*)e->wg_head);
+    if (e->epoch_on) {
+        const EngEpoch E{e->epoch, e->gran, e->S.g_total};
+        if (advance) *advance = E;
+        else hipLaunchKernelGGL(eng_epoch_kernel, dim3(1), dim3(256), 0, q, E);
+    }
     WRK_LAUNCH_CHECK(ctx);
+    return WRK_OK;
+}
+
+int32_t wrk_v7_engine_debug(wrk_v7_engine* e, uint32_t set_epoch, uint32_t prefill_stale) {
+    using namespace wrk;
+    wrk_ctx* ctx = e->m->ctx;
+    WRK_HIP(ctx, hipStreamSynchronize(ctx->stream));
+    if (set_epoch) {
+        if (set_epoch > ENG_EPOCH_MAX) return wrk_fail(ctx, WRK_E_ARG, "decode engine: epoch %u above %u", set_epoch, ENG_EPOCH_MAX);
+        WRK_HIP(ctx, hipMemcpy(e->epoch, &set_epoch, 4, hipMemcpyHostToDevice));
+    }
+    if (prefill_stale) {
+        uint32_t cur = 1;
+        WRK_HIP(ctx, hipMemcpy(&cur, e->epoch, 4, hipMemcpyDeviceToHost));
+        const uint32_t prev = cur > 1 ? cur - 1 : ENG_EPOCH_MAX, last = (uint32_t)e->m->layers.size() - 1;
+        const EngShape& S = e->S;
+        std::vector<unsigned long long> h(S.g_total, 0ull);
+        const struct { uint32_t begin, stage; } reg[] = {{S.g_x, 4}, {S.g_k1, 0}, {S.g_o, 1}, {S.g_x1, 2}, {S.g_k, 3}};
+        for (size_t r = 0; r < 5; ++r) {
+            const uint32_t end = r + 1 < 5 ? reg[r + 1].begin : S.g_total;
+            const unsigned long long tag = (prev << ENG_TAG_BITS) | (last * 8u + reg[r].stage + 1u);
+            for (uint32_t g = reg[r].begin; g < end; ++g) h[g] = (tag << 32) | 0x7e007e00ull;
+        }
+        WRK_HIP(ctx, hipMemcpy(e->gran, h.data(), h.size() * 8, hipMemcpyHostToDevice));
+    }
     return WRK_OK;
 }
 
@@ -1038,7 +1158,8 @@
                     (double)tail[0] / ((double)tail[1] * 0.01), tail[0], (double)tail[1] * 0.01);
     }
     const int G = e->ncw, Ld = e->ncw + 1;
-    fprintf(stderr, "[WRK_TIMING] decode engine (%d compute waves), one layer of the last token; us since the layer's first stamp\n", e->ncw);
+    fprintf(stderr, "[WRK_TIMING] decode engine (%d compute waves; %s), one layer of the last token; us since the layer's first stamp\n", e->ncw,
+            wrk_v7_engine_levers(e).c_str());
     col(G, 0, "gather: layer input complete");
     col(0, 1, "K1 start (input + weights in LDS), wave 0");
     col(0, 2, "K1 LN + shift done, wave 0");
diff --git a/web-rwkv-gguf_amd/csrc/wrk_v7_fused.hip b/web-rwkv-gguf_amd/csrc/wrk_v7_fused.hip
--- a/web-rwkv-gguf_amd/csrc/wrk_v7_fused.hip
+++ b/web-rwkv-gguf_amd/csrc/wrk_v7_fused.hip
@@ -89,6 +89,7 @@
             }
         }
     }
+    if (P.eng_epoch && blockIdx.x == 0) eng_epoch_advance(EngEpoch{P.eng_epoch, P.eng_gran, P.eng_ngran});
 }
 
 int ln_mix(hipStream_t s, const LnMixParams& P, uint32_t T) {
@@ -498,10 +499,12 @@
         LN(P, T);
     }
     uint32_t first_launch_layer = layer_begin;
+    EngEpoch eng_epoch{nullptr, nullptr, 0};
     if (T == 1 && engine_on() && !engine_skip_once) {
         const uint32_t l1 = std::min<uint32_t>(d.num_layer, layer_end);
         if (layer_begin < l1) {
-            const int32_t rc = wrk_v7_engine_enqueue(engine, q, st, cursor0_batch, layer_begin, l1, s.x, s.x, s.att_v0, eng_embeds ? s.tokens : nullptr);
+            const int32_t rc = wrk_v7_engine_enqueue(engine, q, st, cursor0_batch, layer_begin, l1, s.x, s.x, s.att_v0, eng_embeds ? s.tokens : nullptr,
+                                                     NH > 0 ? &eng_epoch : nullptr);
             if (rc != WRK_OK) return rc;
         }
         first_launch_layer = l1;
@@ -634,6 +637,7 @@
         P.src = (const f16*)s.x; P.ids = identity_headers ? nullptr : s.headers;
         P.ln_w = (const f16*)ln_out_w->ptr; P.ln_b = (const f16*)ln_out_b->ptr; P.eps = 1.0e-5f;
         P.d = D; P.nmix = 0; P.ln_out = (f16*)s.head_x;
+        P.eng_epoch = eng_epoch.epoch; P.eng_gran = eng_epoch.gran; P.eng_ngran = eng_epoch.ngran;
         LN(P, NH);
         MatJob j = mat_job(head, make_dense(s.head_x, WRK_F16, D, NH), make_dense(s.head_o, WRK_F32, V, NH), WRK_ACT_NONE);
         uint32_t nwg = 0;
diff --git a/web-rwkv-gguf_amd/wrk/__init__.py b/web-rwkv-gguf_amd/wrk/__init__.py
--- a/web-rwkv-gguf_amd/wrk/__init__.py
+++ b/web-rwkv-gguf_amd/wrk/__init__.py
@@ -124,6 +124,7 @@
     "wrk_v7_infer": (C.c_int32, [_P, _P, _P, _u32p, C.POINTER(C.c_uint16), _u32p, C.c_uint32, _u32p, C.c_uint32, _f32p, _u32p, C.c_uint32]),
     "wrk_v7_model_set_frame_dtype": (C.c_int32, [_P, _P, C.c_uint32]),
     "wrk_v7_model_engine_status": (C.c_int32, [_P, _P, C.c_char_p, C.c_size_t]),
+    "wrk_v7_model_engine_debug": (C.c_int32, [_P, _P, C.c_uint32, C.c_uint32]),
     "wrk_v7_infer_layer": (C.c_int32, [_P, _P, _P, C.c_uint32, _P, _P, _u32p, C.c_uint32, C.c_uint32]),
     "wrk_v7_frame_read": (C.c_int32, [_P, _P, C.c_char_p, C.c_uint32, _P, C.c_size_t, C.POINTER(C.c_size_t)]),
     "wrk_v7_generate_greedy": (C.c_int32, [_P, _P, _P, _u32p, C.c_uint32, C.c_uint32, _u32p, _f32p, _f32p, C.c_uint32]),
@@ -839,6 +840,9 @@
             self.ctx.check(rc)
         return rc == 1, buf.value.decode()
 
+    def engine_debug(self, set_epoch: int = 0, prefill_stale: bool = False):
+        self.ctx.check(hip.wrk_v7_model_engine_debug(self.ctx.h, self.model, set_epoch, 1 if prefill_stale else 0))
+
     def infer_layer(self, layer: int, x: np.ndarray, v_first: Optional[np.ndarray], cursors, mode: int = 0):
         dt = np.float32 if getattr(self, "frame_dtype", F16) == F32 else np.float16
         xa = np.ascontiguousarray(x, dtype=dt)
```

New measurement: 1794 tokens/s (median of 6 runs). +7.7%, better.
